# bdaiinstitute/vlfm

Measured on AMD Instinct MI355X. Metric: env-steps/s (VLM+value-map update), 640x480 RGB-D, higher is better.
Workload: dtype f16 ViT-g (f32 accumulate) + f32 Q-Former (split-f16, 22-bit); f32 confidence + f64 value maps; 1 GPU; configs[1] step x resident envs: BLIP-2 ITC + ValueMap+ObstacleMap+sort_waypoints; envs_per_gpu=256, global_envs=256, map=1000x1000 @ 20 px/m, parallelism=env-sharded x1, tuned_gemms=True, vit_gemm=hip:fc1, attention=hip

## Files before the change

### include/vlfm_amd.h

```cpp
#ifndef VLFM_AMD_H
#define VLFM_AMD_H

#include <stddef.h>
#include <stdint.h>

#ifdef __cplusplus
extern "C" {
#endif

typedef enum {
    VLFM_OK = 0,
    VLFM_ERR_INVALID = -1,
    VLFM_ERR_OUTSIDE_MAP = -2,
    VLFM_ERR_INDEX = -3,
    VLFM_ERR_HIP = -4,
    VLFM_ERR_CAPACITY = -5
} vlfm_status;

enum { VLFM_FUSE_DEFAULT = 0, VLFM_FUSE_REPLACE = 1, VLFM_FUSE_EQUAL_WEIGHTING = 2 };

const char* vlfm_last_error(void);
int vlfm_abi_version(void);

int vlfm_profile_enable(int on);
int vlfm_profile_read(const char* kernel_name, double* mean_ms, int* launches);

int vlfm_host_wait_mode(int blocking);

typedef struct {
    double inv_affine[6];
    int32_t row0, col0;
    int32_t env;
    int32_t reserved;
} vlfm_vm_pose;

int vlfm_value_map_pose_params(const double* h_tf, const double* h_yaw, const int32_t* h_env, int n, int map_size,
                               int pixels_per_meter, int template_size, vlfm_vm_pose* h_out, int* bad_index);

int vlfm_cone_template_host(double fov, double max_depth, int pixels_per_meter, double min_confidence,
                            float* h_conf, int conf_capacity, int64_t* h_poly_xy, int poly_capacity,
                            int* n_poly);

int vlfm_tan_table_host(double fov, int width, double* h_out);

int vlfm_cone_template_build(const float* d_conf, const int64_t* d_poly_xy, int n_poly, int template_size,
                             float* d_template, uint32_t* d_template_bits, void* stream);

typedef struct {
    double tf[12];
    float depth_scale;
    float depth_offset;
    float depth_max;
    float reserved0;
    double fx, fy;
    double min_height, max_height;
    int32_t env;
    int32_t scatter;
} vlfm_ingest_params;

typedef struct {
    uint32_t* d_cells;
    int32_t* d_count;
    int32_t capacity;
    int32_t reserved;
} vlfm_scatter_journal;

int vlfm_depth_ingest_batched(const float* d_depth, int n, int height, int width,
                              const vlfm_ingest_params* d_params,
                              uint32_t* d_colmax_keys ,
                              uint32_t* d_obstacle , int map_size, int pixels_per_meter,
                              int32_t* d_status ,
                              uint32_t* d_hole_bits ,
                              const uint32_t* d_filled_bits ,
                              const vlfm_scatter_journal* journal ,
                              void* stream);

int vlfm_selftest_div_exact(const double* d_numerators, int n, double divisor, int32_t* d_mismatches, void* stream);

size_t vlfm_hole_scratch_bytes(int n, int height, int width, int cap_pts, int cap_contours);
int vlfm_fill_small_holes_batched(const uint32_t* d_hole_bits, const int32_t* d_status, int n, int height, int width,
                                  double area_thresh, void* d_scratch, size_t scratch_bytes, int cap_pts,
                                  int cap_contours, uint32_t* d_filled_bits, int32_t* d_counts,
                                  const vlfm_ingest_params* d_params, uint32_t* d_obstacle, int map_size,
                                  const vlfm_scatter_journal* journal, void* stream);
int vlfm_depth_scatter_holes_batched(const vlfm_ingest_params* d_params, int n, int height, int width,
                                     const uint32_t* d_hole_bits, const uint32_t* d_filled_bits,
                                     const int32_t* d_hole_counts ,
                                     uint32_t* d_obstacle, int map_size, int pixels_per_meter, int32_t* d_status,
                                     const float* d_depth ,
                                     void* stream);

int vlfm_fill_small_holes_rig_batched(const uint32_t* d_hole_bits, const int32_t* d_status, int n, int height, int width,
                                      double area_thresh, void* d_scratch, size_t scratch_bytes, int cap_pts,
                                      int cap_contours, uint32_t* d_filled_bits, int32_t* d_counts,
                                      const vlfm_ingest_params* d_params, uint32_t* d_obstacle, int map_size,
                                      const vlfm_scatter_journal* journal, int32_t* d_slot_undone, int n_envs, void* stream);
int vlfm_depth_scatter_holes_rig_batched(const vlfm_ingest_params* d_params, int n, int height, int width,
                                         const uint32_t* d_hole_bits, const uint32_t* d_filled_bits,
                                         const int32_t* d_hole_counts, uint32_t* d_obstacle, int map_size,
                                         int pixels_per_meter, int32_t* d_status, const float* d_depth,
                                         const int32_t* d_slot_undone, void* stream);

int vlfm_value_map_update_fused_batched(uint32_t* d_colmax_keys, int width, const double* d_tan,
                                        const float* d_template, const uint32_t* d_template_bits, int template_size,
                                        const vlfm_vm_pose* d_pose, const double* d_values, int n,
                                        float* d_conf, double* d_value, int map_size, int channels, int pixels_per_meter,
                                        double min_depth, double max_depth, int use_max_confidence, int fusion_type,
                                        const uint32_t* d_explored_bits, uint32_t* d_written_bits, int32_t* d_counters,
                                        const float* d_conf_quadrant, void* stream);

typedef struct {
    const float* d_template;
    const uint32_t* d_template_bits;
    const float* d_conf_quadrant;
    const double* d_tan;
    float depth_scale;
    float depth_offset;
    int32_t template_size;
    int32_t reserved;
} vlfm_vm_optics;

int vlfm_value_map_update_rig_batched(uint32_t* d_colmax_keys, int width, const vlfm_vm_pose* d_pose,
                                      const vlfm_vm_optics* d_optics, const int32_t* d_slots, int n_slots, int n,
                                      int max_template_size, const double* d_values, float* d_conf, double* d_value,
                                      int map_size, int channels, int pixels_per_meter, int use_max_confidence,
                                      int fusion_type, const uint32_t* d_explored_bits, uint32_t* d_written_bits,
                                      int32_t* d_counters, void* stream);

int vlfm_disc_rows_host(int radius, int32_t* h_halfwidth );
int vlfm_value_map_sort_waypoints_batched(const double* d_value, int map_size, int channels,
                                          const int32_t* d_cells, int m, int radius, const int32_t* d_disc,
                                          int value_is_f32, double* d_out, void* stream);



int vlfm_resample_coeffs_host(int in_size, int out_size, int32_t* h_bounds, int32_t* h_kk, int kk_capacity,
                              int* ksize_out);

int vlfm_resample_coeffs_filter_host(int in_size, int out_size, int filter, int32_t* h_bounds, int32_t* h_kk,
                                     int kk_capacity, int* ksize_out);

int vlfm_preprocess_sam_batched(const uint8_t* d_rgb, int n, int height, int width, int out_h, int out_w,
                                const int32_t* d_hbounds, const int32_t* d_hk, int hksize,
                                const int32_t* d_vbounds, const int32_t* d_vk, int vksize,
                                const float* h_mean3, const float* h_std3, int pad_size, uint8_t* d_tmp, float* d_out,
                                void* stream);

int vlfm_preprocess_rgb_batched(const uint8_t* d_rgb, int n, int height, int width, int out_size,
                                const int32_t* d_hbounds, const int32_t* d_hk, int hksize,
                                const int32_t* d_vbounds, const int32_t* d_vk, int vksize,
                                const float* h_mean3, const float* h_std3, uint8_t* d_tmp, void* d_out,
                                int out_dtype, int patch_size, void* stream);

int vlfm_itc_head_batched(const float* d_proj, int batch, int n_query, int proj_dim,
                          const float* d_text, float* d_out, void* stream);

#define VLFM_ITC_MAX_PROMPTS 8
int vlfm_itc_head_multi(const float* d_proj, int batch, int n_query, int proj_dim, const float* d_text_table, int n_text,
                        const int32_t* d_text_index, int n_prompts, float* d_out, void* stream);

int vlfm_layernorm_bias_f16(const void* d_x, const float* d_channel_bias, const void* d_gamma, const void* d_beta,
                            void* d_y, int rows, int dim, float eps, void* stream);

int vlfm_vit_attention_f16(const void* d_qkv, void* d_out, int batch, int tokens, int heads, int head_dim, float scale,
                           void* stream);

int vlfm_gemm_f16_nt(const void* d_x, const void* d_w, const void* d_bias, void* d_c, int m, int n, int k, int epilogue,
                     void* stream);

int vlfm_gemm_f16_pair_f32_nt(const void* d_x, const void* d_w_pair, const void* d_bias_f32, void* d_out, int m, int n_out, int k,
                              void* stream);

int vlfm_qformer_cross_attention_f32(const void* d_q, const void* d_kv_blocks, void* d_out, int batch, int tokens, int queries,
                                     int heads, int k_block0, int v_block0, int m_total, float scale, void* stream);

int vlfm_gemm_f16_tile_order(int m, int n, int group_m, int* out, int capacity_pairs);
int vlfm_gemm_f16_work_items(int m, int n, int grid, int* out, int capacity_pairs);

int vlfm_split_f32_to_f16_pair(const float* d_src, void* d_hi, void* d_lo, long long count, int* d_overflow, void* stream);
int vlfm_gemm_f32_nt(const float* d_x, const float* d_w, const float* d_bias, const float* d_residual, float* d_c, int m, int n,
                     int k, int activation, int precision, const void* d_w_hi, const void* d_w_lo, int* d_overflow, void* stream);


int vlfm_layernorm_rows_f32(const float* d_x, const float* d_gamma, const float* d_beta, float* d_out, int batch, int height,
                            int width, int channels, int window, float eps, void* stream);
int vlfm_window_reverse_add_f32(float* d_x, const float* d_windows, int batch, int height, int width, int channels, int window,
                                void* stream);
int vlfm_dwconv3x3_nhwc_f32(const float* d_x, const float* d_w9c, const float* d_bias, float* d_out, int batch, int height, int width,
                            int channels, void* stream);
int vlfm_window_attention_f32(const float* d_qkv, const float* d_bias_t, float* d_out, long long windows, int tokens, int heads,
                              float scale, void* stream);
int vlfm_layernorm_rows_shifted_f32(const float* d_x, const float* d_gamma, const float* d_beta, float* d_out, int batch, int height,
                                    int width, int channels, int window, float eps, int shift, int pad_zero, void* stream);
int vlfm_window_reverse_add_shifted_f32(float* d_x, const float* d_windows, int batch, int height, int width, int channels, int window,
                                        int shift, void* stream);
int vlfm_window_attention_masked_f32(const float* d_qkv, const float* d_bias_t, const float* d_mask_t, int windows_per_image, float* d_out,
                                     long long windows, int tokens, int heads, float scale, void* stream);

int vlfm_maxpool2x2_nhwc_f16(const void* d_x, void* d_out, int batch, int height, int width, int channels, void* stream);
int vlfm_conv_nhwc_tile(int pixels, int cin, int cout, int ksize, int* tile_pixels, int* tile_channels);
int vlfm_conv_nhwc_f16(const void* d_x, const void* d_w, const void* d_bias, void* d_out, const void* d_zero, int batch,
                       int height, int width, int cin, int cout, int ksize, int stride, int x_pix_stride,
                       int out_pix_stride, int act, void* stream);

int vlfm_resize_area_tab_host(int ssize, int dsize, int32_t* h_first, int32_t* h_count, float* h_w, int ktaps_capacity);

int vlfm_resize_area_batched(const uint8_t* d_rgb, int n, int height, int width, int out_h, int out_w,
                             const int32_t* d_xfirst, const int32_t* d_xcount, const float* d_xw, int xktaps,
                             const int32_t* d_yfirst, const int32_t* d_ycount, const float* d_yw, int yktaps,
                             void* d_out, int out_dtype, void* stream);

int vlfm_to_tensor_normalize_batched(const uint8_t* d_rgb, int n, int height, int width, const float* h_mean3,
                                     const float* h_std3, float* d_out, void* stream);

size_t vlfm_nms_scratch_bytes(int n);
int vlfm_nms(const float* d_boxes_xyxy, const int32_t* d_order, int n, float iou_threshold, void* d_scratch,
             size_t scratch_bytes, int32_t* d_keep, int32_t* d_num_keep, int max_keep, void* stream);

int vlfm_ms_deform_attn(const float* d_value, const int32_t* d_spatial_shapes, const int32_t* d_level_start,
                        const float* d_sampling_loc, const float* d_attn_weight, int batch, int n_query, int n_heads,
                        int head_dim, int n_levels, int n_points, int total_len, float* d_out, void* stream);
int vlfm_ms_deform_attn_fused(const float* d_value, const int32_t* d_spatial_shapes, const int32_t* d_level_start,
                              const float* d_offsets_logits, const float* d_reference, int batch, int n_query, int n_heads,
                              int head_dim, int n_levels, int n_points, int ref_coords, int total_len, float* d_out, void* stream);

int vlfm_dwconv3x3_f32(const float* d_x, const float* d_w, const float* d_bias, float* d_y, int n, int channels, int height,
                       int width, int stride, int gelu, void* stream);

int vlfm_bias_act_nchw(void* d_y, const void* d_bias, int n, int channels, long long hw, int dtype, int act, void* stream);


size_t vlfm_object_cloud_scratch_bytes(int height, int width);
int vlfm_object_cloud_extract(const float* d_depth, const uint8_t* d_mask, int height, int width, int erosion_iterations,
                              double min_depth, double max_depth, double fx, double fy, void* d_scratch, double* d_cloud,
                              int capacity, int32_t* d_count, void* stream);

size_t vlfm_dbscan_scratch_bytes(int n);
int vlfm_dbscan_largest_cluster(const double* d_points, int n, double eps, int min_points, void* d_scratch,
                                size_t scratch_bytes, int32_t* d_labels, int32_t* d_keep, int32_t* d_num_keep, void* stream);

size_t vlfm_object_cloud_batch_scratch_bytes(int jobs, int height, int width);
int vlfm_object_cloud_batch_stats(const uint8_t* d_masks, const int32_t* d_erosion, int jobs, int max_erosion, int height, int width,
                                  void* d_scratch, int32_t* d_stats, void* stream);
int vlfm_object_cloud_batch_expand(const float* d_depth, int frames, int height, int width, double min_depth, double max_depth,
                                   double fx, double fy, const void* d_scratch, int scratch_jobs, const int32_t* d_jobs, int n_jobs,
                                   int max_points, const int32_t* d_ranks, int n_ranks, double* d_points, int capacity, void* stream);
size_t vlfm_dbscan_batch_scratch_bytes(int n);
int vlfm_dbscan_largest_cluster_batch(const double* d_points, int capacity, const int64_t* d_jobs, int n_jobs, int max_n, double eps,
                                      int min_points, void* d_scratch, size_t scratch_bytes, double* d_kept, int32_t* d_num_keep,
                                      void* stream);
long long vlfm_object_cloud_launch_count(void);


typedef struct {
    const double* d_rows;
    const int32_t* d_slots;
    double p[3];
    double heading, half_fov, range;
    int32_t n, k, flag_offset, n_slots;
} vlfm_cloud_query;

int vlfm_cloud_cone_flags(const vlfm_cloud_query* d_queries, int n_queries, int max_points, int32_t* d_flags, void* stream);

size_t vlfm_cloud_closest_scratch_bytes(int n_queries, int max_points);
int vlfm_cloud_closest(const vlfm_cloud_query* d_queries, int n_queries, int max_points, void* d_scratch, size_t scratch_bytes,
                       int32_t* d_result, void* stream);
int vlfm_cloud_query_chunk(void);
long long vlfm_cloud_query_launch_count(void);

int vlfm_bits_pack(const uint8_t* d_src, uint32_t* d_dst, int planes, int rows, int cols, void* stream);
int vlfm_bits_unpack(const uint32_t* d_src, uint8_t* d_dst, int planes, int rows, int cols, void* stream);

int vlfm_bits_dilate(const uint32_t* d_src, uint32_t* d_dst, int planes, int rows, int cols, int kernel_w,
                     int kernel_h, void* stream);

int vlfm_find_contours_external(const uint32_t* d_img, int planes, int rows, int cols, int method,
                                uint32_t* d_scratch , int32_t* d_pts, int cap_pts,
                                int32_t* d_starts, int32_t* d_lens, int cap_contours, int32_t* d_counts, void* stream);

size_t vlfm_find_contours_wg_scratch_bytes(int planes, int rows, int cols, int cap_pts);
int vlfm_walk_path_counters(long long* h_out4, int reset);
int vlfm_find_contours_external_wg(const uint32_t* d_img, int planes, int rows, int cols, int method, void* d_scratch,
                                   size_t scratch_bytes, int32_t* d_pts, int cap_pts, int32_t* d_starts, int32_t* d_lens,
                                   int cap_contours, int32_t* d_counts, void* stream);

#define VLFM_FOG_MAX_POLY 80
typedef struct {
    int32_t env;
    int32_t ax, ay;
    int32_t radius;
    int32_t n_poly;
    int32_t reserved;
    double rot_c, rot_s;
    double line_len;
    long long poly[2 * VLFM_FOG_MAX_POLY];
} vlfm_fog_params;

int vlfm_fog_params_host(const int32_t* h_agent_px, const double* h_angle_cv2_deg, const double* h_rot_cs,
                         double fov_deg, double max_line_len, const int32_t* h_env, const int32_t* h_explore, int n,
                         vlfm_fog_params* h_out);

size_t vlfm_obstacle_scratch_bytes(int n_envs, int map_size, int cap_pts, int cap_contours);

int vlfm_obstacle_map_update_batched(const vlfm_fog_params* d_prm, int n, const uint32_t* d_obstacle,
                                     uint32_t* d_navigable, uint32_t* d_explored, int32_t* d_bbox, int n_envs,
                                     int map_size, int kernel_size, int fog_radius, double area_thresh_px,
                                     void* d_scratch, size_t scratch_bytes, int cap_pts, int cap_contours,
                                     double* d_frontiers, int cap_frontiers, int32_t* d_counts, int update_obstacles,
                                     int explore, const int32_t* d_windows, int window_blocks_navigable,
                                     int window_blocks_prepare, void* stream);

int vlfm_obstacle_status(const void* d_scratch, int n_envs, int map_size, int cap_pts, int cap_contours,
                         int32_t* h_out);

enum { VLFM_REDUCE_MAX = 0,
       VLFM_REDUCE_EXPLORE = 1,
       VLFM_REDUCE_PLANE = 2 };
enum { VLFM_PRIM_CIRCLE_FILL = 0,
       VLFM_PRIM_CIRCLE = 1,
       VLFM_PRIM_LINE = 2,
       VLFM_PRIM_POLYLINE = 3 };
#define VLFM_RENDER_FLIP_ROWS 1
#define VLFM_RENDER_UNDER_PATH 2
typedef struct {
    int32_t frame;
    int32_t kind;
    int32_t flags;
    int32_t thickness;
    int32_t x0, y0, x1, y1;
    int32_t vtx_off, n_vtx;
    uint8_t bgr[4];
    int32_t reserved;
} vlfm_render_prim;

size_t vlfm_value_render_scratch_bytes(int n, int map_size);

int vlfm_value_map_render(const double* d_value, int n_envs, int map_size, int channels, const int32_t* d_frames, int n,
                          int reduce_mode, double explore_thresh, const double* d_plane, const uint32_t* d_explored,
                          const uint32_t* d_path, const int32_t* d_prim_off, const vlfm_render_prim* d_prims,
                          const int64_t* d_vtx, int rgb, void* d_scratch, size_t scratch_bytes, uint8_t* d_out,
                          void* stream);

int vlfm_obstacle_map_render(const uint32_t* d_obstacle, const uint32_t* d_navigable, const uint32_t* d_explored,
                             int n_envs, int map_size, const int32_t* d_frames, int n, uint32_t pad_bgr,
                             const uint32_t* d_path, const int32_t* d_prim_off, const vlfm_render_prim* d_prims,
                             const int64_t* d_vtx, int rgb, uint8_t* d_out, void* stream);

int vlfm_traj_append(uint32_t* d_path, int n_envs, int map_size, const int32_t* d_segs, int m, int thickness,
                     void* stream);

int vlfm_circle_polygon_host(const int32_t* h_circles, int n, int64_t* h_xy, int32_t* h_off, int capacity);

int vlfm_jpeg_quant_tables_host(int quality, uint16_t* h_tables);
size_t vlfm_jpeg_scratch_bytes(int n, int H, int W);
int vlfm_jpeg_roundtrip_batched(const uint8_t* d_in, uint8_t* d_out, int n, int H, int W, const uint16_t* h_tables,
                                void* d_scratch, size_t scratch_bytes, void* stream);

int vlfm_jpeg_header_host(int quality, int H, int W, uint8_t* h_out, size_t cap, size_t* len);
size_t vlfm_jpeg_encode_bound(int H, int W);
size_t vlfm_jpeg_encode_scratch_bytes(int n, int H, int W);
int vlfm_jpeg_encode_batched(const uint8_t* d_in, int n, int H, int W, int rgb_order, const uint16_t* h_tables,
                             uint8_t* d_out, size_t capacity, uint32_t* d_lengths, void* d_scratch, size_t scratch_bytes,
                             void* stream);

typedef struct vlfm_jpeg_huff {
    uint32_t limit[16];
    int32_t delta[16];
    uint8_t vals[256];
} vlfm_jpeg_huff;
typedef struct vlfm_jpeg_table_set {
    uint16_t quant[3][64];
    vlfm_jpeg_huff dc[3];
    vlfm_jpeg_huff ac[3];
} vlfm_jpeg_table_set;
typedef struct vlfm_jpeg_frame {
    int32_t height, width, restart_interval, scan_offset, table_set, reserved[3];
} vlfm_jpeg_frame;
enum {
    VLFM_JPEG_BAD_HEADER = 1,
    VLFM_JPEG_BAD_LENGTH = 2,
    VLFM_JPEG_BAD_EOI = 3,
    VLFM_JPEG_BAD_RESTART = 4,
    VLFM_JPEG_BAD_CODE = 5,
    VLFM_JPEG_BAD_SIZE = 6,
    VLFM_JPEG_BAD_INDEX = 7,
    VLFM_JPEG_BAD_BITS = 8
};
int vlfm_jpeg_parse_host(const uint8_t* h_file, size_t len, vlfm_jpeg_frame* frame, vlfm_jpeg_table_set* set);
const char* vlfm_jpeg_parse_reason(int code);
size_t vlfm_jpeg_decode_chunk_bytes(void);
size_t vlfm_jpeg_decode_scratch_bytes(int n, int H, int W, size_t max_file_bytes);
int vlfm_jpeg_decode_batched(const uint8_t* d_files, size_t files_bytes, const int64_t* d_offsets, size_t stride,
                             const int32_t* d_lengths, int n, int H, int W, const vlfm_jpeg_frame* d_frames,
                             const vlfm_jpeg_table_set* d_sets, int n_sets, const uint8_t* d_header, int header_bytes,
                             int max_segments, size_t max_file_bytes, int rgb_order, uint8_t* d_out, int32_t* d_status,
                             void* d_scratch, size_t scratch_bytes, void* stream);

int vlfm_rooms_raycast(const double* d_cameras, int n, const double* d_boxes, int n_boxes, int H, int W, float* d_out,
                       void* stream);

int vlfm_rooms_raycast_objects(const double* d_cameras, int n, const double* d_boxes, int n_boxes, const double* d_objects,
                               const int32_t* d_env_of, int n_envs, int H, int W, float* d_depth, uint8_t* d_ids,
                               int32_t* d_stats, void* stream);

#ifdef __cplusplus
}
#endif
#endif
```

### vlfm_amd/_lib.py

```python
from __future__ import annotations

import ctypes
import os
import subprocess
from typing import Optional

_HERE = os.path.dirname(os.path.abspath(__file__))
LIB_PATH = os.path.join(_HERE, "libvlfm_amd.so")
SOURCES = ["value_map.hip", "depth_ingest.hip", "depth_holes.hip", "obstacle_map.hip", "vlm_ops.hip", "vit_attention.hip", "qformer_attention.hip", "detect_ops.hip", "object_cloud.hip", "cloud_query.hip", "gemm_f16.hip", "gemm_f32.hip", "conv_nhwc.hip", "sam_ops.hip", "map_render.hip", "jpeg_codec.hip", "jpeg_entropy.hip", "jpeg_decode.hip", "world_render.hip", "host.cpp"]

VLFM_OK = 0
VLFM_ERR_INVALID = -1
VLFM_ERR_OUTSIDE_MAP = -2
VLFM_ERR_INDEX = -3
VLFM_ERR_HIP = -4
VLFM_ERR_CAPACITY = -5

FUSION_TYPES = {"default": 0, "replace": 1, "equal_weighting": 2}


class VmPose(ctypes.Structure):
    _fields_ = [("inv_affine", ctypes.c_double * 6), ("row0", ctypes.c_int32), ("col0", ctypes.c_int32),
                ("env", ctypes.c_int32), ("reserved", ctypes.c_int32)]


class IngestParams(ctypes.Structure):
    _fields_ = [("tf", ctypes.c_double * 12), ("depth_scale", ctypes.c_float), ("depth_offset", ctypes.c_float),
                ("depth_max", ctypes.c_float), ("reserved0", ctypes.c_float), ("fx", ctypes.c_double),
                ("fy", ctypes.c_double), ("min_height", ctypes.c_double), ("max_height", ctypes.c_double),
                ("env", ctypes.c_int32), ("scatter", ctypes.c_int32)]


FOG_MAX_POLY = 80


class FogParams(ctypes.Structure):
    _fields_ = [("env", ctypes.c_int32), ("ax", ctypes.c_int32), ("ay", ctypes.c_int32), ("radius", ctypes.c_int32),
                ("n_poly", ctypes.c_int32), ("reserved", ctypes.c_int32), ("rot_c", ctypes.c_double),
                ("rot_s", ctypes.c_double), ("line_len", ctypes.c_double), ("poly", ctypes.c_longlong * (2 * FOG_MAX_POLY))]


class ScatterJournal(ctypes.Structure):
    _fields_ = [("d_cells", ctypes.c_void_p), ("d_count", ctypes.c_void_p), ("capacity", ctypes.c_int32),
                ("reserved", ctypes.c_int32)]


class VmOptics(ctypes.Structure):
    _fields_ = [("d_template", ctypes.c_void_p), ("d_template_bits", ctypes.c_void_p), ("d_conf_quadrant", ctypes.c_void_p),
                ("d_tan", ctypes.c_void_p), ("depth_scale", ctypes.c_float), ("depth_offset", ctypes.c_float),
                ("template_size", ctypes.c_int32), ("reserved", ctypes.c_int32)]


class CloudQuery(ctypes.Structure):
    _fields_ = [("d_rows", ctypes.c_void_p), ("d_slots", ctypes.c_void_p), ("p", ctypes.c_double * 3),
                ("heading", ctypes.c_double), ("half_fov", ctypes.c_double), ("range", ctypes.c_double),
                ("n", ctypes.c_int32), ("k", ctypes.c_int32), ("flag_offset", ctypes.c_int32), ("n_slots", ctypes.c_int32)]


assert ctypes.sizeof(CloudQuery) == 80
assert ctypes.sizeof(ScatterJournal) == 24 and ctypes.sizeof(VmOptics) == 48
assert ctypes.sizeof(VmPose) == 64 and ctypes.sizeof(IngestParams) == 152 and ctypes.sizeof(FogParams) == 48 + 16 * FOG_MAX_POLY


def build(verbose: bool = False) -> str:
    from concurrent.futures import ThreadPoolExecutor

    csrc = os.path.join(_HERE, "csrc")
    srcs = [os.path.join(csrc, s) for s in SOURCES if os.path.exists(os.path.join(csrc, s))]
    hdrs = [os.path.join(csrc, h) for h in os.listdir(csrc) if h.endswith(".h")] + [
        os.path.join(_HERE, "..", "include", "vlfm_amd.h")]
    hdr_time = max(os.path.getmtime(h) for h in hdrs)
    objdir = os.path.join(csrc, "build")
    os.makedirs(objdir, exist_ok=True)
    flags = ["--offload-arch=gfx950", "-O3", "-std=c++17", "-fPIC", "-ffp-contract=off"]

    def compile_one(src: str) -> str:
        obj = os.path.join(objdir, os.path.basename(src) + ".o")
        if not os.path.exists(obj) or os.path.getmtime(obj) < max(os.path.getmtime(src), hdr_time):
            cmd = ["hipcc"] + flags + ["-c", src, "-o", obj]
            if verbose:
                print(" ".join(cmd), flush=True)
            subprocess.check_call(cmd)
        return obj

    with ThreadPoolExecutor(max_workers=min(8, len(srcs))) as pool:
        objs = list(pool.map(compile_one, srcs))
    if os.path.exists(LIB_PATH) and all(os.path.getmtime(LIB_PATH) >= os.path.getmtime(o) for o in objs):
        return LIB_PATH
    cmd = ["hipcc", "--offload-arch=gfx950", "-shared", "-fPIC", "-o", LIB_PATH] + objs
    if verbose:
        print(" ".join(cmd), flush=True)
    subprocess.check_call(cmd)
    return LIB_PATH


_lib: Optional[ctypes.CDLL] = None


def lib() -> ctypes.CDLL:
    global _lib
    if _lib is None:
        if not os.path.exists(LIB_PATH):
            raise ImportError(
                f"{LIB_PATH} is missing: build it with `python -c 'import __graft_entry__ as g; g.build()'` "
                "(hipcc --offload-arch=gfx950).  vlfm_amd has no CPU fallback.")
        L = ctypes.CDLL(LIB_PATH)
        vp, ci, cd = ctypes.c_void_p, ctypes.c_int, ctypes.c_double
        L.vlfm_last_error.restype = ctypes.c_char_p
        L.vlfm_abi_version.restype = ci
        L.vlfm_profile_enable.argtypes = [ci]
        L.vlfm_host_wait_mode.argtypes = [ci]
        L.vlfm_profile_read.argtypes = [ctypes.c_char_p, ctypes.POINTER(cd), ctypes.POINTER(ci)]
        L.vlfm_value_map_pose_params.argtypes = [vp, vp, vp, ci, ci, ci, ci, vp, ctypes.POINTER(ci)]
        L.vlfm_cone_template_host.argtypes = [cd, cd, ci, cd, vp, ci, vp, ci, ctypes.POINTER(ci)]
        L.vlfm_tan_table_host.argtypes = [cd, ci, vp]
        L.vlfm_disc_rows_host.argtypes = [ci, vp]
        L.vlfm_cone_template_build.argtypes = [vp, vp, ci, ci, vp, vp, vp]
        L.vlfm_depth_ingest_batched.argtypes = [vp, ci, ci, ci, vp, vp, vp, ci, ci, vp, vp, vp, vp, vp]
        L.vlfm_selftest_div_exact.argtypes = [vp, ci, cd, vp, vp]
        L.vlfm_hole_scratch_bytes.argtypes = [ci, ci, ci, ci, ci]
        L.vlfm_hole_scratch_bytes.restype = ctypes.c_size_t
        L.vlfm_fill_small_holes_batched.argtypes = [vp, vp, ci, ci, ci, cd, vp, ctypes.c_size_t, ci, ci, vp, vp, vp, vp,
                                                    ci, vp, vp]
        L.vlfm_depth_scatter_holes_batched.argtypes = [vp, ci, ci, ci, vp, vp, vp, vp, ci, ci, vp, vp, vp]
        L.vlfm_fill_small_holes_rig_batched.argtypes = [vp, vp, ci, ci, ci, cd, vp, ctypes.c_size_t, ci, ci, vp, vp, vp, vp,
                                                        ci, vp, vp, ci, vp]
        L.vlfm_depth_scatter_holes_rig_batched.argtypes = [vp, ci, ci, ci, vp, vp, vp, vp, ci, ci, vp, vp, vp, vp]
        L.vlfm_layernorm_bias_f16.argtypes = [vp, vp, vp, vp, vp, ci, ci, ctypes.c_float, vp]
        L.vlfm_vit_attention_f16.argtypes = [vp, vp, ci, ci, ci, ci, ctypes.c_float, vp]
        L.vlfm_gemm_f16_nt.argtypes = [vp, vp, vp, vp, ci, ci, ci, ci, vp]
        L.vlfm_gemm_f16_pair_f32_nt.argtypes = [vp, vp, vp, vp, ci, ci, ci, vp]
        L.vlfm_qformer_cross_attention_f32.argtypes = [vp, vp, vp, ci, ci, ci, ci, ci, ci, ci, ctypes.c_float, vp]
        L.vlfm_gemm_f32_nt.argtypes = [vp, vp, vp, vp, vp, ci, ci, ci, ci, ci, vp, vp, vp, vp]
        L.vlfm_split_f32_to_f16_pair.argtypes = [vp, vp, vp, ctypes.c_longlong, vp, vp]
        L.vlfm_layernorm_rows_f32.argtypes = [vp, vp, vp, vp, ci, ci, ci, ci, ci, ctypes.c_float, vp]
        L.vlfm_window_reverse_add_f32.argtypes = [vp, vp, ci, ci, ci, ci, ci, vp]
        L.vlfm_dwconv3x3_nhwc_f32.argtypes = [vp, vp, vp, vp, ci, ci, ci, ci, vp]
        L.vlfm_window_attention_f32.argtypes = [vp, vp, vp, ctypes.c_longlong, ci, ci, ctypes.c_float, vp]
        L.vlfm_layernorm_rows_shifted_f32.argtypes = [vp, vp, vp, vp, ci, ci, ci, ci, ci, ctypes.c_float, ci, ci, vp]
        L.vlfm_window_reverse_add_shifted_f32.argtypes = [vp, vp, ci, ci, ci, ci, ci, ci, vp]
        L.vlfm_window_attention_masked_f32.argtypes = [vp, vp, vp, ci, vp, ctypes.c_longlong, ci, ci, ctypes.c_float, vp]
        L.vlfm_maxpool2x2_nhwc_f16.argtypes = [vp, vp, ci, ci, ci, ci, vp]
        L.vlfm_conv_nhwc_tile.argtypes = [ci, ci, ci, ci, ctypes.POINTER(ci), ctypes.POINTER(ci)]
        L.vlfm_conv_nhwc_f16.argtypes = [vp, vp, vp, vp, vp, ci, ci, ci, ci, ci, ci, ci, ci, ci, ci, vp]
        L.vlfm_value_map_update_fused_batched.argtypes = [vp, ci, vp, vp, vp, ci, vp, vp, ci, vp, vp, ci, ci, ci, cd, cd,
                                                          ci, ci, vp, vp, vp, vp, vp]
        L.vlfm_value_map_update_rig_batched.argtypes = [vp, ci, vp, vp, vp, ci, ci, ci, vp, vp, vp, ci, ci, ci, ci, ci, vp, vp,
                                                        vp, vp]
        L.vlfm_value_map_sort_waypoints_batched.argtypes = [vp, ci, ci, vp, ci, ci, vp, ci, vp, vp]
        L.vlfm_resample_coeffs_host.argtypes = [ci, ci, vp, vp, ci, ctypes.POINTER(ci)]
        L.vlfm_resample_coeffs_filter_host.argtypes = [ci, ci, ci, vp, vp, ci, ctypes.POINTER(ci)]
        L.vlfm_preprocess_sam_batched.argtypes = [vp, ci, ci, ci, ci, ci, vp, vp, ci, vp, vp, ci, vp, vp, ci, vp, vp, vp]
        L.vlfm_preprocess_rgb_batched.argtypes = [vp, ci, ci, ci, ci, vp, vp, ci, vp, vp, ci, vp, vp, vp, vp, ci, ci, vp]
        L.vlfm_itc_head_batched.argtypes = [vp, ci, ci, ci, vp, vp, vp]
        L.vlfm_itc_head_multi.argtypes = [vp, ci, ci, ci, vp, ci, vp, ci, vp, vp]
        cf = ctypes.c_float
        L.vlfm_resize_area_tab_host.argtypes = [ci, ci, vp, vp, vp, ci]
        L.vlfm_resize_area_batched.argtypes = [vp, ci, ci, ci, ci, ci, vp, vp, vp, ci, vp, vp, vp, ci, vp, ci, vp]
        L.vlfm_to_tensor_normalize_batched.argtypes = [vp, ci, ci, ci, vp, vp, vp, vp]
        L.vlfm_nms_scratch_bytes.argtypes = [ci]
        L.vlfm_nms_scratch_bytes.restype = ctypes.c_size_t
        L.vlfm_nms.argtypes = [vp, vp, ci, cf, vp, ctypes.c_size_t, vp, vp, ci, vp]
        L.vlfm_ms_deform_attn.argtypes = [vp, vp, vp, vp, vp, ci, ci, ci, ci, ci, ci, ci, vp, vp]
        L.vlfm_ms_deform_attn_fused.argtypes = [vp, vp, vp, vp, vp, ci, ci, ci, ci, ci, ci, ci, ci, vp, vp]
        L.vlfm_object_cloud_scratch_bytes.argtypes = [ci, ci]
        L.vlfm_object_cloud_scratch_bytes.restype = ctypes.c_size_t
        L.vlfm_object_cloud_extract.argtypes = [vp, vp, ci, ci, ci, cd, cd, cd, cd, vp, vp, ci, vp, vp]
        L.vlfm_dbscan_scratch_bytes.argtypes = [ci]
        L.vlfm_dbscan_scratch_bytes.restype = ctypes.c_size_t
        L.vlfm_dbscan_largest_cluster.argtypes = [vp, ci, cd, ci, vp, ctypes.c_size_t, vp, vp, vp, vp]
        L.vlfm_object_cloud_batch_scratch_bytes.argtypes = [ci, ci, ci]
        L.vlfm_object_cloud_batch_scratch_bytes.restype = ctypes.c_size_t
        L.vlfm_object_cloud_batch_stats.argtypes = [vp, vp, ci, ci, ci, ci, vp, vp, vp]
        L.vlfm_object_cloud_batch_expand.argtypes = [vp, ci, ci, ci, cd, cd, cd, cd, vp, ci, vp, ci, ci, vp, ci, vp, ci, vp]
        L.vlfm_dbscan_batch_scratch_bytes.argtypes = [ci]
        L.vlfm_dbscan_batch_scratch_bytes.restype = ctypes.c_size_t
        L.vlfm_dbscan_largest_cluster_batch.argtypes = [vp, ci, vp, ci, ci, cd, ci, vp, ctypes.c_size_t, vp, vp, vp]
        L.vlfm_object_cloud_launch_count.argtypes = []
        L.vlfm_object_cloud_launch_count.restype = ctypes.c_longlong
        L.vlfm_cloud_cone_flags.argtypes = [vp, ci, ci, vp, vp]
        L.vlfm_cloud_closest_scratch_bytes.argtypes = [ci, ci]
        L.vlfm_cloud_closest_scratch_bytes.restype = ctypes.c_size_t
        L.vlfm_cloud_closest.argtypes = [vp, ci, ci, vp, ctypes.c_size_t, vp, vp]
        L.vlfm_cloud_query_chunk.argtypes = []
        L.vlfm_cloud_query_launch_count.argtypes = []
        L.vlfm_cloud_query_launch_count.restype = ctypes.c_longlong
        L.vlfm_bits_pack.argtypes = [vp, vp, ci, ci, ci, vp]
        L.vlfm_bits_unpack.argtypes = [vp, vp, ci, ci, ci, vp]
        L.vlfm_bits_dilate.argtypes = [vp, vp, ci, ci, ci, ci, ci, vp]
        L.vlfm_find_contours_external.argtypes = [vp, ci, ci, ci, ci, vp, vp, ci, vp, vp, ci, vp, vp]
        L.vlfm_dwconv3x3_f32.argtypes = [vp, vp, vp, vp, ci, ci, ci, ci, ci, ci, vp]
        L.vlfm_bias_act_nchw.argtypes = [vp, vp, ci, ci, ctypes.c_longlong, ci, ci, vp]
        L.vlfm_find_contours_wg_scratch_bytes.argtypes = [ci, ci, ci, ci]
        L.vlfm_find_contours_wg_scratch_bytes.restype = ctypes.c_size_t
        L.vlfm_find_contours_external_wg.argtypes = [vp, ci, ci, ci, ci, vp, ctypes.c_size_t, vp, ci, vp, vp, ci, vp, vp]
        L.vlfm_walk_path_counters.argtypes = [vp, ci]
        L.vlfm_fog_params_host.argtypes = [vp, vp, vp, cd, cd, vp, vp, ci, vp]
        L.vlfm_obstacle_scratch_bytes.argtypes = [ci, ci, ci, ci]
        L.vlfm_obstacle_scratch_bytes.restype = ctypes.c_size_t
        L.vlfm_obstacle_map_update_batched.argtypes = [vp, ci, vp, vp, vp, vp, ci, ci, ci, ci, cd, vp, ctypes.c_size_t,
                                                       ci, ci, vp, ci, vp, ci, ci, vp, ci, ci, vp]
        L.vlfm_obstacle_status.argtypes = [vp, ci, ci, ci, ci, vp]
        L.vlfm_value_render_scratch_bytes.argtypes = [ci, ci]
        L.vlfm_value_render_scratch_bytes.restype = ctypes.c_size_t
        L.vlfm_value_map_render.argtypes = [vp, ci, ci, ci, vp, ci, ci, cd, vp, vp, vp, vp, vp, vp, ci, vp,
                                            ctypes.c_size_t, vp, vp]
        L.vlfm_obstacle_map_render.argtypes = [vp, vp, vp, ci, ci, vp, ci, ctypes.c_uint32, vp, vp, vp, vp, ci, vp, vp]
        L.vlfm_traj_append.argtypes = [vp, ci, ci, vp, ci, ci, vp]
        L.vlfm_circle_polygon_host.argtypes = [vp, ci, vp, vp, ci]
        L.vlfm_jpeg_quant_tables_host.argtypes = [ci, vp]
        L.vlfm_jpeg_scratch_bytes.argtypes = [ci, ci, ci]
        L.vlfm_jpeg_scratch_bytes.restype = ctypes.c_size_t
        L.vlfm_jpeg_roundtrip_batched.argtypes = [vp, vp, ci, ci, ci, vp, vp, ctypes.c_size_t, vp]
        L.vlfm_jpeg_header_host.argtypes = [ci, ci, ci, vp, ctypes.c_size_t, ctypes.POINTER(ctypes.c_size_t)]
        L.vlfm_jpeg_encode_bound.argtypes = [ci, ci]
        L.vlfm_jpeg_encode_bound.restype = ctypes.c_size_t
        L.vlfm_jpeg_encode_scratch_bytes.argtypes = [ci, ci, ci]
        L.vlfm_jpeg_encode_scratch_bytes.restype = ctypes.c_size_t
        L.vlfm_jpeg_encode_batched.argtypes = [vp, ci, ci, ci, ci, vp, vp, ctypes.c_size_t, vp, vp, ctypes.c_size_t, vp]
        L.vlfm_jpeg_parse_host.argtypes = [vp, ctypes.c_size_t, vp, vp]
        L.vlfm_jpeg_parse_reason.argtypes = [ci]
        L.vlfm_jpeg_parse_reason.restype = ctypes.c_char_p
        L.vlfm_jpeg_decode_chunk_bytes.restype = ctypes.c_size_t
        L.vlfm_jpeg_decode_scratch_bytes.argtypes = [ci, ci, ci, ctypes.c_size_t]
        L.vlfm_jpeg_decode_scratch_bytes.restype = ctypes.c_size_t
        L.vlfm_jpeg_decode_batched.argtypes = [vp, ctypes.c_size_t, vp, ctypes.c_size_t, vp, ci, ci, ci, vp, vp, ci, vp, ci, ci,
                                               ctypes.c_size_t, ci, vp, vp, vp, ctypes.c_size_t, vp]
        L.vlfm_rooms_raycast.argtypes = [vp, ci, vp, ci, ci, ci, vp, vp]
        L.vlfm_rooms_raycast_objects.argtypes = [vp, ci, vp, ci, vp, vp, ci, ci, ci, vp, vp, vp, vp]
        _lib = L
    return _lib


def profile_read(kernel: str):
    ms, n = ctypes.c_double(0.0), ctypes.c_int(0)
    lib().vlfm_profile_read(kernel.encode(), ctypes.byref(ms), ctypes.byref(n))
    return ms.value, n.value


def last_error() -> str:
    return lib().vlfm_last_error().decode()


def host_wait_blocking(device=None, blocking: bool = True) -> None:
    import torch

    with torch.cuda.device(device if device is not None else torch.cuda.current_device()):
        check(lib().vlfm_host_wait_mode(int(bool(blocking))), "host_wait_mode")


def try_host_wait_blocking(device=None) -> bool:
    import os
    import warnings

    if os.environ.get("VLFM_HOST_WAIT", "blocking") == "spin":
        return False
    try:
        host_wait_blocking(device)
        return True
    except Exception as exc:
        warnings.warn(f"blocking host waits not enabled on {device}: {exc} (call vlfm_amd._lib.host_wait_blocking before the "
                      f"device's first allocation; waits will spin on a host core)")
        return False


def check(rc: int, what: str = "") -> int:
    if rc >= 0:
        return rc
    msg = last_error()
    if rc == VLFM_ERR_OUTSIDE_MAP:
        raise AssertionError(msg or "Pixel location is outside the image.")
    if rc == VLFM_ERR_INDEX:
        raise IndexError(msg or "index out of bounds for obstacle map")
    raise RuntimeError(f"libvlfm_amd {what} failed ({rc}): {msg}")
```

### vlfm_amd/csrc/gemm_f16.hip

```cpp
#include <hip/hip_runtime.h>
#include <stdint.h>

#include "../../include/vlfm_amd.h"
#include "gelu_f16.h"
#include "profile.h"
#include "status.h"

namespace vlfm {

typedef _Float16 half8 __attribute__((ext_vector_type(8)));
typedef _Float16 half4 __attribute__((ext_vector_type(4)));
typedef float floatx4 __attribute__((ext_vector_type(4)));
typedef float f32x16 __attribute__((ext_vector_type(16)));

constexpr int GB = 256;
constexpr int GK = 64;
constexpr int ROWB = GK * 2;
constexpr int OPER = GB * ROWB;
constexpr int BUF = 2 * OPER;
constexpr int EPI_ROW = 272;
constexpr int EPI_WAVE = 64 * EPI_ROW;
constexpr int GEMM_LDS = 8 * EPI_WAVE > 2 * BUF ? 8 * EPI_WAVE : 2 * BUF;
enum { EPI_BIAS = 0, EPI_BIAS_GELU = 1, EPI_ACCUM = 2,
       EPI_PAIR_F32 = 3 };

struct GemmArgs {
    const _Float16* x;
    const _Float16* w;
    const _Float16* bias;
    _Float16* c;
    int M, N, K;
    int tiles_m, tiles_n;
    int group_m;
    int split_ragged;
};

using lds_ptr = __attribute__((address_space(3))) unsigned char*;
using gbl_ptr = const __attribute__((address_space(1))) unsigned char*;

template <int EPI, int BAL, int SYNC = 2>
struct Gemm8p {
    static constexpr int SLOT = 128 * ROWB;
    static constexpr int KBUF = 4 * SLOT;

    const GemmArgs& a;
    lds_ptr lds;
    const unsigned char* smem;
    int wave, lane;
    bool half;
    bool active;
    uint32_t voff[4][2];
    uint32_t rdP[2], rdQ[2];
    half8 fp[4][2], fq0[BAL ? 2 : 1][2][2], fq1[2][2];
    floatx4 acc[8][4];

    __device__ Gemm8p(const GemmArgs& a_, unsigned char* smem_, int m0, int n0) : a(a_), lds((lds_ptr)smem_), smem(smem_) {
        const int tid = threadIdx.x;
        lane = tid & 63;
        wave = __builtin_amdgcn_readfirstlane(tid >> 6);
        const int wn = wave >> 2, wm = wave & 3;
        half = false;
        active = n0 + wn * (half ? 64 : 128) < a.N;
        offsets(m0, n0, voff);
        const int r16 = lane & 15, swz = (r16 >> 1) & 7, s0 = lane >> 4;
        const uint32_t bp = (uint32_t)(wn * 64 + r16) * ROWB + (uint32_t)((s0 ^ swz) << 4);
        const uint32_t bq = (uint32_t)(wm * 32 + r16) * ROWB + (uint32_t)((s0 ^ swz) << 4);
        rdP[0] = bp; rdP[1] = bp ^ 64u;
        rdQ[0] = bq; rdQ[1] = bq ^ 64u;
        zero_acc();
    }
    __device__ inline void zero_acc() {
#pragma unroll
        for (int i = 0; i < 8; i++)
#pragma unroll
            for (int j = 0; j < 4; j++) acc[i][j] = floatx4{0.f, 0.f, 0.f, 0.f};
    }
    __device__ inline void kill_fragments() {
        const half8 z = {(_Float16)0.f, (_Float16)0.f, (_Float16)0.f, (_Float16)0.f, (_Float16)0.f, (_Float16)0.f, (_Float16)0.f, (_Float16)0.f};
#pragma unroll
        for (int f = 0; f < 4; f++) { fp[f][0] = z; fp[f][1] = z; }
#pragma unroll
        for (int g = 0; g < 2; g++)
#pragma unroll
            for (int k = 0; k < 2; k++) {
                fq1[g][k] = z;
#pragma unroll
                for (int q = 0; q < (BAL ? 2 : 1); q++) fq0[q][g][k] = z;
            }
    }
    __device__ inline void offsets(int m0, int n0, uint32_t (&vo)[4][2]) const {
        const int sub = lane >> 3, p = lane & 7;
#pragma unroll
        for (int j = 0; j < 2; j++) {
            const int rho = (wave * 2 + j) * 8 + sub;
            const int s = p ^ ((rho >> 1) & 7);
#pragma unroll
            for (int h = 0; h < 2; h++) {
                const int rq = min(m0 + (rho >> 5) * 64 + h * 32 + (rho & 31), a.M - 1);
                const int rp = min(n0 + (half ? rho + h * 128 : (rho >> 6) * 128 + h * 64 + (rho & 63)), a.N - 1);
                vo[2 * h][j] = (uint32_t)rq * (uint32_t)a.K * 2u + (uint32_t)s * 16u;
                vo[2 * h + 1][j] = (uint32_t)rp * (uint32_t)a.K * 2u + (uint32_t)s * 16u;
            }
        }
    }

    template <int SLOT_ID>
    __device__ inline void stage_at(int b, int t, const uint32_t (&vo)[4][2]) {
        const unsigned char* base = reinterpret_cast<const unsigned char*>((SLOT_ID & 1) ? a.w : a.x) + (size_t)t * (GK * 2);
#pragma unroll
        for (int j = 0; j < 2; j++) {
            const int dst = __builtin_amdgcn_readfirstlane(b * KBUF + SLOT_ID * SLOT + (wave * 2 + j) * 1024);
            __builtin_amdgcn_global_load_lds((gbl_ptr)(base + vo[SLOT_ID][j]), lds + dst, 16, 0, 0);
        }
    }
    template <int SLOT_ID>
    __device__ inline void stage(int b, int t) { stage_at<SLOT_ID>(b, t, voff); }
    template <int B, int SLOT_ID>
    __device__ inline void read_p() {
#pragma unroll
        for (int kk = 0; kk < 2; kk++)
#pragma unroll
            for (int f = 0; f < 4; f++)
                fp[f][kk] = *reinterpret_cast<const half8*>(smem + B * KBUF + SLOT_ID * SLOT + f * 16 * ROWB + rdP[kk]);
    }
    template <int B, int SLOT_ID>
    __device__ inline void read_q(half8 (&fq)[2][2]) {
#pragma unroll
        for (int kk = 0; kk < 2; kk++)
#pragma unroll
            for (int g = 0; g < 2; g++)
                fq[g][kk] = *reinterpret_cast<const half8*>(smem + B * KBUF + SLOT_ID * SLOT + g * 16 * ROWB + rdQ[kk]);
    }
    template <int PI, int QJ>
    __device__ inline void mma(const half8 (&fq)[2][2]) {
#pragma unroll
        for (int kk = 0; kk < 2; kk++)
#pragma unroll
            for (int f = 0; f < 4; f++)
#pragma unroll
                for (int g = 0; g < 2; g++)
                    acc[PI * 4 + f][QJ * 2 + g] =
                        __builtin_amdgcn_mfma_f32_16x16x32_f16(fp[f][kk], fq[g][kk], acc[PI * 4 + f][QJ * 2 + g], 0, 0, 0);
    }
    static __device__ inline void bar() {
        __builtin_amdgcn_s_barrier();
        asm volatile("" ::: "memory");
    }
    template <int PI, int QJ>
    __device__ inline void compute(const half8 (&fq)[2][2], bool work = true) {
        bar();
        __builtin_amdgcn_s_waitcnt(0xC07F);
        __builtin_amdgcn_sched_barrier(0);
        if (active && work) {
            __builtin_amdgcn_s_setprio(1);
            mma<PI, QJ>(fq);
            __builtin_amdgcn_s_setprio(0);
        }
        __builtin_amdgcn_sched_barrier(0);
        if (SYNC == 2) bar();
    }

    template <int B>
    __device__ inline void tile(int t, int NT) {
        constexpr int QS = BAL ? B : 0;
        if (active) {
            if (!BAL) read_q<B, 0>(fq0[QS]);
            read_p<B, 1>();
        }
        __builtin_amdgcn_sched_barrier(0);
        if (t + 1 < NT) stage<2>(B ^ 1, t + 1);
        compute<0, 0>(fq0[QS]);
        if (active) read_q<B, 2>(fq1);
        __builtin_amdgcn_sched_barrier(0);
        if (t + 1 < NT) stage<3>(B ^ 1, t + 1);
        compute<0, 1>(fq1);
        if (active) read_p<B, 3>();
        __builtin_amdgcn_sched_barrier(0);
        if (t + 2 < NT) {
            stage<0>(B, t + 2);
            if (BAL) __builtin_amdgcn_s_waitcnt(0x0F78);
        } else if (BAL) {
            __builtin_amdgcn_s_waitcnt(0x0F76);
        }
        compute<1, 1>(fq1);
        if (BAL && active && t + 1 < NT) read_q<B ^ 1, 0>(fq0[BAL ? (B ^ 1) : 0]);
        __builtin_amdgcn_sched_barrier(0);
        if (t + 2 < NT) {
            stage<1>(B, t + 2);
            __builtin_amdgcn_s_waitcnt(0x0F74);
        } else {
            __builtin_amdgcn_s_waitcnt(0x0F70);
        }
        compute<1, 0>(fq0[QS]);
    }
};

__host__ __device__ inline void tile_of(const GemmArgs& a, int bid, int& tm, int& tn) {
    const int nwg = a.tiles_m * a.tiles_n;
    const int xcd = bid & 7, idx = bid >> 3;
    const int tail_cols = a.N - (a.tiles_n - 1) * GB;
    const bool ragged = a.tiles_n > 1 && tail_cols <= GB / 2;
    const int ncols = ragged ? a.tiles_n - 1 : a.tiles_n;
    const int nfull = a.tiles_m * ncols, nhalf = nwg - nfull;
    const int qf = nfull >> 3, rf = nfull & 7, qh = nhalf >> 3, rh = nhalf & 7;
    const int myfull = qf + (xcd < rf ? 1 : 0);
    if (idx < myfull) {
        const int f = xcd * qf + min(xcd, rf) + idx;
        const int GM = a.group_m;
        const int per_group = GM * ncols, grp = f / per_group, in = f - grp * per_group;
        const int rows = min(GM, a.tiles_m - grp * GM);
        tn = in / rows;
        tm = grp * GM + (in - tn * rows);
    } else {
        int before = 0;
        for (int x = 0; x < xcd; x++) before += (((x - rf) & 7) < rh) ? 1 : 0;
        tm = xcd * qh + before + (idx - myfull);
        tn = a.tiles_n - 1;
    }
}

constexpr int EPI2_ROW = 144;
constexpr int EPI2_WAVE = 64 * EPI2_ROW;
constexpr int PBIAS_OFF = GEMM_LDS;
constexpr int GEMM_LDS_P = GEMM_LDS + 512;

__device__ __forceinline__ half8 add_half8(half8 a, const half8 b) {
#pragma unroll
    for (int e = 0; e < 8; e++) a[e] = (_Float16)((float)a[e] + (float)b[e]);
    return a;
}
template <int EPI, int H>
__device__ __forceinline__ void epi2_pass(const floatx4 (&acc)[8][4], const half4 (&bias4)[8], unsigned char* stg, int g4, int c16, int rsub,
                                 int chunk, half8 (&v)[8]) {
#pragma unroll
    for (int ii = 0; ii < 4; ii++) {
        constexpr int I0 = H * 4;
        const float b0 = (float)bias4[I0 + ii][0], b1 = (float)bias4[I0 + ii][1], b2 = (float)bias4[I0 + ii][2], b3 = (float)bias4[I0 + ii][3];
#pragma unroll
        for (int j = 0; j < 4; j++) {
            float v0 = acc[I0 + ii][j][0] + b0, v1 = acc[I0 + ii][j][1] + b1, v2 = acc[I0 + ii][j][2] + b2, v3 = acc[I0 + ii][j][3] + b3;
            if (EPI == EPI_BIAS_GELU) gelu_erf4(v0, v1, v2, v3);
            const half4 hv = {(_Float16)v0, (_Float16)v1, (_Float16)v2, (_Float16)v3};
            *reinterpret_cast<half4*>(stg + (j * 16 + c16) * EPI2_ROW + (ii * 16 + g4) * 2) = hv;
        }
    }
    __builtin_amdgcn_s_waitcnt(0xC07F);
#pragma unroll
    for (int it = 0; it < 8; it++) v[it] = *reinterpret_cast<const half8*>(stg + (it * 8 + rsub) * EPI2_ROW + chunk * 16);
}
template <int P>
__device__ __forceinline__ void epi_pair_pass(const floatx4 (&acc)[8][4], const floatx4 (&bias4)[4], unsigned char* stg, int g4, int c16,
                                              int rsub, int chunk, floatx4 (&v)[8]) {
#pragma clang fp contract(off)
#pragma unroll
    for (int i2 = 0; i2 < 2; i2++) {
        constexpr int I0 = 2 * P;
#pragma unroll
        for (int j = 0; j < 4; j++) {
            floatx4 r;
#pragma unroll
            for (int e = 0; e < 4; e++) {
                const float low = acc[4 + I0 + i2][j][e] * 0x1p-11f;
                const float mid = bias4[I0 + i2][e] + low;
                r[e] = acc[I0 + i2][j][e] + mid;
            }
            *reinterpret_cast<floatx4*>(stg + (j * 16 + c16) * EPI2_ROW + (i2 * 16 + g4) * 4) = r;
        }
    }
    __builtin_amdgcn_s_waitcnt(0xC07F);
#pragma unroll
    for (int it = 0; it < 8; it++) v[it] = *reinterpret_cast<const floatx4*>(stg + (it * 8 + rsub) * EPI2_ROW + chunk * 16);
}
__device__ __forceinline__ void stage_bias(const GemmArgs& a, lds_ptr lds, int wave, int lane, int n_first) {
    if (a.bias != nullptr && wave == 0 && lane < 32) {
        const _Float16* src = a.bias + min(n_first + lane * 8, a.N - 8);
        __builtin_amdgcn_global_load_lds((gbl_ptr)src, lds + PBIAS_OFF, 16, 0, 0);
    }
}

struct WorkList {
    int nwg, first_split, nitems;
    __host__ __device__ WorkList(int nwg_, int grid, bool allow = true) : nwg(nwg_) {
        const int left = nwg > grid ? nwg % grid : 0;
        const bool split = allow && left > 0 && 2 * left <= grid;
        first_split = split ? nwg - left : nwg;
        nitems = nwg + (split ? left : 0);
    }
    __host__ __device__ void item(int w, int& pos, int& half) const {
        if (w < first_split) { pos = w; half = -1; }
        else { const int j = w - first_split; pos = first_split + (j >> 1); half = j & 1; }
    }
};

template <int EPI>
__global__ __launch_bounds__(512) void gemm_f16_8pp_kernel(GemmArgs a) {
    extern __shared__ __attribute__((aligned(16))) unsigned char smem[];
    using G = Gemm8p<EPI, 1, 2>;
    const int stride = gridDim.x;
    const WorkList work(a.tiles_m * a.tiles_n, stride, a.split_ragged != 0);
    int bid = blockIdx.x;
    int tm, tn, pos, half;
    work.item(bid, pos, half);
    tile_of(a, pos, tm, tn);
    int m0 = tm * GB, n0 = tn * GB;
    G g(a, smem, m0, n0);
    g.active = g.active && (half < 0 || half == (g.wave >> 2));
    const int NT = a.K / GK;
    const int wave = g.wave, lane = g.lane, wn = wave >> 2, wm = wave & 3, late = wn;
    const int g4 = (lane >> 4) * 4, c16 = lane & 15;
    const int rsub = lane >> 3, chunk = lane & 7;
    unsigned char* stg = smem + G::KBUF + wave * EPI2_WAVE;
    const bool has_bias = a.bias != nullptr;
    stage_bias(a, g.lds, wave, lane, n0);
    g.template stage<0>(0, 0); g.template stage<1>(0, 0); g.template stage<2>(0, 0); g.template stage<3>(0, 0);
    if (NT > 1) {
        g.template stage<0>(1, 1); g.template stage<1>(1, 1);
        __builtin_amdgcn_s_waitcnt(0x0F74);
    } else {
        __builtin_amdgcn_s_waitcnt(0x0F70);
    }
    g.bar();
    for (;;) {
        g.kill_fragments();
        if (late) g.bar();
        if (g.active) g.template read_q<0, 0>(g.fq0[0]);
        for (int t = 0; t < NT; t += 2) {
            g.template tile<0>(t, NT);
            if (t + 1 < NT) g.template tile<1>(t + 1, NT);
        }
        if (!late) g.bar();

        half4 bias4[EPI == EPI_PAIR_F32 ? 1 : 8];
        floatx4 biasf[EPI == EPI_PAIR_F32 ? 4 : 1];
        if constexpr (EPI == EPI_PAIR_F32) {
#pragma unroll
            for (int i = 0; i < 4; i++) {
                const floatx4 ld = *reinterpret_cast<const floatx4*>(smem + PBIAS_OFF + (wn * 64 + i * 16 + g4) * 4);
                biasf[i] = has_bias ? ld : floatx4{0.f, 0.f, 0.f, 0.f};
            }
        } else {
#pragma unroll
            for (int i = 0; i < 8; i++) {
                const half4 ld = *reinterpret_cast<const half4*>(smem + PBIAS_OFF + (wn * 128 + i * 16 + g4) * 2);
                bias4[i] = has_bias ? ld : half4{(_Float16)0.f, (_Float16)0.f, (_Float16)0.f, (_Float16)0.f};
            }
        }
        __builtin_amdgcn_sched_barrier(0);
        const int nbid = bid + stride;
        const bool more = nbid < work.nitems;
        const bool store = g.active;
        work.item(more ? nbid : bid, pos, half);
        tile_of(a, pos, tm, tn);
        const int m1 = tm * GB, n1 = tn * GB;
        uint32_t von[4][2];
        g.offsets(m1, n1, von);
        g.template stage_at<0>(0, 0, von); g.template stage_at<1>(0, 0, von);
        g.template stage_at<2>(0, 0, von); g.template stage_at<3>(0, 0, von);
        __builtin_amdgcn_sched_barrier(0);
        half8 old[EPI == EPI_ACCUM ? 16 : 1];
        if (EPI == EPI_ACCUM) {
#pragma unroll
            for (int h = 0; h < 2; h++)
#pragma unroll
                for (int it = 0; it < 8; it++) {
                    const int m = min(m0 + wm * 64 + it * 8 + rsub, a.M - 1);
                    const int n = max(min(n0 + wn * 128 + h * 64 + chunk * 8, a.N - 8), 0);
                    old[h * 8 + it] = *reinterpret_cast<const half8*>(a.c + (size_t)m * a.N + n);
                }
        }
        __builtin_amdgcn_sched_barrier(0);
        if constexpr (EPI == EPI_PAIR_F32) {
            (void)bias4; (void)old;
            floatx4 p0[8], p1[8];
            epi_pair_pass<0>(g.acc, biasf, stg, g4, c16, rsub, chunk, p0);
            epi_pair_pass<1>(g.acc, biasf, stg, g4, c16, rsub, chunk, p1);
            __builtin_amdgcn_sched_barrier(0);
            __builtin_amdgcn_s_waitcnt(0x0F70);
            __builtin_amdgcn_sched_barrier(0);
            const int nblk = n0 + wn * 128;
            if (store && nblk + 128 <= a.N) {
                float* ob = reinterpret_cast<float*>(a.c) + (size_t)(nblk >> 7) * (size_t)a.M * 64 + chunk * 4;
#pragma unroll
                for (int it = 0; it < 8; it++) {
                    const int m = m0 + wm * 64 + it * 8 + rsub;
                    if (m < a.M) *reinterpret_cast<floatx4*>(ob + (size_t)m * 64) = p0[it];
                }
#pragma unroll
                for (int it = 0; it < 8; it++) {
                    const int m = m0 + wm * 64 + it * 8 + rsub;
                    if (m < a.M) *reinterpret_cast<floatx4*>(ob + (size_t)m * 64 + 32) = p1[it];
                }
            }
        } else {
        (void)biasf;
        half8 v0[8], v1[8];
        epi2_pass<EPI, 0>(g.acc, bias4, stg, g4, c16, rsub, chunk, v0);
        epi2_pass<EPI, 1>(g.acc, bias4, stg, g4, c16, rsub, chunk, v1);
        if (EPI == EPI_ACCUM) {
#pragma unroll
            for (int it = 0; it < 8; it++) {
                v0[it] = add_half8(v0[it], old[it]);
                v1[it] = add_half8(v1[it], old[8 + it]);
            }
        }
        __builtin_amdgcn_sched_barrier(0);
        __builtin_amdgcn_s_waitcnt(0x0F70);
        __builtin_amdgcn_sched_barrier(0);
        {
            const int n = n0 + wn * 128 + chunk * 8;
            if (store && n + 8 <= a.N) {
#pragma unroll
                for (int it = 0; it < 8; it++) {
                    const int m = m0 + wm * 64 + it * 8 + rsub;
                    if (m < a.M) *reinterpret_cast<half8*>(a.c + (size_t)m * a.N + n) = v0[it];
                }
            }
            if (store && n + 64 + 8 <= a.N) {
#pragma unroll
                for (int it = 0; it < 8; it++) {
                    const int m = m0 + wm * 64 + it * 8 + rsub;
                    if (m < a.M) *reinterpret_cast<half8*>(a.c + (size_t)m * a.N + n + 64) = v1[it];
                }
            }
        }
        }
        if (!more) break;
        bid = nbid; m0 = m1; n0 = n1;
#pragma unroll
        for (int s = 0; s < 4; s++) { g.voff[s][0] = von[s][0]; g.voff[s][1] = von[s][1]; }
        g.active = n0 + wn * 128 < a.N && (half < 0 || half == wn);
        g.zero_acc();
        g.bar();
        stage_bias(a, g.lds, wave, lane, n0);
        if (NT > 1) { g.template stage<0>(1, 1); g.template stage<1>(1, 1); }
    }
}


}

using namespace vlfm;

template <int EPI>
static int launch_gemm(const GemmArgs& a, hipStream_t stream) {
    const void* fn = reinterpret_cast<const void*>(gemm_f16_8pp_kernel<EPI>);
    static LdsOptIn optp;
    if (!optp.ensure(fn, GEMM_LDS_P)) return fail(VLFM_ERR_HIP, "gemm_f16_nt: cannot opt in to the LDS size");
    const int n_cu = device_cu_count() & ~7;
    const int nwg = a.tiles_m * a.tiles_n;
    const dim3 grid(nwg < n_cu ? nwg : n_cu), block(512);
    VLFM_TIMED(EPI == EPI_BIAS ? "gemm_f16_8pp_kernel<0>" : EPI == EPI_BIAS_GELU ? "gemm_f16_8pp_kernel<1>" :
               EPI == EPI_ACCUM ? "gemm_f16_8pp_kernel<2>" : "gemm_f16_8pp_kernel<3>", stream);
    VLFM_KLAUNCH((gemm_f16_8pp_kernel<EPI>), grid, block, GEMM_LDS_P, stream, a);
    return check_launch("gemm_f16_8pp_kernel");
}

extern "C" int vlfm_gemm_f16_nt(const void* d_x, const void* d_w, const void* d_bias, void* d_c, int m, int n, int k,
                                int epilogue, void* stream) {
    if (m == 0 || n == 0) return VLFM_OK;
    if (!d_x || !d_w || !d_c || m < 0 || n < 0 || k <= 0 || (k % GK) != 0 || (n % 8) != 0 || epilogue < 0 || epilogue > 2)
        return fail(VLFM_ERR_INVALID, "gemm_f16_nt: K must be a multiple of 64, N of 8, epilogue 0, 1 or 2");
    if (((uintptr_t)d_x | (uintptr_t)d_w | (uintptr_t)d_c | (uintptr_t)d_bias) & 15)
        return fail(VLFM_ERR_INVALID, "gemm_f16_nt: X, W, C and the bias must be 16-byte aligned");
    if ((size_t)m * (size_t)k * 2 >= (1ull << 32) || (size_t)n * (size_t)k * 2 >= (1ull << 32))
        return fail(VLFM_ERR_INVALID, "gemm_f16_nt: an operand of 4 GB or more (32-bit byte offsets inside an operand)");
    GemmArgs a;
    a.x = (const _Float16*)d_x; a.w = (const _Float16*)d_w; a.bias = (const _Float16*)d_bias; a.c = (_Float16*)d_c;
    a.M = m; a.N = n; a.K = k;
    a.tiles_m = (m + GB - 1) / GB; a.tiles_n = (n + GB - 1) / GB;
    a.group_m = 4;
    a.split_ragged = 1;
    if (epilogue == 0) return launch_gemm<EPI_BIAS>(a, (hipStream_t)stream);
    if (epilogue == 1) return launch_gemm<EPI_BIAS_GELU>(a, (hipStream_t)stream);
    return launch_gemm<EPI_ACCUM>(a, (hipStream_t)stream);
}

extern "C" int vlfm_gemm_f16_pair_f32_nt(const void* d_x, const void* d_w_pair, const void* d_bias_f32, void* d_out, int m, int n_out,
                                         int k, void* stream) {
    if (m == 0 || n_out == 0) return VLFM_OK;
    if (!d_x || !d_w_pair || !d_out || m < 0 || n_out < 0 || k <= 0 || (k % GK) != 0 || (n_out % 64) != 0)
        return fail(VLFM_ERR_INVALID, "gemm_f16_pair_f32_nt: K and N_out must be multiples of 64");
    if (((uintptr_t)d_x | (uintptr_t)d_w_pair | (uintptr_t)d_out | (uintptr_t)d_bias_f32) & 15)
        return fail(VLFM_ERR_INVALID, "gemm_f16_pair_f32_nt: X, the weight pair, the result and the bias must be 16-byte aligned");
    if ((size_t)m * (size_t)k * 2 >= (1ull << 32) || (size_t)n_out * (size_t)k * 4 >= (1ull << 32))
        return fail(VLFM_ERR_INVALID, "gemm_f16_pair_f32_nt: an operand of 4 GB or more (32-bit byte offsets inside an operand)");
    GemmArgs a;
    a.x = (const _Float16*)d_x; a.w = (const _Float16*)d_w_pair;
    a.bias = (const _Float16*)d_bias_f32;
    a.c = (_Float16*)d_out;
    a.M = m; a.N = 2 * n_out; a.K = k;
    a.tiles_m = (m + GB - 1) / GB; a.tiles_n = (a.N + GB - 1) / GB;
    a.group_m = 4;
    a.split_ragged = 1;
    return launch_gemm<EPI_PAIR_F32>(a, (hipStream_t)stream);
}

extern "C" int vlfm_gemm_f16_tile_order(int m, int n, int group_m, int* out, int capacity_pairs) {
    if (m <= 0 || n <= 0 || !out) return fail(VLFM_ERR_INVALID, "gemm_f16_tile_order: m, n > 0 and an output array");
    GemmArgs a{};
    a.M = m; a.N = n; a.K = GK;
    a.tiles_m = (m + GB - 1) / GB; a.tiles_n = (n + GB - 1) / GB;
    a.group_m = group_m > 0 ? group_m : 4;
    const int nwg = a.tiles_m * a.tiles_n;
    if (capacity_pairs < nwg) return fail(VLFM_ERR_INVALID, "gemm_f16_tile_order: output array too small");
    for (int b = 0; b < nwg; b++) tile_of(a, b, out[2 * b], out[2 * b + 1]);
    return nwg;
}

extern "C" int vlfm_gemm_f16_work_items(int m, int n, int grid, int* out, int capacity_pairs) {
    if (m <= 0 || n <= 0 || grid <= 0 || !out) return fail(VLFM_ERR_INVALID, "gemm_f16_work_items: m, n, grid > 0 and an output array");
    const int nwg = ((m + GB - 1) / GB) * ((n + GB - 1) / GB);
    const WorkList work(nwg, grid < nwg ? grid : nwg);
    if (capacity_pairs < work.nitems) return fail(VLFM_ERR_INVALID, "gemm_f16_work_items: output array too small");
    for (int w = 0; w < work.nitems; w++) work.item(w, out[2 * w], out[2 * w + 1]);
    return work.nitems;
}
```

### vlfm_amd/csrc/host.cpp

```cpp
#include <cmath>
#include <cstdint>
#include <cstring>
#include <mutex>
#include <string>

#include "../../include/vlfm_amd.h"
#include "status.h"

namespace vlfm {
static thread_local std::string g_last_error;
void set_last_error(const char* msg) { g_last_error = msg ? msg : ""; }
}

extern "C" const char* vlfm_last_error(void) { return vlfm::g_last_error.c_str(); }
extern "C" int vlfm_abi_version(void) { return 18; }

namespace {

const double kPi = 3.141592653589793238462643383279502884;

inline long round_half_even(double v) { return std::lrint(v); }

float sin_deg_table(int deg) {
    static float tab[451];
    static std::once_flag once;
    std::call_once(once, [] {
        for (int i = 0; i <= 450; i++) tab[i] = (float)(std::round(std::sin(i * kPi / 180.0) * 1e7) / 1e7);
    });
    return tab[deg];
}

}

extern "C" int vlfm_value_map_pose_params(const double* h_tf, const double* h_yaw, const int32_t* h_env, int n,
                                          int map_size, int pixels_per_meter, int template_size,
                                          vlfm_vm_pose* h_out, int* bad_index) {
    if (!h_tf || !h_out || n < 0 || map_size <= 0 || template_size <= 0)
        return vlfm::fail(VLFM_ERR_INVALID, "value_map_pose_params: bad argument");
    const double ppm = (double)pixels_per_meter;
    const int half = template_size / 2;
    for (int k = 0; k < n; k++) {
        const double* tf = h_tf + 16 * k;
        const double yaw = h_yaw ? h_yaw[k] : std::atan2(tf[4], tf[0]);
        const double degrees = (-yaw) * (180.0 / kPi);
        const double ang = degrees * (kPi / 180);
        const double alpha = std::cos(ang), beta = std::sin(ang);
        const double cx = (double)(float)half, cy = (double)(float)half;
        double M[6] = {alpha, beta, (1 - alpha) * cx - beta * cy, -beta, alpha, beta * cx + (1 - alpha) * cy};
        double D = M[0] * M[4] - M[1] * M[3];
        D = D != 0 ? 1. / D : 0;
        const double A11 = M[4] * D, A22 = M[0] * D;
        M[0] = A11; M[1] *= -D;
        M[3] *= -D; M[4] = A22;
        const double b1 = -M[0] * M[2] - M[1] * M[5];
        const double b2 = -M[3] * M[2] - M[4] * M[5];
        M[2] = b1; M[5] = b2;
        vlfm_vm_pose& p = h_out[k];
        std::memcpy(p.inv_affine, M, sizeof(M));
        const double cam_x = tf[3] / tf[15], cam_y = tf[7] / tf[15];
        const long px = (long)(cam_x * ppm) + map_size / 2;
        const long py = (long)(-cam_y * ppm) + map_size / 2;
        if (px < 0 || px >= map_size || py < 0 || py >= map_size) {
            if (bad_index) *bad_index = k;
            return vlfm::fail(VLFM_ERR_OUTSIDE_MAP, "Pixel location is outside the image.");
        }
        p.row0 = (int32_t)(px - half);
        p.col0 = (int32_t)(py - half);
        p.env = h_env ? h_env[k] : k;
        p.reserved = 0;
    }
    return VLFM_OK;
}

static int ellipse_sector_polygon(int cx, int cy, int radius, double start_angle, double end_angle, int64_t* out_xy,
                                  int capacity) {
    int a0 = (int)round_half_even(start_angle), a1 = (int)round_half_even(end_angle);
    const bool full = (a1 - a0) >= 360;
    if (a0 > a1) { int t = a0; a0 = a1; a1 = t; }
    while (a0 < 0) { a0 += 360; a1 += 360; }
    while (a1 > 360) { a1 -= 360; a0 -= 360; }
    if (a1 - a0 > 360) { a0 = 0; a1 = 360; }
    const int step = radius < 3 ? 90 : radius < 10 ? 30 : radius < 15 ? 18 : 5;
    const double ccx = (double)((int64_t)cx << 16), ccy = (double)((int64_t)cy << 16);
    const double axis = (double)((int64_t)radius << 16);
    int m = 0;
    int64_t last_x = -1, last_y = -1;
    for (int a = a0; a < a1 + step; a += step) {
        int t = a > a1 ? a1 : a;
        if (t < 0) t += 360;
        const double ex = axis * sin_deg_table(450 - t), ey = axis * sin_deg_table(t);
        const double vx = ccx + ex * sin_deg_table(90) - ey * sin_deg_table(0);
        const double vy = ccy + ex * sin_deg_table(0) + ey * sin_deg_table(90);
        int64_t qx = (int64_t)round_half_even(vx / 65536.0) << 16, qy = (int64_t)round_half_even(vy / 65536.0) << 16;
        qx += round_half_even(vx - (double)qx);
        qy += round_half_even(vy - (double)qy);
        if (qx == last_x && qy == last_y) continue;
        if (m >= capacity) return VLFM_ERR_CAPACITY;
        out_xy[2 * m] = qx; out_xy[2 * m + 1] = qy; m++;
        last_x = qx; last_y = qy;
    }
    if (!full) {
        if (m >= capacity) return VLFM_ERR_CAPACITY;
        out_xy[2 * m] = (int64_t)cx << 16; out_xy[2 * m + 1] = (int64_t)cy << 16; m++;
    }
    return m;
}

extern "C" int vlfm_fog_params_host(const int32_t* h_agent_px, const double* h_angle_cv2_deg, const double* h_rot_cs,
                                    double fov_deg, double max_line_len, const int32_t* h_env,
                                    const int32_t* h_explore, int n, vlfm_fog_params* h_out) {
    if (!h_agent_px || !h_angle_cv2_deg || !h_rot_cs || !h_out || n < 0)
        return vlfm::fail(VLFM_ERR_INVALID, "fog_params_host: bad argument");
    for (int k = 0; k < n; k++) {
        vlfm_fog_params& p = h_out[k];
        std::memset(&p, 0, sizeof(p));
        p.env = h_env ? h_env[k] : k;
        p.ax = h_agent_px[2 * k]; p.ay = h_agent_px[2 * k + 1];
        p.radius = (int)max_line_len;
        p.rot_c = h_rot_cs[2 * k]; p.rot_s = h_rot_cs[2 * k + 1];
        p.line_len = max_line_len * 1.05;
        if (h_explore && !h_explore[k]) { p.n_poly = 0; continue; }
        const int m = ellipse_sector_polygon(p.ax, p.ay, p.radius, h_angle_cv2_deg[k] - fov_deg / 2,
                                             h_angle_cv2_deg[k] + fov_deg / 2, (int64_t*)p.poly, VLFM_FOG_MAX_POLY);
        if (m < 0) return vlfm::fail(m, "fog_params_host: sector polygon does not fit VLFM_FOG_MAX_POLY");
        p.n_poly = m;
    }
    return VLFM_OK;
}

extern "C" int vlfm_circle_polygon_host(const int32_t* h_circles, int n, int64_t* h_xy, int32_t* h_off, int capacity) {
    if (!h_circles || !h_xy || !h_off || n < 0 || capacity < 0)
        return vlfm::fail(VLFM_ERR_INVALID, "circle_polygon_host: bad argument");
    int total = 0;
    h_off[0] = 0;
    for (int k = 0; k < n; k++) {
        const int cx = h_circles[3 * k], cy = h_circles[3 * k + 1], r = h_circles[3 * k + 2];
        if (r < 0) return vlfm::fail(VLFM_ERR_INVALID, "circle_polygon_host: negative radius");
        const int m = ellipse_sector_polygon(cx, cy, r, 0.0, 360.0, h_xy + 2 * (size_t)total, capacity - total);
        if (m < 0) return vlfm::fail(m, "circle_polygon_host: vertex capacity");
        if (m == 1) {
            if (total + 2 > capacity) return vlfm::fail(VLFM_ERR_CAPACITY, "circle_polygon_host: vertex capacity");
            for (int i = 0; i < 2; i++) {
                h_xy[2 * (size_t)(total + i)] = (int64_t)cx << 16;
                h_xy[2 * (size_t)(total + i) + 1] = (int64_t)cy << 16;
            }
            total += 2;
        } else {
            total += m;
        }
        h_off[k + 1] = total;
    }
    return total;
}

extern "C" int vlfm_cone_template_host(double fov, double max_depth, int pixels_per_meter, double min_confidence,
                                       float* h_conf, int conf_capacity, int64_t* h_poly_xy, int poly_capacity,
                                       int* n_poly) {
    if (!h_conf || !h_poly_xy || !n_poly || pixels_per_meter <= 0)
        return vlfm::fail(VLFM_ERR_INVALID, "cone_template_host: bad argument");
    const int size = (int)(max_depth * pixels_per_meter);
    const int T = 2 * size + 1;
    if (size <= 0) return vlfm::fail(VLFM_ERR_INVALID, "cone_template_host: empty template");
    if ((long)T * T > conf_capacity) return vlfm::fail(VLFM_ERR_CAPACITY, "cone_template_host: conf capacity");
    const int mid = T / 2;
    for (int r = 0; r < T; r++) {
        const double fwd = std::abs(r - mid);
        for (int c = 0; c < T; c++) {
            const double lat = std::abs(c - mid);
            double ang = std::atan2(lat, fwd);
            ang = (ang - 0) * (kPi / 2 - 0) / (fov / 2 - 0) + 0;
            double cf = std::pow(std::cos(ang), 2.0);
            cf = (cf - 0) * (1 - min_confidence) / (1 - 0) + min_confidence;
            h_conf[(size_t)r * T + c] = (float)cf;
        }
    }
    const double deg = fov * (180.0 / kPi);
    const int m = ellipse_sector_polygon(size, size, size, -deg / 2 + 90, deg / 2 + 90, h_poly_xy, poly_capacity);
    if (m < 0) return vlfm::fail(m, "cone_template_host: polygon capacity");
    *n_poly = m;
    return T;
}

extern "C" int vlfm_tan_table_host(double fov, int width, double* h_out) {
    if (!h_out || width <= 0) return vlfm::fail(VLFM_ERR_INVALID, "tan_table_host: bad argument");
    const double start = -fov / 2, stop = fov / 2;
    const int div = width - 1;
    const double step = div > 0 ? (stop - start) / div : 0.0;
    for (int i = 0; i < width; i++) {
        double a = (double)i * step + start;
        if (i == width - 1 && width > 1) a = stop;
        h_out[i] = std::tan(a);
    }
    return VLFM_OK;
}

extern "C" int vlfm_disc_rows_host(int radius, int32_t* h_halfwidth) {
    if (!h_halfwidth || radius < 0) return vlfm::fail(VLFM_ERR_INVALID, "disc_rows_host: bad argument");
    for (int i = 0; i <= 2 * radius; i++) h_halfwidth[i] = -1;
    int err = 0, dx = radius, dy = 0, plus = 1, minus = (radius << 1) - 1;
    while (dx >= dy) {
        auto widen = [&](int row_off, int hw) {
            int32_t& slot = h_halfwidth[radius + row_off];
            if (hw > slot) slot = hw;
        };
        widen(-dy, dx); widen(dy, dx); widen(-dx, dy); widen(dx, dy);
        dy++;
        err += plus;
        plus += 2;
        const int mask = (err <= 0) - 1;
        err -= minus & mask;
        dx += mask;
        minus -= 2 & mask;
    }
    return VLFM_OK;
}

#include <hip/hip_runtime.h>

#include <map>
#include <vector>

#include "profile.h"

namespace vlfm {
namespace {
struct KernelLog { std::vector<std::pair<hipEvent_t, hipEvent_t>> spans; long launches = 0; };
std::mutex g_prof_mu;
int g_prof_every = 0;
std::map<std::string, KernelLog> g_prof;
const size_t kMaxSpans = 8192;
}

static thread_local ProfileScope* g_scope = nullptr;
ProfileScope* current_profile_scope() { return g_scope; }

ProfileScope::ProfileScope(const char* name, hipStream_t stream) : name_(name), stream_(stream) {
    prev_ = g_scope;
    g_scope = this;
    if (!g_prof_every) return;
    if (g_prof_every > 1) {
        std::lock_guard<std::mutex> lk(g_prof_mu);
        if (g_prof[name_].launches++ % g_prof_every != 0) return;
    }
    if (hipEventCreate(&start_) != hipSuccess || hipEventCreate(&stop_) != hipSuccess) return;
    active_ = true;
}
ProfileScope::~ProfileScope() {
    g_scope = prev_;
    if (!active_) return;
    if (!used_) { (void)hipEventDestroy(start_); (void)hipEventDestroy(stop_); return; }
    std::lock_guard<std::mutex> lk(g_prof_mu);
    KernelLog& log = g_prof[name_];
    if (log.spans.size() < kMaxSpans) log.spans.emplace_back(start_, stop_);
    else { (void)hipEventDestroy(start_); (void)hipEventDestroy(stop_); }
}
}

extern "C" int vlfm_host_wait_mode(int blocking) {
    hipError_t e = hipSetDeviceFlags(blocking ? hipDeviceScheduleBlockingSync : hipDeviceScheduleAuto);
    if (e != hipSuccess) {
        (void)hipGetLastError();
        vlfm::set_last_error((std::string("hipSetDeviceFlags: ") + hipGetErrorString(e)).c_str());
        return VLFM_ERR_HIP;
    }
    return VLFM_OK;
}

extern "C" int vlfm_profile_enable(int on) {
    std::lock_guard<std::mutex> lk(vlfm::g_prof_mu);
    for (auto& kv : vlfm::g_prof)
        for (auto& sp : kv.second.spans) { (void)hipEventDestroy(sp.first); (void)hipEventDestroy(sp.second); }
    vlfm::g_prof.clear();
    vlfm::g_prof_every = on > 0 ? on : 0;
    return VLFM_OK;
}

extern "C" int vlfm_profile_read(const char* kernel_name, double* mean_ms, int* launches) {
    if (!kernel_name || !mean_ms || !launches) return vlfm::fail(VLFM_ERR_INVALID, "profile_read: bad argument");
    std::lock_guard<std::mutex> lk(vlfm::g_prof_mu);
    auto it = vlfm::g_prof.find(kernel_name);
    *mean_ms = 0.0; *launches = 0;
    if (it == vlfm::g_prof.end()) return VLFM_OK;
    double total = 0.0; int n = 0;
    for (auto& sp : it->second.spans) {
        if (hipEventSynchronize(sp.second) != hipSuccess) continue;
        float ms = 0.f;
        if (hipEventElapsedTime(&ms, sp.first, sp.second) == hipSuccess) { total += ms; n++; }
    }
    *launches = n;
    *mean_ms = n ? total / n : 0.0;
    return VLFM_OK;
}
```

### vlfm_amd/csrc/vlm_ops.hip

```cpp
#include <hip/hip_fp16.h>
#include <hip/hip_bf16.h>
#include <hip/hip_runtime.h>
#include <stdint.h>

#include <cmath>
#include <cstdlib>
#include <vector>

#include "../../include/vlfm_amd.h"
#include "profile.h"
#include "status.h"

namespace vlfm {

constexpr int PRECISION_BITS = 32 - 8 - 2;

__device__ inline unsigned char clip8(int v) {
    v >>= PRECISION_BITS;
    return (unsigned char)(v < 0 ? 0 : v > 255 ? 255 : v);
}

__global__ __launch_bounds__(256) void resample_h_kernel(const unsigned char* __restrict__ src, int H, int W, int O,
                                                         const int* __restrict__ bounds, const int* __restrict__ kk,
                                                         int ksize, unsigned char* __restrict__ dst) {
    extern __shared__ __attribute__((aligned(16))) unsigned char smem[];
    const int y = blockIdx.x, n = blockIdx.y;
    const unsigned char* row = src + ((size_t)n * H + y) * W * 3;
    const int row_bytes = W * 3;
    if ((row_bytes & 15) == 0 && ((size_t)row & 15) == 0) {
        for (int i = threadIdx.x; i < row_bytes / 16; i += blockDim.x)
            reinterpret_cast<uint4*>(smem)[i] = reinterpret_cast<const uint4*>(row)[i];
    } else {
        for (int i = threadIdx.x; i < row_bytes; i += blockDim.x) smem[i] = row[i];
    }
    __syncthreads();
    unsigned char* out = dst + ((size_t)n * H + y) * O * 3;
    for (int o = threadIdx.x; o < O * 3; o += blockDim.x) {
        const int xx = o / 3, c = o - xx * 3;
        const int xmin = bounds[2 * xx], cnt = bounds[2 * xx + 1];
        const int* k = kk + xx * ksize;
        int ss = 1 << (PRECISION_BITS - 1);
        for (int x = 0; x < cnt; x++) ss += (int)smem[(xmin + x) * 3 + c] * k[x];
        out[o] = clip8(ss);
    }
}

template <typename OutT>
__device__ inline OutT cast_out(float v);
template <> __device__ inline float cast_out<float>(float v) { return v; }
template <> __device__ inline __half cast_out<__half>(float v) { return __float2half_rn(v); }
template <> __device__ inline __hip_bfloat16 cast_out<__hip_bfloat16>(float v) { return __float2bfloat16(v); }

struct Norm3 { float mean[3]; float std[3]; };

template <typename OutT>
__global__ __launch_bounds__(256) void resample_v_norm_kernel(const unsigned char* __restrict__ src, int H, int O,
                                                              const int* __restrict__ bounds,
                                                              const int* __restrict__ kk, int ksize, Norm3 nrm,
                                                              OutT* __restrict__ dst, int patch) {
    const int yy = blockIdx.x, n = blockIdx.y;
    const int ymin = bounds[2 * yy], cnt = bounds[2 * yy + 1];
    const int* k = kk + yy * ksize;
    const unsigned char* img = src + (size_t)n * H * O * 3;
    for (int o = threadIdx.x; o < 3 * O; o += blockDim.x) {
        const int c = o / O, xx = o - c * O;
        int ss = 1 << (PRECISION_BITS - 1);
        for (int y = 0; y < cnt; y++) ss += (int)img[((size_t)(ymin + y) * O + xx) * 3 + c] * k[y];
        const float px = (float)clip8(ss);
        const float v = __fdiv_rn(__fsub_rn(__fdiv_rn(px, 255.0f), nrm.mean[c]), nrm.std[c]);
        if (patch == 0) {
            dst[(((size_t)n * 3 + c) * O + yy) * O + xx] = cast_out<OutT>(v);
        } else {
            const int g = O / patch, py = yy / patch, px_ = xx / patch;
            const size_t cell = ((size_t)n * g * g + (size_t)py * g + px_) * (3 * patch * patch);
            dst[cell + (size_t)c * patch * patch + (yy - py * patch) * patch + (xx - px_ * patch)] = cast_out<OutT>(v);
        }
    }
}

constexpr int PF_THREADS = 768;
constexpr int PF_GROUPS = PF_THREADS / 256;
constexpr int PF_VGROUP = 192;
constexpr int PF_ROW_BYTES = 4096 + 128;

template <typename OutT> struct alignas(2 * sizeof(OutT)) Pair { OutT a, b; };

template <int KS, typename OutT>
__global__ __launch_bounds__(PF_THREADS) void preprocess_fused_kernel(const unsigned char* __restrict__ src, int H, int W, int O, int R,
                                                                      int TR, const int* __restrict__ hbounds,
                                                                      const int* __restrict__ hk, int hksize,
                                                                      const int* __restrict__ vbounds,
                                                                      const int* __restrict__ vk, int vksize, Norm3 nrm,
                                                                      OutT* __restrict__ dst, int patch) {
    extern __shared__ __attribute__((aligned(16))) unsigned char smem[];
    const int OP = (O + 3) & ~3;
    float* lut = reinterpret_cast<float*>(smem);
    unsigned char* rowbuf = smem + 3 * 256 * 4;
    unsigned char* tmp = rowbuf + 2 * PF_GROUPS * PF_ROW_BYTES;
    const int tid = threadIdx.x, n = blockIdx.y;
    const int yy0 = blockIdx.x * R, yy1 = min(O, yy0 + R);
    const int r0 = vbounds[2 * yy0], r1 = vbounds[2 * (yy1 - 1)] + vbounds[2 * (yy1 - 1) + 1];
    if (r1 - r0 > TR) __builtin_trap();
    {
        const int c = tid >> 8, v = tid & 255;
        lut[tid] = __fdiv_rn(__fsub_rn(__fdiv_rn((float)v, 255.0f), nrm.mean[c]), nrm.std[c]);
    }
    const int g = tid >> 8, xx = tid & 255;
    const bool live = xx < O;
    int k[KS];
    int d0 = 0, b0 = 0;
    if (live) {
        const int xmin = hbounds[2 * xx];
        d0 = (xmin * 3) >> 2;
        b0 = (xmin * 3) & 3;
    }
#pragma unroll
    for (int x = 0; x < KS; x++) k[x] = (live && x < hksize) ? hk[xx * hksize + x] : 0;
    const int row_bytes = W * 3;
    const unsigned char* img = src + (size_t)n * H * row_bytes;
    const int steps = (r1 - r0 + PF_GROUPS - 1) / PF_GROUPS;
    const bool loader = xx * 16 < row_bytes;
    uint4 pre = make_uint4(0u, 0u, 0u, 0u);
    if (loader && r0 + g < r1) pre = *reinterpret_cast<const uint4*>(img + (size_t)(r0 + g) * row_bytes + xx * 16);
    if (loader) *reinterpret_cast<uint4*>(rowbuf + (size_t)g * PF_ROW_BYTES + xx * 16) = pre;
    for (int st = 0; st < steps; st++) {
        const int r = r0 + st * PF_GROUPS + g, rn = r + PF_GROUPS;
        if (loader && rn < r1) pre = *reinterpret_cast<const uint4*>(img + (size_t)rn * row_bytes + xx * 16);
        __syncthreads();
        if (live && r < r1) {
            const unsigned* rowdw = reinterpret_cast<const unsigned*>(rowbuf + (size_t)((st & 1) * PF_GROUPS + g) * PF_ROW_BYTES);
            constexpr int NA = (3 * KS + 3) / 4;
            unsigned w[NA + 1], a[NA];
#pragma unroll
            for (int i = 0; i <= NA; i++) w[i] = rowdw[d0 + i];
#pragma unroll
            for (int i = 0; i < NA; i++) a[i] = __builtin_amdgcn_alignbyte(w[i + 1], w[i], (unsigned)b0);
            int s0 = 1 << (PRECISION_BITS - 1), s1 = s0, s2 = s0;
#pragma unroll
            for (int x = 0; x < KS; x++) {
                const int j = 3 * x;
                s0 = __mul24((int)((a[j >> 2] >> (8 * (j & 3))) & 0xFFu), k[x]) + s0;
                s1 = __mul24((int)((a[(j + 1) >> 2] >> (8 * ((j + 1) & 3))) & 0xFFu), k[x]) + s1;
                s2 = __mul24((int)((a[(j + 2) >> 2] >> (8 * ((j + 2) & 3))) & 0xFFu), k[x]) + s2;
            }
            unsigned char* t = tmp + (size_t)(r - r0) * OP + xx;
            t[0] = clip8(s0);
            t[(size_t)TR * OP] = clip8(s1);
            t[(size_t)2 * TR * OP] = clip8(s2);
        }
        if (loader) *reinterpret_cast<uint4*>(rowbuf + (size_t)(((st + 1) & 1) * PF_GROUPS + g) * PF_ROW_BYTES + xx * 16) = pre;
    }
    __syncthreads();
    const int vg = tid / PF_VGROUP, vt = tid - vg * PF_VGROUP;
    const int opd = OP >> 2;
    const bool vlive = vt < 3 * opd;
    const bool pair_ok = (O & 1) == 0 && (patch & 1) == 0;
    const int c = vlive ? vt / opd : 0, dc = vt - c * opd, x4 = 4 * dc;
    const int cell = 3 * patch * patch, gp = patch ? O / patch : 0;
    int coloff[4];
#pragma unroll
    for (int i = 0; i < 4; i++) {
        const int x = x4 + i;
        coloff[i] = patch ? (x / patch) * cell + (x % patch) : x;
    }
    const int chan_off = c * (patch ? patch * patch : O * O);
    const unsigned* col0 = reinterpret_cast<const unsigned*>(tmp) + (size_t)c * TR * opd + dc;
    const float* lut_c = lut + c * 256;
    for (int yy = yy0 + vg; yy < yy1; yy += PF_THREADS / PF_VGROUP) {
        const int yu = __builtin_amdgcn_readfirstlane(yy);
        const int ymin = vbounds[2 * yu], cnt = vbounds[2 * yu + 1];
        const int* kv = vk + (size_t)yu * vksize;
        size_t row_off;
        if (patch == 0) {
            row_off = ((size_t)n * 3 * O + yu) * O;
        } else {
            const int py = yu / patch;
            row_off = ((size_t)n * gp * gp + (size_t)py * gp) * cell + (size_t)(yu - py * patch) * patch;
        }
        if (!vlive) continue;
        const unsigned* col = col0 + (size_t)(ymin - r0) * opd;
        int s[4];
#pragma unroll
        for (int i = 0; i < 4; i++) s[i] = 1 << (PRECISION_BITS - 1);
        for (int y = 0; y < cnt; y++) {
            const unsigned wv = col[(size_t)y * opd];
            const int kq = kv[y];
            s[0] = __mul24((int)(wv & 0xFFu), kq) + s[0];
            s[1] = __mul24((int)((wv >> 8) & 0xFFu), kq) + s[1];
            s[2] = __mul24((int)((wv >> 16) & 0xFFu), kq) + s[2];
            s[3] = __mul24((int)(wv >> 24), kq) + s[3];
        }
        OutT v[4];
#pragma unroll
        for (int i = 0; i < 4; i++) v[i] = cast_out<OutT>(lut_c[clip8(s[i])]);
        OutT* o = dst + row_off + chan_off;
        if (pair_ok && x4 + 3 < O) {
            *reinterpret_cast<Pair<OutT>*>(o + coloff[0]) = Pair<OutT>{v[0], v[1]};
            *reinterpret_cast<Pair<OutT>*>(o + coloff[2]) = Pair<OutT>{v[2], v[3]};
        } else {
#pragma unroll
            for (int i = 0; i < 4; i++)
                if (x4 + i < O) o[coloff[i]] = v[i];
        }
    }
}

__global__ __launch_bounds__(256) void resample_v_sam_kernel(const unsigned char* __restrict__ src, int H, int OH, int OW,
                                                             int P, const int* __restrict__ bounds,
                                                             const int* __restrict__ kk, int ksize, Norm3 nrm,
                                                             float* __restrict__ dst) {
    const int yy = blockIdx.x, n = blockIdx.y;
    const unsigned char* img = src + (size_t)n * H * OW * 3;
    const bool row_in = yy < OH;
    const int ymin = row_in ? bounds[2 * yy] : 0, cnt = row_in ? bounds[2 * yy + 1] : 0;
    const int* k = kk + (size_t)(row_in ? yy : 0) * ksize;
    for (int o = threadIdx.x; o < 3 * P; o += blockDim.x) {
        const int c = o / P, xx = o - c * P;
        float v = 0.0f;
        if (row_in && xx < OW) {
            int ss = 1 << (PRECISION_BITS - 1);
            for (int y = 0; y < cnt; y++) ss += (int)img[((size_t)(ymin + y) * OW + xx) * 3 + c] * k[y];
            v = __fdiv_rn(__fsub_rn((float)clip8(ss), nrm.mean[c]), nrm.std[c]);
        }
        dst[(((size_t)n * 3 + c) * P + yy) * P + xx] = v;
    }
}

constexpr int LN_MAXV = 4;
constexpr int LN_ROWS = 8;

struct alignas(16) Half8 { __half2 h[4]; };

template <int NV>
__global__ __launch_bounds__(256) void layernorm_bias_f16_kernel(const __half* __restrict__ x, const float* __restrict__ cb,
                                                                 const __half* __restrict__ gamma,
                                                                 const __half* __restrict__ beta, __half* __restrict__ y,
                                                                 int rows, int D, float eps, int rows_per_wave) {
    const int lane = threadIdx.x & 63, wave = (blockIdx.x * blockDim.x + threadIdx.x) >> 6;
    const int nvec = D >> 3;
    const int r0 = wave * rows_per_wave;
    if (r0 >= rows) return;
    Half8 gm[NV], bt[NV];
    float4 c0[NV], c1[NV];
#pragma unroll
    for (int i = 0; i < NV; i++) {
        const int v = lane + 64 * i;
        if (v < nvec) {
            gm[i] = reinterpret_cast<const Half8*>(gamma)[v];
            bt[i] = reinterpret_cast<const Half8*>(beta)[v];
            c0[i] = cb ? reinterpret_cast<const float4*>(cb)[2 * v] : make_float4(0.f, 0.f, 0.f, 0.f);
            c1[i] = cb ? reinterpret_cast<const float4*>(cb)[2 * v + 1] : make_float4(0.f, 0.f, 0.f, 0.f);
        }
    }
    Half8 cur[NV], nxt[NV], nx2[NV];
    auto load_row = [&](int r, Half8* dst) {
#pragma unroll
        for (int i = 0; i < NV; i++) {
            const int v = lane + 64 * i;
            if (v < nvec) dst[i] = reinterpret_cast<const Half8*>(x + (size_t)r * D)[v];
        }
    };
    auto val = [&](const Half8* row, int i, int j) -> float {
        const float2 t = __half22float2(row[i].h[j >> 1]);
        const float cc = j < 4 ? (&c0[i].x)[j] : (&c1[i].x)[j - 4];
        return ((j & 1) ? t.y : t.x) + cc;
    };
    const int r_end = min(rows, r0 + rows_per_wave);
    load_row(r0, cur);
    if (r0 + 1 < r_end) load_row(r0 + 1, nxt);
    const float inv_d = 1.0f / (float)D;
    for (int r = r0; r < r_end; r++) {
        if (r + 2 < r_end) load_row(r + 2, nx2);
        float sum = 0.0f;
#pragma unroll
        for (int i = 0; i < NV; i++) {
            if (lane + 64 * i < nvec) {
#pragma unroll
                for (int j = 0; j < 8; j++) sum += val(cur, i, j);
            }
        }
#pragma unroll
        for (int off = 32; off > 0; off >>= 1) sum += __shfl_xor(sum, off, 64);
        const float mean = sum * inv_d;
        float sq = 0.0f;
#pragma unroll
        for (int i = 0; i < NV; i++) {
            if (lane + 64 * i < nvec) {
#pragma unroll
                for (int j = 0; j < 8; j++) {
                    const float dlt = val(cur, i, j) - mean;
                    sq = fmaf(dlt, dlt, sq);
                }
            }
        }
#pragma unroll
        for (int off = 32; off > 0; off >>= 1) sq += __shfl_xor(sq, off, 64);
        const float rstd = rsqrtf(sq * inv_d + eps);
#pragma unroll
        for (int i = 0; i < NV; i++) {
            const int v = lane + 64 * i;
            if (v < nvec) {
                Half8 o;
#pragma unroll
                for (int j = 0; j < 4; j++) {
                    const float2 g2 = __half22float2(gm[i].h[j]), b2 = __half22float2(bt[i].h[j]);
                    o.h[j] = __floats2half2_rn((val(cur, i, 2 * j) - mean) * rstd * g2.x + b2.x,
                                               (val(cur, i, 2 * j + 1) - mean) * rstd * g2.y + b2.y);
                }
                reinterpret_cast<Half8*>(y + (size_t)r * D)[v] = o;
            }
        }
#pragma unroll
        for (int i = 0; i < NV; i++) { cur[i] = nxt[i]; nxt[i] = nx2[i]; }
    }
}

__global__ __launch_bounds__(512) void itc_head_kernel(const float* __restrict__ proj, int NQ, int P,
                                                       const float* __restrict__ text, float* __restrict__ out) {
    __shared__ float cos_q[64];
    const int b = blockIdx.x, lane = threadIdx.x & 63, wave = threadIdx.x >> 6, n_waves = blockDim.x >> 6;
    const float* t = text + (size_t)b * P;
    for (int q = wave; q < NQ; q += n_waves) {
        const float* p = proj + ((size_t)b * NQ + q) * P;
        float n2 = 0.0f, dt = 0.0f;
        for (int j = lane; j < P; j += 64) {
            const float v = p[j];
            n2 = fmaf(v, v, n2);
            dt = fmaf(v, t[j], dt);
        }
        for (int off = 32; off > 0; off >>= 1) {
            n2 += __shfl_down(n2, off, 64);
            dt += __shfl_down(dt, off, 64);
        }
        if (lane == 0) cos_q[q] = dt / fmaxf(sqrtf(n2), 1e-12f);
    }
    __syncthreads();
    if (wave == 0) {
        float c = lane < NQ ? cos_q[lane] : -__builtin_huge_valf();
        for (int off = 32; off > 0; off >>= 1) c = fmaxf(c, __shfl_down(c, off, 64));
        if (lane == 0) out[b] = c;
    }
}

template <int T>
__global__ __launch_bounds__(512) void itc_head_multi_kernel(const float* __restrict__ proj, int NQ, int P,
                                                             const float* __restrict__ text, int U,
                                                             const int* __restrict__ idx, float* __restrict__ out) {
    __shared__ float cos_q[T][64];
    const int b = blockIdx.x, lane = threadIdx.x & 63, wave = threadIdx.x >> 6, n_waves = blockDim.x >> 6;
    const float* tp[T];
    unsigned ok = 0;
#pragma unroll
    for (int t = 0; t < T; t++) {
        const int u = idx[(size_t)b * T + t];
        const bool in = u >= 0 && u < U;
        ok |= (unsigned)in << t;
        tp[t] = text + (size_t)(in ? u : 0) * P;
    }
    for (int q = wave; q < NQ; q += n_waves) {
        const float* p = proj + ((size_t)b * NQ + q) * P;
        float n2 = 0.0f, dt[T];
#pragma unroll
        for (int t = 0; t < T; t++) dt[t] = 0.0f;
        for (int j = lane; j < P; j += 64) {
            const float v = p[j];
            n2 = fmaf(v, v, n2);
#pragma unroll
            for (int t = 0; t < T; t++) dt[t] = fmaf(v, tp[t][j], dt[t]);
        }
        for (int off = 32; off > 0; off >>= 1) {
            n2 += __shfl_down(n2, off, 64);
#pragma unroll
            for (int t = 0; t < T; t++) dt[t] += __shfl_down(dt[t], off, 64);
        }
        if (lane == 0) {
            const float nrm = fmaxf(sqrtf(n2), 1e-12f);
#pragma unroll
            for (int t = 0; t < T; t++) cos_q[t][q] = dt[t] / nrm;
        }
    }
    __syncthreads();
    if (wave < T) {
        float c = lane < NQ ? cos_q[wave][lane] : -__builtin_huge_valf();
        for (int off = 32; off > 0; off >>= 1) c = fmaxf(c, __shfl_down(c, off, 64));
        if (lane == 0) out[(size_t)b * T + wave] = (ok >> wave) & 1u ? c : __builtin_nanf("");
    }
}

}

using namespace vlfm;

extern "C" int vlfm_resample_coeffs_filter_host(int in_size, int out_size, int filter, int32_t* h_bounds, int32_t* h_kk,
                                                int kk_capacity, int* ksize_out) {
    if (in_size <= 0 || out_size <= 0 || !h_bounds || !h_kk || !ksize_out || (filter != 0 && filter != 1))
        return fail(VLFM_ERR_INVALID, "resample_coeffs_host: bad argument (filter 0 = bicubic, 1 = bilinear)");
    auto bicubic = [filter](double x) {
        if (x < 0.0) x = -x;
        if (filter == 1) return x < 1.0 ? 1.0 - x : 0.0;
        const double a = -0.5;
        if (x < 1.0) return ((a + 2.0) * x - (a + 3.0)) * x * x + 1;
        if (x < 2.0) return (((x - 5) * x + 8) * x - 4) * a;
        return 0.0;
    };
    const float in0 = 0.0f, in1 = (float)in_size;
    double scale = (double)(in1 - in0) / out_size, filterscale = scale;
    if (filterscale < 1.0) filterscale = 1.0;
    const double support = (filter == 1 ? 1.0 : 2.0) * filterscale;
    const int ksize = (int)std::ceil(support) * 2 + 1;
    *ksize_out = ksize;
    if ((long)out_size * ksize > kk_capacity) return fail(VLFM_ERR_CAPACITY, "resample_coeffs_host: kk capacity");
    std::vector<double> k(ksize);
    for (int xx = 0; xx < out_size; xx++) {
        const double center = in0 + (xx + 0.5) * scale;
        double ww = 0.0;
        const double ss = 1.0 / filterscale;
        int xmin = (int)(center - support + 0.5);
        if (xmin < 0) xmin = 0;
        int xmax = (int)(center + support + 0.5);
        if (xmax > in_size) xmax = in_size;
        xmax -= xmin;
        for (int x = 0; x < xmax; x++) {
            const double w = bicubic((x + xmin - center + 0.5) * ss);
            k[x] = w;
            ww += w;
        }
        for (int x = 0; x < xmax; x++)
            if (ww != 0.0) k[x] /= ww;
        for (int x = xmax; x < ksize; x++) k[x] = 0;
        h_bounds[2 * xx] = xmin;
        h_bounds[2 * xx + 1] = xmax;
        for (int x = 0; x < ksize; x++) {
            const double v = k[x];
            h_kk[(size_t)xx * ksize + x] = v < 0 ? (int)(-0.5 + v * (1 << PRECISION_BITS)) : (int)(0.5 + v * (1 << PRECISION_BITS));
        }
    }
    return VLFM_OK;
}

extern "C" int vlfm_resample_coeffs_host(int in_size, int out_size, int32_t* h_bounds, int32_t* h_kk, int kk_capacity,
                                         int* ksize_out) {
    return vlfm_resample_coeffs_filter_host(in_size, out_size, 0, h_bounds, h_kk, kk_capacity, ksize_out);
}

extern "C" int vlfm_preprocess_sam_batched(const uint8_t* d_rgb, int n, int height, int width, int out_h, int out_w,
                                           const int32_t* d_hbounds, const int32_t* d_hk, int hksize,
                                           const int32_t* d_vbounds, const int32_t* d_vk, int vksize,
                                           const float* h_mean3, const float* h_std3, int pad_size, uint8_t* d_tmp,
                                           float* d_out, void* stream) {
    if (n == 0) return VLFM_OK;
    if (!d_rgb || !d_hbounds || !d_hk || !d_vbounds || !d_vk || !h_mean3 || !h_std3 || !d_tmp || !d_out || n < 0 ||
        height <= 0 || width <= 0 || out_h <= 0 || out_w <= 0 || pad_size < out_h || pad_size < out_w)
        return fail(VLFM_ERR_INVALID, "preprocess_sam_batched: bad argument");
    hipStream_t s = (hipStream_t)stream;
    const size_t lds = ((size_t)width * 3 + 15) / 16 * 16;
    {
        VLFM_TIMED("resample_h_kernel", s);
        VLFM_KLAUNCH(resample_h_kernel, dim3(height, n), dim3(256), lds, s, d_rgb, height, width, out_w, d_hbounds, d_hk,
                     hksize, d_tmp);
    }
    int rc = check_launch("resample_h_kernel");
    if (rc != VLFM_OK) return rc;
    Norm3 nrm;
    for (int c = 0; c < 3; c++) { nrm.mean[c] = h_mean3[c]; nrm.std[c] = h_std3[c]; }
    VLFM_TIMED("resample_v_sam_kernel", s);
    VLFM_KLAUNCH(resample_v_sam_kernel, dim3(pad_size, n), dim3(256), 0, s, d_tmp, height, out_h, out_w, pad_size,
                 d_vbounds, d_vk, vksize, nrm, d_out);
    return check_launch("resample_v_sam_kernel");
}

extern "C" int vlfm_preprocess_rgb_batched(const uint8_t* d_rgb, int n, int height, int width, int out_size,
                                           const int32_t* d_hbounds, const int32_t* d_hk, int hksize,
                                           const int32_t* d_vbounds, const int32_t* d_vk, int vksize,
                                           const float* h_mean3, const float* h_std3, uint8_t* d_tmp, void* d_out,
                                           int out_dtype, int patch_size, void* stream) {
    if (n == 0) return VLFM_OK;
    if (!d_rgb || !d_hbounds || !d_hk || !d_vbounds || !d_vk || !h_mean3 || !h_std3 || !d_tmp || !d_out || n < 0 ||
        height <= 0 || width <= 0 || out_size <= 0 || patch_size < 0 || (patch_size > 0 && out_size % patch_size != 0))
        return fail(VLFM_ERR_INVALID, "preprocess_rgb_batched: bad argument");
    hipStream_t s = (hipStream_t)stream;
    Norm3 nrm;
    for (int c = 0; c < 3; c++) { nrm.mean[c] = h_mean3[c]; nrm.std[c] = h_std3[c]; }
    if (out_dtype < 0 || out_dtype > 2)
        return fail(VLFM_ERR_INVALID, "preprocess_rgb_batched: out_dtype must be 0 (f32), 1 (f16) or 2 (bf16)");
    const int row_bytes = width * 3;
    if (row_bytes % 16 == 0 && row_bytes <= 4096 && ((uintptr_t)d_rgb & 15) == 0 && hksize <= 32 && out_size <= 256 &&
        !getenv("VLFM_PREPROCESS_TWO_PASS")) {
        const int OP = (out_size + 3) & ~3;
        auto span = [&](int R) { return (int)(((long)(R - 1) * height + out_size - 1) / out_size) + vksize + 2; };
        auto lds_of = [&](int R) { return (size_t)3 * 256 * 4 + (size_t)2 * PF_GROUPS * PF_ROW_BYTES + (size_t)3 * span(R) * OP; };
        int R = out_size < 32 ? out_size : 32;
        while (R > 1 && lds_of(R) > 80 * 1024) R--;
        while (R > 8 && (long)((out_size + R - 1) / R) * n < 512) R = (R + 1) / 2;
        const int bands = (out_size + R - 1) / R;
        R = (out_size + bands - 1) / bands;
        const size_t lds = lds_of(R);
        const int TR = span(R);
        const dim3 grid(bands, n), block(PF_THREADS);
        VLFM_TIMED("preprocess_fused_kernel", s);
#define VLFM_PF_LAUNCH(KS, T)                                                                                          \
    do {                                                                                                               \
        static LdsOptIn opt;                                                                                           \
        if (!opt.ensure(reinterpret_cast<const void*>(preprocess_fused_kernel<KS, T>), 80 * 1024))                     \
            return fail(VLFM_ERR_HIP, "preprocess_rgb_batched: cannot opt in to 80 KB of LDS");                        \
        VLFM_KLAUNCH((preprocess_fused_kernel<KS, T>), grid, block, lds, s, d_rgb, height, width, out_size, R, TR,     \
                     d_hbounds, d_hk, hksize, d_vbounds, d_vk, vksize, nrm, (T*)d_out, patch_size);                    \
    } while (0)
#define VLFM_PF_DTYPE(KS)                                                                                              \
    do {                                                                                                               \
        if (out_dtype == 0) VLFM_PF_LAUNCH(KS, float);                                                                 \
        else if (out_dtype == 1) VLFM_PF_LAUNCH(KS, __half);                                                           \
        else VLFM_PF_LAUNCH(KS, __hip_bfloat16);                                                                       \
    } while (0)
        if (hksize <= 8) VLFM_PF_DTYPE(8);
        else if (hksize <= 13) VLFM_PF_DTYPE(13);
        else if (hksize <= 16) VLFM_PF_DTYPE(16);
        else if (hksize <= 25) VLFM_PF_DTYPE(25);
        else VLFM_PF_DTYPE(32);
#undef VLFM_PF_DTYPE
#undef VLFM_PF_LAUNCH
        return check_launch("preprocess_fused_kernel");
    }
    const size_t lds = ((size_t)width * 3 + 15) / 16 * 16;
    {
        VLFM_TIMED("resample_h_kernel", s);
    VLFM_KLAUNCH(resample_h_kernel, dim3(height, n), dim3(256), lds, s, d_rgb, height, width, out_size,
                       d_hbounds, d_hk, hksize, d_tmp);
    }
    int rc = check_launch("resample_h_kernel");
    if (rc != VLFM_OK) return rc;
    VLFM_TIMED("resample_v_norm_kernel", s);
    if (out_dtype == 0)
        VLFM_KLAUNCH(resample_v_norm_kernel<float>, dim3(out_size, n), dim3(256), 0, s, d_tmp, height, out_size,
                           d_vbounds, d_vk, vksize, nrm, (float*)d_out, patch_size);
    else if (out_dtype == 1)
        VLFM_KLAUNCH(resample_v_norm_kernel<__half>, dim3(out_size, n), dim3(256), 0, s, d_tmp, height,
                           out_size, d_vbounds, d_vk, vksize, nrm, (__half*)d_out, patch_size);
    else
        VLFM_KLAUNCH(resample_v_norm_kernel<__hip_bfloat16>, dim3(out_size, n), dim3(256), 0, s, d_tmp, height,
                           out_size, d_vbounds, d_vk, vksize, nrm, (__hip_bfloat16*)d_out, patch_size);
    return check_launch("resample_v_norm_kernel");
}

extern "C" int vlfm_itc_head_batched(const float* d_proj, int batch, int n_query, int proj_dim, const float* d_text,
                                     float* d_out, void* stream) {
    if (batch == 0) return VLFM_OK;
    if (!d_proj || !d_text || !d_out || batch < 0 || n_query <= 0 || n_query > 64 || proj_dim <= 0)
        return fail(VLFM_ERR_INVALID, "itc_head_batched: bad argument (n_query <= 64)");
    VLFM_TIMED("itc_head_kernel", stream);
    VLFM_KLAUNCH(itc_head_kernel, dim3(batch), dim3(512), 0, (hipStream_t)stream, d_proj, n_query, proj_dim,
                       d_text, d_out);
    return check_launch("itc_head_kernel");
}

extern "C" int vlfm_itc_head_multi(const float* d_proj, int batch, int n_query, int proj_dim, const float* d_text_table,
                                   int n_text, const int32_t* d_text_index, int n_prompts, float* d_out, void* stream) {
    if (!d_proj || !d_text_table || !d_text_index || !d_out || batch < 0 || n_query <= 0 || n_query > 64 || proj_dim <= 0 ||
        n_text < 1 || n_prompts < 1 || n_prompts > VLFM_ITC_MAX_PROMPTS)
        return fail(VLFM_ERR_INVALID, "itc_head_multi: bad argument (n_query <= 64, 1 <= n_prompts <= 8, n_text >= 1)");
    if (batch == 0) return VLFM_OK;
    VLFM_TIMED("itc_head_multi_kernel", stream);
#define VLFM_ITC_MULTI(T)                                                                                              \
    case T:                                                                                                            \
        VLFM_KLAUNCH(itc_head_multi_kernel<T>, dim3(batch), dim3(512), 0, (hipStream_t)stream, d_proj, n_query,        \
                     proj_dim, d_text_table, n_text, d_text_index, d_out);                                             \
        break
    switch (n_prompts) {
        VLFM_ITC_MULTI(1); VLFM_ITC_MULTI(2); VLFM_ITC_MULTI(3); VLFM_ITC_MULTI(4);
        VLFM_ITC_MULTI(5); VLFM_ITC_MULTI(6); VLFM_ITC_MULTI(7); VLFM_ITC_MULTI(8);
    }
#undef VLFM_ITC_MULTI
    return check_launch("itc_head_multi_kernel");
}

extern "C" int vlfm_layernorm_bias_f16(const void* d_x, const float* d_channel_bias, const void* d_gamma, const void* d_beta,
                                       void* d_y, int rows, int dim, float eps, void* stream) {
    if (rows == 0) return VLFM_OK;
    if (!d_x || !d_gamma || !d_beta || !d_y || rows < 0 || dim <= 0 || dim % 8 != 0 || dim > 64 * 8 * LN_MAXV)
        return fail(VLFM_ERR_INVALID, "layernorm_bias_f16: dim must be a multiple of 8 and <= 2048");
    const int nvec = dim / 8, nv = (nvec + 63) / 64;
    int rpw = rows / 8192;
    rpw = rpw < 1 ? 1 : rpw > LN_ROWS ? LN_ROWS : rpw;
    const int waves = (rows + rpw - 1) / rpw;
    const dim3 grid((waves + 3) / 4), block(256);
    const __half* x = (const __half*)d_x; const __half* g = (const __half*)d_gamma; const __half* b = (const __half*)d_beta;
    __half* y = (__half*)d_y;
    VLFM_TIMED("layernorm_bias_f16_kernel", stream);
    switch (nv) {
        case 1: VLFM_KLAUNCH(layernorm_bias_f16_kernel<1>, grid, block, 0, (hipStream_t)stream, x, d_channel_bias, g, b, y, rows, dim, eps, rpw); break;
        case 2: VLFM_KLAUNCH(layernorm_bias_f16_kernel<2>, grid, block, 0, (hipStream_t)stream, x, d_channel_bias, g, b, y, rows, dim, eps, rpw); break;
        case 3: VLFM_KLAUNCH(layernorm_bias_f16_kernel<3>, grid, block, 0, (hipStream_t)stream, x, d_channel_bias, g, b, y, rows, dim, eps, rpw); break;
        default: VLFM_KLAUNCH(layernorm_bias_f16_kernel<4>, grid, block, 0, (hipStream_t)stream, x, d_channel_bias, g, b, y, rows, dim, eps, rpw); break;
    }
    return check_launch("layernorm_bias_f16_kernel");
}
```

### vlfm_amd/vlm/blip2itm.py

```python
from __future__ import annotations

import hashlib
import math
import os
import re
from dataclasses import dataclass
from typing import Dict, List, Optional, Sequence, Tuple

import numpy as np
import torch
import torch.nn as nn
import torch.nn.functional as F


@dataclass
class Blip2ITCConfig:
    image_size: int = 224
    patch_size: int = 14
    v_hidden: int = 1408
    v_layers: int = 39
    v_heads: int = 16
    v_mlp: int = 6144
    v_ln_eps: float = 1e-6
    q_hidden: int = 768
    q_layers: int = 12
    q_heads: int = 12
    q_mlp: int = 3072
    q_ln_eps: float = 1e-12
    cross_attention_frequency: int = 2
    vocab_size: int = 30523
    max_position_embeddings: int = 512
    num_query_tokens: int = 32
    proj_dim: int = 256
    max_txt_len: int = 32

    @staticmethod
    def tiny() -> "Blip2ITCConfig":
        return Blip2ITCConfig(image_size=28, patch_size=14, v_hidden=32, v_layers=2, v_heads=4, v_mlp=64,
                              q_hidden=24, q_layers=4, q_heads=4, q_mlp=48, vocab_size=97,
                              max_position_embeddings=40, num_query_tokens=5, proj_dim=8)


DEFAULT_HIP_GEMMS = ("fc1",)


def x_is_contiguous_f16(t: torch.Tensor) -> bool:
    return t.dtype == torch.float16 and t.is_contiguous()


class _VitBlock(nn.Module):
    def __init__(self, c: Blip2ITCConfig):
        super().__init__()
        self.heads = c.v_heads
        self.layer_norm1 = nn.LayerNorm(c.v_hidden, eps=c.v_ln_eps)
        self.qkv = nn.Linear(c.v_hidden, 3 * c.v_hidden, bias=True)
        self.projection = nn.Linear(c.v_hidden, c.v_hidden)
        self.layer_norm2 = nn.LayerNorm(c.v_hidden, eps=c.v_ln_eps)
        self.fc1 = nn.Linear(c.v_hidden, c.v_mlp)
        self.fc2 = nn.Linear(c.v_mlp, c.v_hidden)

        self._packed = None
        self.hip_attention = True
        self.strict_hip_attention = True
        self.hip_mlp_min_rows = 32 * 257
        self.hip_gemms = frozenset(DEFAULT_HIP_GEMMS)

    def pack_heads(self, multiple: int = 32) -> None:
        h, d = self.heads, self.qkv.in_features
        hd = d // h
        hp = (hd + multiple - 1) // multiple * multiple
        if hp == hd:
            self._packed = None
            return
        w = self.qkv.weight.detach().view(3, h, hd, d)
        bq = self.qkv.bias.detach().view(3, h, hd)
        wq = torch.zeros((3, h, hp, d), dtype=w.dtype, device=w.device)
        bb = torch.zeros((3, h, hp), dtype=w.dtype, device=w.device)
        wq[:, :, :hd] = w
        bb[:, :, :hd] = bq
        pw = self.projection.weight.detach().view(d, h, hd)
        wp = torch.zeros((d, h, hp), dtype=pw.dtype, device=pw.device)
        wp[:, :, :hd] = pw
        self._packed = (wq.view(3 * h * hp, d).contiguous(), bb.view(-1).contiguous(), wp.view(d, h * hp).contiguous(),
                        hp, float(hd) ** -0.5)

    def hip_gemms_at(self, rows: int) -> frozenset:
        from . import ops

        if not (self.hip_mlp_min_rows and rows >= self.hip_mlp_min_rows):
            return frozenset()
        layers = {"qkv": self.qkv, "proj": self.projection, "fc1": self.fc1, "fc2": self.fc2}

        def ok(lin: nn.Linear) -> bool:
            w, b = lin.weight, lin.bias
            return (x_is_contiguous_f16(w) and w.shape[1] % 64 == 0 and w.shape[0] % 8 == 0 and w.numel() * 2 < (1 << 32)
                    and rows * max(w.shape) * 2 < (1 << 32) and (b is None or x_is_contiguous_f16(b)))

        return frozenset(n for n in self.hip_gemms if ok(layers[n]))

    def forward_deferred(self, x: torch.Tensor, c_in: torch.Tensor, c_mid: torch.Tensor) -> torch.Tensor:
        from . import ops

        b, n, d = x.shape
        hd = d // self.heads
        hip = self.hip_gemms_at(b * n)
        h = ops.layernorm_bias(x, c_in, self.layer_norm1.weight, self.layer_norm1.bias, self.layer_norm1.eps)
        x2 = x.view(b * n, d)
        a = None
        if self.hip_attention and n == ops.VIT_ATTENTION_TOKENS and hd in ops.VIT_ATTENTION_HEADS:
            if "qkv" in hip:
                qkv = ops.linear_f16(h.view(b * n, d), self.qkv.weight, self.qkv.bias, "bias")
            else:
                qkv = F.linear(h.view(b * n, d), self.qkv.weight, self.qkv.bias)
            try:
                a = ops.vit_attention(qkv, b, n, self.heads, hd, float(hd) ** -0.5)
            except (RuntimeError, AssertionError, IndexError) as exc:
                if self.strict_hip_attention:
                    raise
                import warnings

                warnings.warn(f"vlfm_vit_attention_f16 unavailable ({exc}); using the library attention kernel instead")
                self.hip_attention = False
        if a is not None:
            if "proj" in hip and x2.is_contiguous():
                ops.linear_f16(a, self.projection.weight, None, "accumulate", out=x2)
            else:
                x2.addmm_(a, self.projection.weight.t())
        elif self._packed is not None:
            wq, bq, wp, hp, scale = self._packed
            q = F.linear(h.view(b * n, d), wq, bq).view(b, n, 3, self.heads, hp).permute(2, 0, 3, 1, 4)
            a = F.scaled_dot_product_attention(q[0], q[1], q[2], scale=scale).transpose(1, 2).reshape(b * n, self.heads * hp)
            x2.addmm_(a, wp.t())
        else:
            q = self.qkv(h).view(b, n, 3, self.heads, hd).permute(2, 0, 3, 1, 4)
            a = F.scaled_dot_product_attention(q[0], q[1], q[2]).transpose(1, 2).reshape(b * n, d)
            x2.addmm_(a, self.projection.weight.t())
        h = ops.layernorm_bias(x, c_mid, self.layer_norm2.weight, self.layer_norm2.bias, self.layer_norm2.eps)
        if "fc1" in hip:
            act = ops.linear_gelu(h.view(b * n, d), self.fc1.weight, self.fc1.bias)
        else:
            act = F.gelu(F.linear(h, self.fc1.weight, self.fc1.bias)).view(b * n, -1)
        if "fc2" in hip and x2.is_contiguous():
            ops.linear_f16(act, self.fc2.weight, None, "accumulate", out=x2)
        else:
            x2.addmm_(act, self.fc2.weight.t())
        return x

    def forward(self, x: torch.Tensor) -> torch.Tensor:
        b, n, d = x.shape
        if self._packed is not None and self._packed[0].dtype == x.dtype:
            wq, bq, wp, hp, scale = self._packed
            qkv = F.linear(self.layer_norm1(x), wq, bq).view(b, n, 3, self.heads, hp).permute(2, 0, 3, 1, 4)
            a = F.scaled_dot_product_attention(qkv[0], qkv[1], qkv[2], scale=scale)
            x = x + F.linear(a.transpose(1, 2).reshape(b, n, self.heads * hp), wp, self.projection.bias)
        else:
            qkv = self.qkv(self.layer_norm1(x)).view(b, n, 3, self.heads, d // self.heads).permute(2, 0, 3, 1, 4)
            a = F.scaled_dot_product_attention(qkv[0], qkv[1], qkv[2])
            x = x + self.projection(a.transpose(1, 2).reshape(b, n, d))
        return x + self.fc2(F.gelu(self.fc1(self.layer_norm2(x))))


def _exact_split3(w: torch.Tensor) -> Tuple[torch.Tensor, torch.Tensor, torch.Tensor]:
    w = w.detach().float()
    w1 = w.half()
    r = (w - w1.float()) * 2048.0
    w2 = r.half()
    return w1, w2, ((r - w2.float()) * 2048.0).half()


KV_SPLIT_PIECES = 2


def _split_gemm(x16: torch.Tensor, pieces, bias: torch.Tensor, n_pieces: Optional[int] = None) -> torch.Tensor:
    w1t, w2t, w3t = pieces
    if (KV_SPLIT_PIECES if n_pieces is None else n_pieces) >= 3:
        o = torch.addmm(bias, x16, w3t, alpha=2.0 ** -22, out_dtype=torch.float32)
        torch.addmm(o, x16, w2t, alpha=2.0 ** -11, out_dtype=torch.float32, out=o)
    else:
        o = torch.addmm(bias, x16, w2t, alpha=2.0 ** -11, out_dtype=torch.float32)
    torch.addmm(o, x16, w1t, out_dtype=torch.float32, out=o)
    return o


QFORMER_SPLIT_MIN_ROWS = 2048


def _qlinear(x: torch.Tensor, lin_w: torch.Tensor, lin_b, act=None, residual=None) -> torch.Tensor:
    from . import ops

    if (x.is_cuda and x.dtype == torch.float32 and lin_w.dtype == torch.float32 and not torch.is_grad_enabled()
            and x.numel() // x.shape[-1] >= QFORMER_SPLIT_MIN_ROWS and ops.linear_f32_supported(x, lin_w)):
        return ops.linear_f32(x, lin_w, lin_b, act=act, residual=residual, precision="split", owner="blip2")
    y = F.linear(x, lin_w, lin_b)
    if act == "gelu":
        y = F.gelu(y)
    return y if residual is None else y + residual


class _BertAttention(nn.Module):
    def __init__(self, hidden: int, kv_hidden: int, heads: int, eps: float):
        super().__init__()
        self.heads = heads
        self.query = nn.Linear(hidden, hidden)
        self.key = nn.Linear(kv_hidden, hidden)
        self.value = nn.Linear(kv_hidden, hidden)
        self.dense = nn.Linear(hidden, hidden)
        self.LayerNorm = nn.LayerNorm(hidden, eps=eps)
        self._kv_split = None
        self._qkv_fused = None

    def _project_kv_f16(self, kv16: torch.Tensor) -> Tuple[torch.Tensor, torch.Tensor]:
        if self._kv_split is None or self._kv_split[0].device != kv16.device:
            w1, w2, w3 = _exact_split3(torch.cat([self.key.weight, self.value.weight]))
            bias = torch.cat([self.key.bias, self.value.bias]).detach().float()
            self._kv_split = (w1.t(), w2.t(), w3.t(), bias)
        o = _split_gemm(kv16.reshape(-1, kv16.shape[-1]), self._kv_split[:3], self._kv_split[3])
        o = o.view(*kv16.shape[:-1], -1)
        hid = self.key.out_features
        return o[..., :hid], o[..., hid:]

    def forward(self, x: torch.Tensor, kv: Optional[torch.Tensor] = None, mask: Optional[torch.Tensor] = None,
                kv_proj: Optional[Tuple[torch.Tensor, torch.Tensor]] = None, kv_blocks=None) -> torch.Tensor:
        b, n, d = x.shape
        h = self.heads
        if kv_blocks is not None:
            from . import ops

            blocks, tokens, k_block0, v_block0 = kv_blocks
            q = _qlinear(x, self.query.weight, self.query.bias).contiguous()
            a = ops.qformer_cross_attention(q, blocks, tokens, h, k_block0, v_block0, (d // h) ** -0.5)
            return self.LayerNorm(_qlinear(a, self.dense.weight, self.dense.bias, residual=x))
        if kv_proj is not None:
            q = _qlinear(x, self.query.weight, self.query.bias).view(b, n, h, d // h).transpose(1, 2)
            k = kv_proj[0].reshape(b, -1, h, d // h).transpose(1, 2)
            v = kv_proj[1].reshape(b, -1, h, d // h).transpose(1, 2)
        elif kv is None and x.is_cuda and not self.training:
            if self._qkv_fused is None or self._qkv_fused[0].device != x.device or self._qkv_fused[0].dtype != x.dtype:
                self._qkv_fused = (torch.cat([self.query.weight, self.key.weight, self.value.weight]).detach(),
                                   torch.cat([self.query.bias, self.key.bias, self.value.bias]).detach())
            qkv = _qlinear(x, *self._qkv_fused).view(b, n, 3, h, d // h).permute(2, 0, 3, 1, 4)
            q, k, v = qkv[0], qkv[1], qkv[2]
        else:
            q = self.query(x).view(b, n, h, d // h).transpose(1, 2)
            if kv is not None and kv.dtype == torch.float16 and kv.is_cuda and self.key.weight.dtype == torch.float32:
                k, v = self._project_kv_f16(kv)
                src_len = kv.shape[1]
            else:
                src = x if kv is None else kv.to(x.dtype)
                k, v, src_len = self.key(src), self.value(src), src.shape[1]
            k = k.reshape(b, src_len, h, d // h).transpose(1, 2)
            v = v.reshape(b, src_len, h, d // h).transpose(1, 2)
        a = F.scaled_dot_product_attention(q, k, v, attn_mask=mask)
        return self.LayerNorm(_qlinear(a.transpose(1, 2).reshape(b, n, d), self.dense.weight, self.dense.bias,
                                       residual=x))


class _BertFFN(nn.Module):
    def __init__(self, hidden: int, inter: int, eps: float):
        super().__init__()
        self.up = nn.Linear(hidden, inter)
        self.down = nn.Linear(inter, hidden)
        self.LayerNorm = nn.LayerNorm(hidden, eps=eps)

    def forward(self, x: torch.Tensor) -> torch.Tensor:
        hid = _qlinear(x, self.up.weight, self.up.bias, act="gelu")
        return self.LayerNorm(_qlinear(hid, self.down.weight, self.down.bias, residual=x))


class _QFormerLayer(nn.Module):
    def __init__(self, c: Blip2ITCConfig, idx: int):
        super().__init__()
        self.attention = _BertAttention(c.q_hidden, c.q_hidden, c.q_heads, c.q_ln_eps)
        self.crossattention = (_BertAttention(c.q_hidden, c.v_hidden, c.q_heads, c.q_ln_eps)
                               if idx % c.cross_attention_frequency == 0 else None)
        self.ffn_text = _BertFFN(c.q_hidden, c.q_mlp, c.q_ln_eps)
        self.ffn_query = _BertFFN(c.q_hidden, c.q_mlp, c.q_ln_eps)


class Blip2ITCModel(nn.Module):

    def __init__(self, cfg: Blip2ITCConfig):
        super().__init__()
        c = self.cfg = cfg
        n_patches = (c.image_size // c.patch_size) ** 2
        self.class_embedding = nn.Parameter(torch.zeros(1, 1, c.v_hidden))
        self.position_embedding = nn.Parameter(torch.zeros(1, n_patches + 1, c.v_hidden))
        self.patch_embedding = nn.Conv2d(3, c.v_hidden, c.patch_size, c.patch_size)
        self.blocks = nn.ModuleList([_VitBlock(c) for _ in range(c.v_layers)])
        self.post_layernorm = nn.LayerNorm(c.v_hidden, eps=c.v_ln_eps)
        self.query_tokens = nn.Parameter(torch.zeros(1, c.num_query_tokens, c.q_hidden))
        self.word_embeddings = nn.Embedding(c.vocab_size, c.q_hidden)
        self.position_embeddings = nn.Embedding(c.max_position_embeddings, c.q_hidden)
        self.q_layernorm = nn.LayerNorm(c.q_hidden, eps=c.q_ln_eps)
        self.q_layers = nn.ModuleList([_QFormerLayer(c, i) for i in range(c.q_layers)])
        self.vision_projection = nn.Linear(c.q_hidden, c.proj_dim)
        self.text_projection = nn.Linear(c.q_hidden, c.proj_dim)
        self.deferred_bias = True
        self._deferred_c: Optional[torch.Tensor] = None
        self.split_kv = True
        self.split_kv_min_rows = 32 * 257
        self._kv_all = None
        self.fused_cross_kv = True
        self._kv_pair = None

    def init_random(self, seed: int = 0) -> "Blip2ITCModel":
        dev = self.query_tokens.device
        g = torch.Generator(device=dev).manual_seed(seed)
        with torch.no_grad():
            for p in self.parameters():
                if p.dim() > 1:
                    p.copy_(torch.randn(p.shape, generator=g, device=dev) * 0.02)
                else:
                    p.zero_()
            for m in self.modules():
                if isinstance(m, nn.LayerNorm):
                    m.weight.fill_(1.0)
        self.weights_changed()
        return self

    def weights_changed(self) -> None:
        self._deferred_c = None
        self._kv_all = None
        self._kv_pair = None
        for layer in self.q_layers:
            layer.attention._qkv_fused = None
            if layer.crossattention is not None:
                layer.crossattention._kv_split = None

    def vision_dtype(self) -> torch.dtype:
        return self.patch_embedding.weight.dtype

    def set_precision(self, vision_dtype: torch.dtype = torch.float16) -> "Blip2ITCModel":
        for m in (self.patch_embedding, self.blocks, self.post_layernorm):
            m.to(vision_dtype)
        self.class_embedding.data = self.class_embedding.data.to(vision_dtype)
        self.position_embedding.data = self.position_embedding.data.to(vision_dtype)
        self.weights_changed()
        return self

    def load_hf_state_dict(self, sd: Dict[str, torch.Tensor]) -> None:
        own = dict(self.named_parameters())

        def put(name: str, src: str) -> None:
            with torch.no_grad():
                own[name].copy_(sd[src].to(own[name].dtype).reshape(own[name].shape))

        put("class_embedding", "vision_model.embeddings.class_embedding")
        put("position_embedding", "vision_model.embeddings.position_embedding")
        put("patch_embedding.weight", "vision_model.embeddings.patch_embedding.weight")
        put("patch_embedding.bias", "vision_model.embeddings.patch_embedding.bias")
        for i in range(self.cfg.v_layers):
            s, d = f"vision_model.encoder.layers.{i}.", f"blocks.{i}."
            for a, b in [("layer_norm1", "layer_norm1"), ("layer_norm2", "layer_norm2"),
                         ("self_attn.qkv", "qkv"), ("self_attn.projection", "projection"),
                         ("mlp.fc1", "fc1"), ("mlp.fc2", "fc2")]:
                put(d + b + ".weight", s + a + ".weight")
                put(d + b + ".bias", s + a + ".bias")
        put("post_layernorm.weight", "vision_model.post_layernorm.weight")
        put("post_layernorm.bias", "vision_model.post_layernorm.bias")
        put("query_tokens", "query_tokens")
        put("word_embeddings.weight", "embeddings.word_embeddings.weight")
        put("position_embeddings.weight", "embeddings.position_embeddings.weight")
        put("q_layernorm.weight", "qformer.layernorm.weight")
        put("q_layernorm.bias", "qformer.layernorm.bias")
        for i, layer in enumerate(self.q_layers):
            s, d = f"qformer.encoder.layer.{i}.", f"q_layers.{i}."
            atts = [("attention", "attention")] + ([("crossattention", "crossattention")]
                                                   if layer.crossattention is not None else [])
            for a, b in atts:
                for hf, mine in [("attention.query", "query"), ("attention.key", "key"), ("attention.value", "value"),
                                 ("output.dense", "dense"), ("output.LayerNorm", "LayerNorm")]:
                    put(f"{d}{b}.{mine}.weight", f"{s}{a}.{hf}.weight")
                    put(f"{d}{b}.{mine}.bias", f"{s}{a}.{hf}.bias")
            for hf_i, hf_o, mine in [("intermediate", "output", "ffn_text"),
                                     ("intermediate_query", "output_query", "ffn_query")]:
                put(f"{d}{mine}.up.weight", f"{s}{hf_i}.dense.weight")
                put(f"{d}{mine}.up.bias", f"{s}{hf_i}.dense.bias")
                put(f"{d}{mine}.down.weight", f"{s}{hf_o}.dense.weight")
                put(f"{d}{mine}.down.bias", f"{s}{hf_o}.dense.bias")
                put(f"{d}{mine}.LayerNorm.weight", f"{s}{hf_o}.LayerNorm.weight")
                put(f"{d}{mine}.LayerNorm.bias", f"{s}{hf_o}.LayerNorm.bias")
        for n in ("vision_projection", "text_projection"):
            put(n + ".weight", n + ".weight")
            put(n + ".bias", n + ".bias")

    def load_lavis_state_dict(self, sd: Dict[str, torch.Tensor], vit_sd: Optional[Dict[str, torch.Tensor]] = None) -> None:
        c = self.cfg
        sd = {(k[len("module."):] if k.startswith("module.") else k): v for k, v in sd.items()}
        vit = {("visual_encoder." + k): v for k, v in (vit_sd or {}).items()}
        overlap = set(vit) & set(sd)
        if overlap:
            raise KeyError(f"the vision tower is given twice (e.g. {sorted(overlap)[:2]})")
        src = {**sd, **vit}
        own = dict(self.named_parameters())
        used, fed = set(), set()

        def take(key: str) -> torch.Tensor:
            if key not in src:
                raise KeyError(f"LAVIS state dict lacks {key}" + ("" if vit_sd is not None or not key.startswith("visual_encoder.")
                                                                 else " (blip2_pretrained.pth does not carry the frozen ViT: "
                                                                      "pass eva_vit_g.pth as the vision checkpoint)"))
            used.add(key)
            return src[key]

        def put(name: str, value: torch.Tensor) -> None:
            if tuple(value.shape) != tuple(own[name].shape) and value.numel() != own[name].numel():
                raise ValueError(f"{name}: {tuple(own[name].shape)} in the graph, {tuple(value.shape)} in the file")
            with torch.no_grad():
                own[name].copy_(value.to(own[name].dtype).reshape(own[name].shape))
            fed.add(name)

        put("class_embedding", take("visual_encoder.cls_token"))
        put("position_embedding", take("visual_encoder.pos_embed"))
        put("patch_embedding.weight", take("visual_encoder.patch_embed.proj.weight"))
        put("patch_embedding.bias", take("visual_encoder.patch_embed.proj.bias"))
        for i in range(c.v_layers):
            o, d = f"visual_encoder.blocks.{i}.", f"blocks.{i}."
            for a, b in (("norm1", "layer_norm1"), ("norm2", "layer_norm2"), ("attn.proj", "projection"),
                         ("mlp.fc1", "fc1"), ("mlp.fc2", "fc2")):
                put(d + b + ".weight", take(o + a + ".weight"))
                put(d + b + ".bias", take(o + a + ".bias"))
            put(d + "qkv.weight", take(o + "attn.qkv.weight"))
            qb, vb = take(o + "attn.q_bias"), take(o + "attn.v_bias")
            put(d + "qkv.bias", torch.cat([qb, torch.zeros_like(vb), vb]))
        put("post_layernorm.weight", take("ln_vision.weight"))
        put("post_layernorm.bias", take("ln_vision.bias"))
        put("query_tokens", take("query_tokens"))
        put("word_embeddings.weight", take("Qformer.bert.embeddings.word_embeddings.weight"))
        put("position_embeddings.weight", take("Qformer.bert.embeddings.position_embeddings.weight"))
        put("q_layernorm.weight", take("Qformer.bert.embeddings.LayerNorm.weight"))
        put("q_layernorm.bias", take("Qformer.bert.embeddings.LayerNorm.bias"))
        for i, layer in enumerate(self.q_layers):
            o, d = f"Qformer.bert.encoder.layer.{i}.", f"q_layers.{i}."
            for att in ["attention"] + (["crossattention"] if layer.crossattention is not None else []):
                for theirs, mine in (("self.query", "query"), ("self.key", "key"), ("self.value", "value"),
                                     ("output.dense", "dense"), ("output.LayerNorm", "LayerNorm")):
                    put(f"{d}{att}.{mine}.weight", take(f"{o}{att}.{theirs}.weight"))
                    put(f"{d}{att}.{mine}.bias", take(f"{o}{att}.{theirs}.bias"))
            for t_i, t_o, mine in (("intermediate", "output", "ffn_text"), ("intermediate_query", "output_query", "ffn_query")):
                put(f"{d}{mine}.up.weight", take(f"{o}{t_i}.dense.weight"))
                put(f"{d}{mine}.up.bias", take(f"{o}{t_i}.dense.bias"))
                put(f"{d}{mine}.down.weight", take(f"{o}{t_o}.dense.weight"))
                put(f"{d}{mine}.down.bias", take(f"{o}{t_o}.dense.bias"))
                put(f"{d}{mine}.LayerNorm.weight", take(f"{o}{t_o}.LayerNorm.weight"))
                put(f"{d}{mine}.LayerNorm.bias", take(f"{o}{t_o}.LayerNorm.bias"))
        put("vision_projection.weight", take("vision_proj.weight"))
        put("vision_projection.bias", take("vision_proj.bias"))
        put("text_projection.weight", take("text_proj.weight"))
        put("text_projection.bias", take("text_proj.bias"))
        unfed = sorted(set(own) - fed)
        if unfed:
            raise KeyError(f"{len(unfed)} parameters of the graph were not fed, e.g. {unfed[:4]}")

        def unused_ok(k: str) -> bool:
            return (k.startswith(("Qformer.cls.", "itm_head.")) or k in ("temp", "Qformer.bert.embeddings.position_ids")
                    or k.startswith(f"visual_encoder.blocks.{c.v_layers}.")
                    or k.startswith(("visual_encoder.norm.", "visual_encoder.fc_norm.", "visual_encoder.head.")))

        left = sorted(k for k in src if k not in used and not unused_ok(k))
        if left:
            raise KeyError(f"{len(left)} tensors of the file have no place in the ITC graph, e.g. {left[:4]}")
        self.weights_changed()

    def vision_tokens(self, pixel_values: torch.Tensor) -> torch.Tensor:
        c = self.cfg
        if pixel_values.dim() == 4:
            b, g = pixel_values.shape[0], c.image_size // c.patch_size
            pixel_values = pixel_values.reshape(b, 3, g, c.patch_size, g, c.patch_size).permute(0, 2, 4, 1, 3, 5) \
                .reshape(b, g * g, 3 * c.patch_size * c.patch_size)
        w = self.patch_embedding.weight
        x = F.linear(pixel_values.to(w.dtype), w.view(w.shape[0], -1), self.patch_embedding.bias)
        x = torch.cat([self.class_embedding.expand(x.shape[0], -1, -1), x], dim=1) + self.position_embedding
        if self.deferred_bias and x.is_cuda and x.dtype == torch.float16 and c.v_hidden % 8 == 0 and c.v_hidden <= 2048:
            from . import ops

            c = self._deferred_constants()
            x = x.contiguous()
            for i, blk in enumerate(self.blocks):
                x = blk.forward_deferred(x, c[2 * i], c[2 * i + 1])
            return ops.layernorm_bias(x, c[2 * len(self.blocks)], self.post_layernorm.weight, self.post_layernorm.bias,
                                      self.post_layernorm.eps)
        for blk in self.blocks:
            x = blk(x)
        return self.post_layernorm(x)

    def _deferred_constants(self) -> torch.Tensor:
        if self._deferred_c is None or self._deferred_c.device != self.post_layernorm.weight.device:
            rows, run = [], torch.zeros(self.cfg.v_hidden, dtype=torch.float32, device=self.post_layernorm.weight.device)
            for blk in self.blocks:
                rows.append(run.clone())
                run = run + blk.projection.bias.detach().float()
                rows.append(run.clone())
                run = run + blk.fc2.bias.detach().float()
            rows.append(run.clone())
            self._deferred_c = torch.stack(rows).contiguous()
        return self._deferred_c

    def query_features(self, image_tokens: torch.Tensor) -> torch.Tensor:
        split_ok = (self.split_kv and image_tokens.dtype == torch.float16 and image_tokens.is_cuda
                    and image_tokens.shape[0] * image_tokens.shape[1] >= self.split_kv_min_rows)
        enc = image_tokens if split_ok else image_tokens.to(self.q_layernorm.weight.dtype)
        h = self.q_layernorm(self.query_tokens).expand(enc.shape[0], -1, -1)
        fused = split_ok and self._fused_cross_ok(enc)
        blocks = self._project_all_kv_blocks(enc) if fused else None
        proj = self._project_all_kv(enc) if split_ok and not fused else None
        hid, at = self.cfg.q_hidden, 0
        for layer in self.q_layers:
            h = layer.attention(h)
            if layer.crossattention is not None:
                if blocks is not None:
                    h = layer.crossattention(h, kv_blocks=(blocks, enc.shape[1], at // 64, (at + hid) // 64))
                    at += 2 * hid
                elif proj is not None:
                    h = layer.crossattention(h, kv_proj=(proj[..., at:at + hid], proj[..., at + hid:at + 2 * hid]))
                    at += 2 * hid
                else:
                    h = layer.crossattention(h, kv=enc)
            h = layer.ffn_query(h)
        return h

    def _fused_cross_ok(self, tokens16: torch.Tensor) -> bool:
        from . import ops

        c = self.cfg
        return (self.fused_cross_kv and KV_SPLIT_PIECES == 2 and not torch.is_grad_enabled()
                and self.q_layernorm.weight.dtype == torch.float32
                and c.q_hidden % c.q_heads == 0 and c.q_hidden // c.q_heads == ops.QFORMER_ATTENTION_HEAD
                and c.num_query_tokens <= ops.QFORMER_ATTENTION_MAX_QUERIES
                and 1 <= tokens16.shape[1] <= ops.QFORMER_ATTENTION_MAX_TOKENS and c.v_hidden % 64 == 0
                and tokens16.shape[0] * tokens16.shape[1] * c.v_hidden * 2 < (1 << 32))

    def _kv_all_pieces(self, device):
        if self._kv_all is None or self._kv_all[0].device != device:
            cross = [l.crossattention for l in self.q_layers if l.crossattention is not None]
            w = torch.cat([torch.cat([c.key.weight, c.value.weight]) for c in cross])
            bias = torch.cat([torch.cat([c.key.bias, c.value.bias]) for c in cross]).detach().float()
            w1, w2, w3 = _exact_split3(w)
            self._kv_all = (w1.t(), w2.t(), w3.t(), bias)
            self._kv_pair = None
        return self._kv_all

    def _project_all_kv_blocks(self, tokens16: torch.Tensor) -> torch.Tensor:
        from . import ops

        w1t, w2t, _, bias = self._kv_all_pieces(tokens16.device)
        if self._kv_pair is None:
            self._kv_pair = (ops.interleave_pair_weights(w1t.t(), w2t.t()), bias.contiguous())
        return ops.linear_pair_f32(tokens16.reshape(-1, tokens16.shape[-1]), *self._kv_pair)

    def _project_all_kv(self, tokens16: torch.Tensor) -> torch.Tensor:
        pieces = self._kv_all_pieces(tokens16.device)
        o = _split_gemm(tokens16.reshape(-1, tokens16.shape[-1]), pieces[:3], pieces[3])
        return o.view(*tokens16.shape[:-1], -1)

    def text_feature(self, input_ids: torch.Tensor, attention_mask: Optional[torch.Tensor] = None) -> torch.Tensor:
        pos = torch.arange(input_ids.shape[1], device=input_ids.device)[None]
        h = self.q_layernorm(self.word_embeddings(input_ids) + self.position_embeddings(pos))
        mask = None
        if attention_mask is not None:
            mask = (attention_mask[:, None, None, :] > 0)
        for layer in self.q_layers:
            h = layer.ffn_text(layer.attention(h, mask=mask))
        return F.normalize(self.text_projection(h[:, 0, :]), dim=-1)

    def itc_reference_head(self, query_feats: torch.Tensor, text_feat: torch.Tensor) -> torch.Tensor:
        img = F.normalize(self.vision_projection(query_feats.float()), dim=-1)
        return torch.einsum("bqd,bd->bq", img, text_feat.float().expand(img.shape[0], -1)).max(dim=1).values


_CAPTION_STRIP = re.compile(r"([.!\"()*#:;~])")


def blip_caption(text: str, max_words: int = 50) -> str:
    t = _CAPTION_STRIP.sub(" ", text.lower())
    t = re.sub(r"\s{2,}", " ", t).rstrip("\n").strip(" ")
    words = t.split(" ")
    return " ".join(words[:max_words]) if len(words) > max_words else t


class HashTokenizer:

    def __init__(self, vocab_size: int, max_len: int):
        self.vocab_size, self.max_len = vocab_size, max_len

    def __call__(self, text: str) -> List[int]:
        ids = [101 % self.vocab_size]
        for w in text.split():
            hv = int.from_bytes(hashlib.sha1(w.encode()).digest()[:4], "little")
            ids.append(1000 % self.vocab_size + hv % max(1, self.vocab_size - 1000))
        ids = ids[: self.max_len - 1] + [102 % self.vocab_size]
        return ids


class BLIP2ITM:

    def __init__(self, name: str = "blip2_image_text_matching", model_type: str = "pretrain", device=None,
                 model_dir: Optional[str] = None, config: Optional[Blip2ITCConfig] = None,
                 vision_dtype: torch.dtype = torch.float16, seed: int = 0, allow_random_init: bool = False,
                 strict_hip_attention: bool = True, checkpoint: Optional[str] = None, vit_checkpoint: Optional[str] = None,
                 tokenizer_dir: Optional[str] = None) -> None:
        from ..mapping.base_map import require_gpu
        from .. import _lib

        self.device = require_gpu(device)
        _lib.lib()
        from . import ops as _ops

        _ops.use_tuned_gemms()
        self.cfg = config or Blip2ITCConfig()
        self.tokenizer = None
        model_dir = model_dir or os.environ.get("BLIP2ITM_MODEL_DIR")
        checkpoint = checkpoint or os.environ.get("BLIP2_LAVIS_CHECKPOINT")
        vit_checkpoint = vit_checkpoint or os.environ.get("EVA_VIT_G_CHECKPOINT")
        if checkpoint and not model_dir:
            for f in (checkpoint, vit_checkpoint):
                if f and not os.path.isfile(f):
                    raise FileNotFoundError(f"BLIP-2 checkpoint {f!r} not found")
            self.model = Blip2ITCModel(self.cfg)
            ck = torch.load(checkpoint, map_location="cpu", weights_only=True)
            vit = torch.load(vit_checkpoint, map_location="cpu", weights_only=True) if vit_checkpoint else None
            self.model.load_lavis_state_dict(ck["model"] if isinstance(ck, dict) and "model" in ck else ck,
                                             vit["model"] if isinstance(vit, dict) and "model" in vit else vit)
            self.tokenizer = self._lavis_tokenizer(tokenizer_dir)
            self.weights = f"lavis:{checkpoint}" + (f" + {vit_checkpoint}" if vit_checkpoint else "")
        elif model_dir:
            self.model = Blip2ITCModel(self.cfg)
            self._load_pretrained(model_dir)
            self.weights = f"pretrained:{model_dir}"
        elif not (allow_random_init or config is not None):
            raise ValueError("BLIP2ITM needs `checkpoint` (+ `vit_checkpoint`): LAVIS' blip2_pretrained.pth and eva_vit_g.pth, what "
                             "the reference loads -- or model_dir / BLIP2ITM_MODEL_DIR (a Salesforce/blip2-itm-vit-g directory); "
                             "pass allow_random_init=True for a randomly initialised network (benchmarks / geometry tests only)")
        else:
            with torch.device(self.device):
                self.model = Blip2ITCModel(self.cfg)
            self.model.init_random(seed)
            self.weights = "random-init"
        if self.tokenizer is None:
            self.tokenizer = HashTokenizer(self.cfg.vocab_size, self.cfg.max_txt_len)
        self.model.eval().to(self.device).set_precision(vision_dtype)
        for blk in self.model.blocks:
            blk.pack_heads()
            blk.strict_hip_attention = bool(strict_hip_attention)
        self._text_cache: Dict[str, torch.Tensor] = {}
        self._prompt_cache: Dict[tuple, tuple] = {}
        self._proj_t = None
        self._graphs, self._prompt_graphs = {}, {}
        self.two_stream_min = None
        self._side_stream = None

    def _lavis_tokenizer(self, tokenizer_dir: Optional[str]):
        from transformers import BertTokenizer

        path = tokenizer_dir or os.environ.get("BLIP2_TOKENIZER")
        try:
            if path:
                vocab = path if os.path.isfile(path) else os.path.join(path, "vocab.txt")
                tok = BertTokenizer(vocab_file=vocab, do_lower_case=True)
            else:
                tok = BertTokenizer.from_pretrained("bert-base-uncased", local_files_only=True)
                if len(tok) < 30522:
                    raise FileNotFoundError("no cached bert-base-uncased vocabulary")
        except Exception as exc:
            raise ValueError("BLIP-2 weights need the bert-base-uncased vocabulary: pass tokenizer_dir (or set BLIP2_TOKENIZER) "
                             "to a directory with its vocab.txt") from exc
        tok.add_special_tokens({"bos_token": "[DEC]"})
        return lambda t: tok(t, truncation=True, max_length=self.cfg.max_txt_len)["input_ids"]

    @property
    def strict_hip_attention(self) -> bool:
        return all(blk.strict_hip_attention for blk in self.model.blocks)

    @strict_hip_attention.setter
    def strict_hip_attention(self, on: bool) -> None:
        for blk in self.model.blocks:
            blk.strict_hip_attention = bool(on)

    @property
    def attention_path(self) -> str:
        flags = {bool(blk.hip_attention) for blk in self.model.blocks}
        return "hip" if flags == {True} else "library" if flags == {False} else "mixed"

    def mlp_path(self, n_images: int) -> str:
        blk = self.model.blocks[0]
        rows = n_images * ((self.cfg.image_size // self.cfg.patch_size) ** 2 + 1)
        return "hip" if "fc1" in blk.hip_gemms_at(rows) else "library"

    def gemm_path(self, n_images: int) -> str:
        blk = self.model.blocks[0]
        rows = n_images * ((self.cfg.image_size // self.cfg.patch_size) ** 2 + 1)
        names = sorted(blk.hip_gemms_at(rows))
        return "hip:" + ",".join(names) if names else "library"

    def _load_pretrained(self, model_dir: str) -> None:
        from safetensors.torch import load_file

        sd: Dict[str, torch.Tensor] = {}
        for f in sorted(os.listdir(model_dir)):
            if f.endswith(".safetensors"):
                sd.update(load_file(os.path.join(model_dir, f)))
        self.model.load_hf_state_dict(sd)
        from transformers import BertTokenizer

        tok = BertTokenizer.from_pretrained(model_dir)
        self.tokenizer = lambda t: tok(t, truncation=True, max_length=self.cfg.max_txt_len)["input_ids"]

    @torch.inference_mode()
    def text_feature(self, txt: str) -> torch.Tensor:
        if txt not in self._text_cache:
            ids = torch.tensor([self.tokenizer(blip_caption(txt))], device=self.device)
            self._text_cache[txt] = self.model.text_feature(ids)[0].float().contiguous()
        return self._text_cache[txt]

    def cosine_batch_graphed(self, images_u8: torch.Tensor, txts: Sequence[str]) -> torch.Tensor:
        return self._replay(self._graphs, (tuple(images_u8.shape), tuple(txts)), lambda x: self.cosine_batch(x, txts), images_u8)

    def _replay(self, graphs: dict, key, forward, images_u8: torch.Tensor, keep_alive=()) -> torch.Tensor:
        if key not in graphs:
            static_in = images_u8.clone()
            for _ in range(2):
                forward(static_in)
            torch.cuda.synchronize(self.device)
            g = torch.cuda.CUDAGraph()
            with torch.cuda.graph(g):
                static_out = forward(static_in)
            graphs[key] = (g, static_in, static_out, keep_alive)
        g, static_in, static_out, _ = graphs[key]
        static_in.copy_(images_u8)
        g.replay()
        return static_out

    def _projection(self):
        if self._proj_t is None:
            self._proj_t = (self.model.vision_projection.weight.float().t().contiguous(),
                            self.model.vision_projection.bias.float().contiguous())
        return self._proj_t

    def _query_feats(self, images_u8: torch.Tensor) -> torch.Tensor:
        from . import ops

        B = images_u8.shape[0]
        pix = ops.preprocess_rgb(images_u8, self.cfg.image_size, self.model.vision_dtype(),
                                 patch_size=self.cfg.patch_size)
        if self.two_stream_min is not None and B >= self.two_stream_min and not torch.cuda.is_current_stream_capturing():
            main = torch.cuda.current_stream(self.device)
            if self._side_stream is None:
                self._side_stream = torch.cuda.Stream(self.device)
            side = self._side_stream
            half = B // 2
            side.wait_stream(main)
            with torch.cuda.stream(side):
                q_hi = self.model.query_features(self.model.vision_tokens(pix[half:])).float()
            q_lo = self.model.query_features(self.model.vision_tokens(pix[:half])).float()
            main.wait_stream(side)
            q = torch.cat([q_lo, q_hi]).contiguous()
        else:
            q = self.model.query_features(self.model.vision_tokens(pix)).float().contiguous()
        return q

    @torch.inference_mode()
    def cosine_batch(self, images_u8: torch.Tensor, txts: Sequence[str]) -> torch.Tensor:
        from . import ops

        B = images_u8.shape[0]
        q = self._query_feats(images_u8)
        if len(txts) == 1:
            text = self.text_feature(txts[0])[None].expand(B, -1).contiguous()
        else:
            assert len(txts) == B
            text = torch.stack([self.text_feature(t) for t in txts]).contiguous()
        return ops.itc_head(q, *self._projection(), text)

    def _prompt_tensors(self, prompts, B: int):
        from . import ops

        key = (B, tuple(prompts) if isinstance(prompts[0], str) else tuple(tuple(p) for p in prompts))
        hit = self._prompt_cache.get(key)
        if hit is None:
            unique, rows = prompt_table(prompts, B)
            table = torch.stack([self.text_feature(t) for t in unique]).contiguous()
            hit = self._prompt_cache[key] = (table, ops.itc_text_index(rows, len(unique), self.device), key)
        return hit

    @torch.inference_mode()
    def cosine_prompts_batch(self, images_u8: torch.Tensor, prompts) -> torch.Tensor:
        from . import ops

        B = images_u8.shape[0]
        q = self._query_feats(images_u8)
        table, index, _ = self._prompt_tensors(prompts, B)
        return ops.itc_head_multi(q, *self._projection(), table, index)

    def cosine_prompts_batch_graphed(self, images_u8: torch.Tensor, prompts) -> torch.Tensor:
        table, index, structure = self._prompt_tensors(prompts, images_u8.shape[0])
        return self._replay(self._prompt_graphs, (tuple(images_u8.shape), structure),
                            lambda x: self.cosine_prompts_batch(x, prompts), images_u8, keep_alive=(table, index))

    def check_numerics(self) -> None:
        from . import ops

        flag = ops.gemm_f32_overflow_flag(self.device, "blip2")
        if int(flag.item()):
            flag.zero_()
            ops.split_weights_bad(self.device, "blip2")
            raise FloatingPointError("BLIP-2 Q-Former: an activation left f16's range inside a split-precision f32 GEMM; set "
                                     "vlfm_amd.vlm.blip2itm.QFORMER_SPLIT_MIN_ROWS = 1 << 60 to run these layers on the library's f32 GEMMs")

    def cosine(self, image: np.ndarray, txt: str) -> float:
        img = torch.from_numpy(np.ascontiguousarray(image)).to(self.device)[None]
        return float(self.cosine_batch(img, [txt])[0].item())

    def cosines(self, image: np.ndarray, prompts: Sequence[str]) -> List[float]:
        img = torch.from_numpy(np.ascontiguousarray(image)).to(self.device)[None]
        return [float(v) for v in self.cosine_prompts_batch(img, list(prompts))[0].tolist()]


def prompt_table(prompts, n_images: int):
    if len(prompts) == 0:
        raise ValueError("at least one prompt is needed")
    per = [list(prompts)] * n_images if isinstance(prompts[0], str) else [list(p) for p in prompts]
    if len(per) != n_images:
        raise ValueError(f"{len(per)} prompt lists for {n_images} images")
    T = len(per[0]) if per else 0
    if any(len(p) != T for p in per) or (per and T == 0):
        raise ValueError("every image needs the same number (>= 1) of prompts")
    unique: Dict[str, int] = {}
    rows = [[unique.setdefault(t, len(unique)) for t in p] for p in per]
    return list(unique), rows


class BLIP2ITMClient:

    _shared: Dict[str, BLIP2ITM] = {}

    def __init__(self, port: int = 12182, device=None, emulate_jpeg: bool = False, **model_kwargs) -> None:
        key = str(device)
        if key not in BLIP2ITMClient._shared:
            BLIP2ITMClient._shared[key] = BLIP2ITM(device=device, **model_kwargs)
        self._model = BLIP2ITMClient._shared[key]
        self._emulate_jpeg = emulate_jpeg
        self.url = f"inprocess://blip2itm (port {port} ignored)"

    def cosine(self, image: np.ndarray, txt: str) -> float:
        if self._emulate_jpeg:
            from .transport import jpeg_roundtrip

            image = jpeg_roundtrip(image)
        return self._model.cosine(image, txt)

    def cosines(self, image: np.ndarray, prompts: Sequence[str]) -> List[float]:
        if self._emulate_jpeg:
            from .transport import jpeg_roundtrip

            image = jpeg_roundtrip(image)
        return self._model.cosines(image, prompts)
```

### vlfm_amd/vlm/ops.py

```python
from __future__ import annotations

import ctypes
from typing import Dict, Optional, Tuple

import numpy as np
import torch

from .. import _lib

CLIP_MEAN = (0.48145466, 0.4578275, 0.40821073)
CLIP_STD = (0.26862954, 0.26130258, 0.27577711)
_DTYPE_CODE = {torch.float32: 0, torch.float16: 1, torch.bfloat16: 2}
_coeff_cache: Dict[Tuple[str, int, int], Tuple[torch.Tensor, torch.Tensor, int]] = {}


def _stream() -> int:
    return torch._C._cuda_getCurrentRawStream(torch._C._cuda_getDevice())


def resample_coeffs(in_size: int, out_size: int, bilinear: bool = False) -> Tuple[np.ndarray, np.ndarray, int]:
    bounds = np.zeros((out_size, 2), np.int32)
    cap = out_size * (2 * int(np.ceil(2.0 * max(1.0, in_size / out_size))) + 1)
    kk = np.zeros(cap, np.int32)
    ks = ctypes.c_int(0)
    _lib.check(_lib.lib().vlfm_resample_coeffs_filter_host(in_size, out_size, int(bilinear), bounds.ctypes.data,
                                                           kk.ctypes.data, cap, ctypes.byref(ks)),
               "resample_coeffs_host")
    return bounds, kk[: out_size * ks.value].reshape(out_size, ks.value), ks.value


def _device_coeffs(device, in_size: int, out_size: int, bilinear: bool = False):
    key = (str(device), in_size, out_size, bilinear)
    if key not in _coeff_cache:
        b, k, ks = resample_coeffs(in_size, out_size, bilinear)
        _coeff_cache[key] = (torch.from_numpy(b).to(device), torch.from_numpy(np.ascontiguousarray(k)).to(device), ks)
    return _coeff_cache[key]


def preprocess_rgb(images_u8: torch.Tensor, out_size: int = 224, dtype: torch.dtype = torch.float16,
                   mean=CLIP_MEAN, std=CLIP_STD, patch_size: int = 0) -> torch.Tensor:
    assert images_u8.is_cuda and images_u8.dtype == torch.uint8 and images_u8.dim() == 4 and images_u8.shape[-1] == 3
    images_u8 = images_u8.contiguous()
    n, H, W, _ = images_u8.shape
    dev = images_u8.device
    hb, hk, hks = _device_coeffs(dev, W, out_size)
    vb, vk, vks = _device_coeffs(dev, H, out_size)
    tmp = torch.empty((n, H, out_size, 3), dtype=torch.uint8, device=dev)
    if patch_size:
        g = out_size // patch_size
        out = torch.empty((n, g * g, 3 * patch_size * patch_size), dtype=dtype, device=dev)
    else:
        out = torch.empty((n, 3, out_size, out_size), dtype=dtype, device=dev)
    m = (ctypes.c_float * 3)(*mean)
    s = (ctypes.c_float * 3)(*std)
    with torch.cuda.device(dev):
        _lib.check(_lib.lib().vlfm_preprocess_rgb_batched(images_u8.data_ptr(), n, H, W, out_size, hb.data_ptr(),
                                                         hk.data_ptr(), hks, vb.data_ptr(), vk.data_ptr(), vks,
                                                         ctypes.addressof(m), ctypes.addressof(s), tmp.data_ptr(),
                                                         out.data_ptr(), _DTYPE_CODE[dtype], int(patch_size), _stream()),
                   "preprocess_rgb")
    return out


def itc_head(query_feats: torch.Tensor, proj_t: torch.Tensor, proj_bias: torch.Tensor,
             text_feats: torch.Tensor) -> torch.Tensor:
    B, NQ, Hd = query_feats.shape
    P = proj_t.shape[1]
    for t in (query_feats, proj_t, proj_bias, text_feats):
        assert t.is_cuda and t.dtype == torch.float32 and t.is_contiguous()
    assert proj_t.shape[0] == Hd and text_feats.shape == (B, P)
    proj = torch.addmm(proj_bias, query_feats.view(B * NQ, Hd), proj_t)
    out = torch.empty(B, dtype=torch.float32, device=query_feats.device)
    with torch.cuda.device(query_feats.device):
        _lib.check(_lib.lib().vlfm_itc_head_batched(proj.data_ptr(), B, NQ, P, text_feats.data_ptr(), out.data_ptr(),
                                                   _stream()), "itc_head")
    return out


ITC_MAX_PROMPTS = 8


def itc_text_index(rows, n_text: int, device) -> torch.Tensor:
    idx = np.asarray(rows, np.int64)
    if idx.ndim != 2 or idx.shape[1] < 1 or idx.shape[1] > ITC_MAX_PROMPTS:
        raise ValueError(f"text index must be [B, T] with 1 <= T <= {ITC_MAX_PROMPTS}, got shape {idx.shape}")
    if n_text < 1 or (idx.size and (idx.min() < 0 or idx.max() >= n_text)):
        raise ValueError(f"text index outside the table of {n_text} row(s)")
    return torch.from_numpy(idx.astype(np.int32)).to(device)


def itc_head_multi(query_feats: torch.Tensor, proj_t: torch.Tensor, proj_bias: torch.Tensor, text_table: torch.Tensor,
                   text_index: torch.Tensor) -> torch.Tensor:
    B, NQ, Hd = query_feats.shape
    P = proj_t.shape[1]
    for t in (query_feats, proj_t, proj_bias, text_table):
        assert t.is_cuda and t.dtype == torch.float32 and t.is_contiguous()
    assert text_index.is_cuda and text_index.dtype == torch.int32 and text_index.is_contiguous()
    assert proj_t.shape[0] == Hd and text_table.dim() == 2 and text_table.shape[1] == P
    assert text_index.dim() == 2 and text_index.shape[0] == B
    U, T = text_table.shape[0], text_index.shape[1]
    proj = torch.addmm(proj_bias, query_feats.view(B * NQ, Hd), proj_t)
    out = torch.empty((B, T), dtype=torch.float32, device=query_feats.device)
    with torch.cuda.device(query_feats.device):
        _lib.check(_lib.lib().vlfm_itc_head_multi(proj.data_ptr(), B, NQ, P, text_table.data_ptr(), U,
                                                 text_index.data_ptr(), T, out.data_ptr(), _stream()), "itc_head_multi")
    return out


SAM_MEAN = (123.675, 116.28, 103.53)
SAM_STD = (58.395, 57.12, 57.375)


def sam_target_size(h: int, w: int, long_side: int = 1024) -> Tuple[int, int]:
    scale = long_side * 1.0 / max(h, w)
    return int(h * scale + 0.5), int(w * scale + 0.5)


def preprocess_sam(images_u8: torch.Tensor, long_side: int = 1024) -> Tuple[torch.Tensor, Tuple[int, int]]:
    assert images_u8.is_cuda and images_u8.dtype == torch.uint8 and images_u8.dim() == 4 and images_u8.shape[-1] == 3
    images_u8 = images_u8.contiguous()
    n, H, W, _ = images_u8.shape
    oh, ow = sam_target_size(H, W, long_side)
    dev = images_u8.device
    hb, hk, hks = _device_coeffs(dev, W, ow, True)
    vb, vk, vks = _device_coeffs(dev, H, oh, True)
    tmp = torch.empty((n, H, ow, 3), dtype=torch.uint8, device=dev)
    out = torch.empty((n, 3, long_side, long_side), dtype=torch.float32, device=dev)
    m, s = (ctypes.c_float * 3)(*SAM_MEAN), (ctypes.c_float * 3)(*SAM_STD)
    with torch.cuda.device(dev):
        _lib.check(_lib.lib().vlfm_preprocess_sam_batched(images_u8.data_ptr(), n, H, W, oh, ow, hb.data_ptr(),
                                                         hk.data_ptr(), hks, vb.data_ptr(), vk.data_ptr(), vks,
                                                         ctypes.addressof(m), ctypes.addressof(s), long_side,
                                                         tmp.data_ptr(), out.data_ptr(), _stream()), "preprocess_sam")
    return out, (oh, ow)


def layernorm_bias(x: torch.Tensor, channel_bias, weight: torch.Tensor, bias: torch.Tensor, eps: float) -> torch.Tensor:
    assert x.is_cuda and x.dtype == torch.float16 and x.is_contiguous() and weight.dtype == torch.float16
    dim = x.shape[-1]
    y = torch.empty_like(x)
    _lib.check(_lib.lib().vlfm_layernorm_bias_f16(x.data_ptr(), channel_bias.data_ptr() if channel_bias is not None else None,
                                                  weight.data_ptr(), bias.data_ptr(), y.data_ptr(), x.numel() // dim, dim,
                                                  float(eps), _stream()), "layernorm_bias_f16")
    return y


_ACT_CODE = {None: 0, "none": 0, "gelu": 1, "silu": 2}


def bias_act_(y: torch.Tensor, bias: torch.Tensor, act=None) -> torch.Tensor:
    assert y.is_cuda and y.dim() == 4 and y.is_contiguous() and y.dtype in (torch.float32, torch.float16)
    assert bias.dtype == y.dtype and bias.numel() == y.shape[1] and bias.is_contiguous()
    n, c, h, w = y.shape
    _lib.check(_lib.lib().vlfm_bias_act_nchw(y.data_ptr(), bias.data_ptr(), n, c, h * w, 0 if y.dtype == torch.float32 else 1,
                                             _ACT_CODE[act], _stream()), "bias_act_nchw")
    return y


_BIAS_ACT_MAX_PLANES = 65535 * 16


class BiasAct(torch.nn.Module):

    def __init__(self, bias: torch.Tensor, act=None, inplace: bool = False):
        super().__init__()
        self.bias = torch.nn.Parameter(bias.detach().clone(), requires_grad=False)
        self.act = act
        self.inplace = inplace

    def forward(self, x):
        return bias_act(x, self.bias, self.act, inplace=self.inplace)


def bias_act(x: torch.Tensor, bias: torch.Tensor, act=None, inplace: bool = False) -> torch.Tensor:
    if (inplace and x.is_cuda and x.dim() == 4 and x.dtype in (torch.float32, torch.float16) and x.is_contiguous()
            and not x.requires_grad and x.shape[0] * x.shape[1] <= _BIAS_ACT_MAX_PLANES):
        return bias_act_(x, bias if bias.dtype == x.dtype else bias.to(x.dtype), act)
    y = x + bias.to(x.dtype).view(1, -1, 1, 1)
    if act == "gelu":
        return torch.nn.functional.gelu(y)
    if act == "silu":
        return torch.nn.functional.silu(y)
    return y


def depthwise_conv3x3(x: torch.Tensor, weight: torch.Tensor, bias, stride: int = 1, gelu: bool = False) -> torch.Tensor:
    assert x.is_cuda and x.dtype == torch.float32 and x.dim() == 4 and x.is_contiguous()
    n, c, h, w = x.shape
    assert weight.shape == (c, 1, 3, 3) and weight.dtype == torch.float32 and weight.is_contiguous()
    ho, wo = (h - 1) // stride + 1, (w - 1) // stride + 1
    y = torch.empty((n, c, ho, wo), dtype=torch.float32, device=x.device)
    _lib.check(_lib.lib().vlfm_dwconv3x3_f32(x.data_ptr(), weight.data_ptr(), bias.data_ptr() if bias is not None else None,
                                             y.data_ptr(), n, c, h, w, int(stride), int(gelu), _stream()), "dwconv3x3_f32")
    return y


def layernorm_rows(x: torch.Tensor, weight: torch.Tensor, bias: torch.Tensor, eps: float, window: int = 0, shift: int = 0,
                   pad_zero: bool = False) -> torch.Tensor:
    assert x.is_cuda and x.dtype == torch.float32 and x.dim() == 4 and x.is_contiguous()
    B, H, W, C = x.shape
    assert weight.dtype == torch.float32 and bias.dtype == torch.float32 and weight.numel() == C == bias.numel()
    if window > 0:
        nwy, nwx = (H + window - 1) // window, (W + window - 1) // window
        out = torch.empty((B * nwy * nwx, window * window, C), dtype=torch.float32, device=x.device)
    else:
        out = torch.empty_like(x)
    _lib.check(_lib.lib().vlfm_layernorm_rows_shifted_f32(x.data_ptr(), weight.data_ptr(), bias.data_ptr(), out.data_ptr(), B, H, W, C,
                                                          int(window), float(eps), int(shift), int(pad_zero), _stream()),
               "layernorm_rows_f32")
    return out


def window_reverse_add_(x: torch.Tensor, windows: torch.Tensor, window: int, shift: int = 0) -> torch.Tensor:
    assert x.is_cuda and x.dtype == torch.float32 and x.dim() == 4 and x.is_contiguous()
    B, H, W, C = x.shape
    nwy, nwx = (H + window - 1) // window, (W + window - 1) // window
    assert windows.is_contiguous() and windows.dtype == torch.float32 and windows.numel() == B * nwy * nwx * window * window * C
    _lib.check(_lib.lib().vlfm_window_reverse_add_shifted_f32(x.data_ptr(), windows.data_ptr(), B, H, W, C, int(window), int(shift),
                                                              _stream()), "window_reverse_add_f32")
    return x


def depthwise_conv3x3_nhwc(x: torch.Tensor, w9c: torch.Tensor, bias) -> torch.Tensor:
    assert x.is_cuda and x.dtype == torch.float32 and x.dim() == 4 and x.is_contiguous()
    B, H, W, C = x.shape
    assert w9c.shape == (9, C) and w9c.is_contiguous() and w9c.dtype == torch.float32
    out = torch.empty_like(x)
    _lib.check(_lib.lib().vlfm_dwconv3x3_nhwc_f32(x.data_ptr(), w9c.data_ptr(), bias.data_ptr() if bias is not None else None,
                                                  out.data_ptr(), B, H, W, C, _stream()), "dwconv3x3_nhwc_f32")
    return out


def window_attention(qkv: torch.Tensor, bias_t: torch.Tensor, heads: int, scale: float, mask_t=None) -> torch.Tensor:
    assert qkv.is_cuda and qkv.dtype == torch.float32 and qkv.dim() == 3 and qkv.is_contiguous() and qkv.shape[2] == heads * 96
    nw, n, _ = qkv.shape
    assert bias_t.shape == (heads, n, n) and bias_t.is_contiguous() and bias_t.dtype == torch.float32 and n <= 256
    out = torch.empty((nw, n, heads * 32), dtype=torch.float32, device=qkv.device)
    per_image = 1
    if mask_t is not None:
        assert mask_t.dim() == 3 and mask_t.shape[1:] == (n, n) and mask_t.is_contiguous() and mask_t.dtype == torch.float32
        per_image = mask_t.shape[0]
        assert nw % per_image == 0
    _lib.check(_lib.lib().vlfm_window_attention_masked_f32(qkv.data_ptr(), bias_t.data_ptr(),
                                                           mask_t.data_ptr() if mask_t is not None else None, per_image,
                                                           out.data_ptr(), nw, n, heads, float(scale), _stream()),
               "window_attention_f32")
    return out


GEMM_F16_EPILOGUE = {"bias": 0, "bias_gelu": 1, "accumulate": 2}


def linear_f16_supported(x: torch.Tensor, weight: torch.Tensor) -> bool:
    k = weight.shape[1]
    return (x.is_cuda and x.dtype == torch.float16 and weight.dtype == torch.float16 and x.shape[-1] == k and k % 64 == 0
            and weight.shape[0] % 8 == 0 and x.numel() * 2 < (1 << 32) and weight.numel() * 2 < (1 << 32))


def linear_f16(x: torch.Tensor, weight: torch.Tensor, bias: Optional[torch.Tensor] = None, epilogue: str = "bias",
               out: Optional[torch.Tensor] = None) -> torch.Tensor:
    assert x.is_cuda and x.dtype == torch.float16 and x.is_contiguous() and x.dim() == 2
    assert weight.dtype == torch.float16 and weight.is_contiguous() and weight.shape[1] == x.shape[1]
    assert bias is None or (bias.dtype == torch.float16 and bias.is_contiguous())
    M, K = x.shape
    N = weight.shape[0]
    assert all(t is None or t.data_ptr() % 16 == 0 for t in (x, weight, bias, out)), "linear_f16: 16-byte aligned tensors only"
    if out is None:
        assert epilogue != "accumulate", "accumulate needs the tensor to accumulate into"
        out = torch.empty((M, N), dtype=torch.float16, device=x.device)
    else:
        assert out.dtype == torch.float16 and out.is_contiguous() and out.shape == (M, N) and out.device == x.device
    _lib.check(_lib.lib().vlfm_gemm_f16_nt(x.data_ptr(), weight.data_ptr(), bias.data_ptr() if bias is not None else None,
                                           out.data_ptr(), M, N, K, GEMM_F16_EPILOGUE[epilogue], _stream()), "gemm_f16_nt")
    return out


def linear_gelu(x: torch.Tensor, weight: torch.Tensor, bias: torch.Tensor) -> torch.Tensor:
    return linear_f16(x, weight, bias, "bias_gelu")


def interleave_pair_weights(w1: torch.Tensor, w2: torch.Tensor) -> torch.Tensor:
    assert w1.shape == w2.shape and w1.dtype == w2.dtype == torch.float16 and w1.dim() == 2 and w1.shape[0] % 64 == 0
    n, k = w1.shape
    return torch.stack([w1.reshape(n // 64, 64, k), w2.reshape(n // 64, 64, k)], dim=1).reshape(2 * n, k).contiguous()


def linear_pair_f32(x: torch.Tensor, w_pair: torch.Tensor, bias: Optional[torch.Tensor] = None,
                    out: Optional[torch.Tensor] = None) -> torch.Tensor:
    assert x.is_cuda and x.dtype == torch.float16 and x.is_contiguous() and x.dim() == 2
    assert w_pair.dtype == torch.float16 and w_pair.is_contiguous() and w_pair.shape[1] == x.shape[1] and w_pair.shape[0] % 128 == 0
    M, K = x.shape
    N = w_pair.shape[0] // 2
    assert bias is None or (bias.dtype == torch.float32 and bias.is_contiguous() and bias.numel() == N)
    assert all(t is None or t.data_ptr() % 16 == 0 for t in (x, w_pair, bias, out)), "linear_pair_f32: 16-byte aligned tensors only"
    if out is None:
        out = torch.empty((N // 64, M, 64), dtype=torch.float32, device=x.device)
    else:
        assert out.dtype == torch.float32 and out.is_contiguous() and out.shape == (N // 64, M, 64) and out.device == x.device
    _lib.check(_lib.lib().vlfm_gemm_f16_pair_f32_nt(x.data_ptr(), w_pair.data_ptr(), bias.data_ptr() if bias is not None else None,
                                                    out.data_ptr(), M, N, K, _stream()), "gemm_f16_pair_f32_nt")
    return out


QFORMER_ATTENTION_MAX_TOKENS, QFORMER_ATTENTION_MAX_QUERIES, QFORMER_ATTENTION_HEAD = 257, 32, 64


def qformer_cross_attention(q: torch.Tensor, kv_blocks: torch.Tensor, tokens: int, heads: int, k_block0: int, v_block0: int,
                            scale: float, out: Optional[torch.Tensor] = None) -> torch.Tensor:
    assert q.is_cuda and q.dtype == torch.float32 and q.is_contiguous() and q.dim() == 3 and q.shape[2] == heads * 64
    assert kv_blocks.dtype == torch.float32 and kv_blocks.is_contiguous() and kv_blocks.dim() == 3 and kv_blocks.shape[2] == 64
    assert kv_blocks.device == q.device and max(k_block0, v_block0) + heads <= kv_blocks.shape[0] and min(k_block0, v_block0) >= 0
    B, Q, _ = q.shape
    if out is None:
        out = torch.empty_like(q)
    else:
        assert out.dtype == torch.float32 and out.is_contiguous() and out.shape[1:] == q.shape[1:] and out.shape[0] >= B
    _lib.check(_lib.lib().vlfm_qformer_cross_attention_f32(q.data_ptr(), kv_blocks.data_ptr(), out.data_ptr(), B, tokens, Q, heads,
                                                           k_block0, v_block0, kv_blocks.shape[1], float(scale), _stream()),
               "qformer_cross_attention_f32")
    return out


VIT_ATTENTION_TOKENS, VIT_ATTENTION_HEADS = 257, (88,)


def vit_attention(qkv: torch.Tensor, batch: int, tokens: int, heads: int, head_dim: int, scale: float) -> torch.Tensor:
    assert qkv.is_cuda and qkv.dtype == torch.float16 and qkv.is_contiguous()
    assert qkv.numel() == batch * tokens * 3 * heads * head_dim
    out = torch.empty((batch * tokens, heads * head_dim), dtype=torch.float16, device=qkv.device)
    _lib.check(_lib.lib().vlfm_vit_attention_f16(qkv.data_ptr(), out.data_ptr(), batch, tokens, heads, head_dim,
                                                 float(scale), _stream()), "vit_attention_f16")
    return out


_ACT32 = {None: 0, "none": 0, "relu": 1, "gelu": 2}
GEMM_F32_PRECISION = {"exact": 0, "split": 1}
_overflow_flags: Dict[tuple, torch.Tensor] = {}
_split_cache: Dict[int, tuple] = {}


def gemm_f32_overflow_flag(device, owner: str = "") -> torch.Tensor:
    d = torch.device(device)
    index = d.index if d.index is not None else (torch.cuda.current_device() if d.type == "cuda" else 0)
    key = (d.type, index, owner)
    if key not in _overflow_flags:
        _overflow_flags[key] = torch.zeros(1, dtype=torch.int32, device=torch.device(d.type, index))
    return _overflow_flags[key]


def tensor_version(t: torch.Tensor) -> int:
    try:
        return t._version
    except RuntimeError:
        return 0


def split_weight(weight: torch.Tensor, owner: str = "") -> Tuple[torch.Tensor, torch.Tensor]:
    import weakref

    key = id(weight)
    hit = _split_cache.get(key)
    if hit is not None and hit[0]() is weight and hit[1] == tensor_version(weight) and hit[2] == weight.data_ptr():
        if hit[6]:
            gemm_f32_overflow_flag(weight.device, owner).bitwise_or_(hit[5])
        return hit[3], hit[4]
    if len(_split_cache) > 2048:
        for k in [k for k, v in _split_cache.items() if v[0]() is None]:
            del _split_cache[k]
    w = weight.detach().contiguous()
    hi = torch.empty(w.shape, dtype=torch.float16, device=w.device)
    lo = torch.empty_like(hi)
    bad = torch.zeros(1, dtype=torch.int32, device=w.device)
    _lib.check(_lib.lib().vlfm_split_f32_to_f16_pair(w.data_ptr(), hi.data_ptr(), lo.data_ptr(), w.numel(), bad.data_ptr(),
                                                     _stream()), "split_f32")
    gemm_f32_overflow_flag(w.device, owner).bitwise_or_(bad)
    _split_cache[key] = [weakref.ref(weight), tensor_version(weight), weight.data_ptr(), hi, lo, bad, False, owner]
    return hi, lo


def split_weights_bad(device, owner: str = "") -> bool:
    d = torch.device(device)
    entries = [v for v in _split_cache.values() if v[7] == owner and v[0]() is not None and v[5].device.type == d.type
               and (d.index is None or v[5].device.index == d.index)]
    if not entries:
        return False
    verdict = torch.cat([v[5] for v in entries]).cpu().tolist()
    for v, b in zip(entries, verdict):
        v[6] = bool(b)
    return any(verdict)


def linear_f32_supported(x: torch.Tensor, weight: torch.Tensor) -> bool:
    k = weight.shape[1]
    return (x.is_cuda and x.dtype == torch.float32 and weight.dtype == torch.float32 and k % 32 == 0 and x.shape[-1] == k
            and weight.shape[0] >= 32 and x.numel() // k >= 64 and not torch.is_grad_enabled())


def linear_f32(x: torch.Tensor, weight: torch.Tensor, bias=None, act=None, residual=None, precision: str = "exact",
               out=None, owner: str = "") -> torch.Tensor:
    K = weight.shape[1]
    N = weight.shape[0]
    lead = x.shape[:-1]
    x2 = x.reshape(-1, K)
    if not x2.is_contiguous() or x2.data_ptr() % 16:
        x2 = x2.contiguous()
    w = weight if weight.is_contiguous() else weight.contiguous()
    M = x2.shape[0]
    if out is None:
        out = torch.empty((M, N), dtype=torch.float32, device=x.device)
    res = None
    if residual is not None:
        res = residual.reshape(M, N)
        if not res.is_contiguous() or res.data_ptr() % 16:
            res = res.contiguous()
    b = None
    if bias is not None:
        b = bias if bias.is_contiguous() else bias.contiguous()
    prec = GEMM_F32_PRECISION[precision]
    hi = lo = None
    if prec == 1:
        hi, lo = split_weight(w, owner)
    _lib.check(_lib.lib().vlfm_gemm_f32_nt(x2.data_ptr(), w.data_ptr(), b.data_ptr() if b is not None else None,
                                           res.data_ptr() if res is not None else None, out.data_ptr(), M, N, K, _ACT32[act], prec,
                                           hi.data_ptr() if hi is not None else None, lo.data_ptr() if lo is not None else None,
                                           gemm_f32_overflow_flag(x.device, owner).data_ptr(), _stream()), "gemm_f32_nt")
    return out.view(*lead, N)


_tuned_gemms_state = None


def use_tuned_gemms() -> bool:
    global _tuned_gemms_state
    if _tuned_gemms_state is None:
        import os

        path = os.path.join(os.path.dirname(os.path.dirname(os.path.abspath(__file__))), "tunableop_results.csv")
        ok = False
        if os.environ.get("VLFM_TUNED_GEMMS", "1") != "0" and os.path.exists(path) and torch.cuda.is_available():
            try:
                import torch.cuda.tunable as tunable

                import tempfile

                tunable.enable(True)
                tunable.tuning_enable(False)
                tunable.set_filename(os.path.join(tempfile.gettempdir(), f"vlfm_amd_tunableop_{os.getpid()}.csv"))
                ok = bool(tunable.read_file(path))
            except Exception as exc:
                import warnings

                warnings.warn(f"tuned GEMM solutions not loaded ({type(exc).__name__}: {exc})")
                ok = False
        _tuned_gemms_state = ok
    return _tuned_gemms_state
```

Before: 1760 env-steps/s.

## Fold ViT LayerNorm2 into fc1 GEMM epilogue using per-row statistics

Instead of materialising the normalised activation before fc1, a light kernel computes per-row rstd and -rstd·mean. The LayerNorm gamma is folded into the fc1 weights, and beta, the fc1 bias and the deferred channel bias become column vectors. A new GEMM epilogue stages these row and column values in LDS and applies the affine correction before GELU. This removes the full write and re-read of the LayerNorm output in every block. A second change replaces the torch cat-plus-add for class and position embeddings with a single fused kernel. The price is extra LDS and epilogue register pressure, plus slightly different rounding, since gamma is now baked into f16 weights.

```diff
diff --git a/include/vlfm_amd.h b/include/vlfm_amd.h
--- a/include/vlfm_amd.h
+++ b/include/vlfm_amd.h
@@ -162,6 +162,11 @@
 int vlfm_layernorm_bias_f16(const void* d_x, const float* d_channel_bias, const void* d_gamma, const void* d_beta,
                             void* d_y, int rows, int dim, float eps, void* stream);
 
+int vlfm_row_stats_f16(const void* d_x, const float* d_channel_bias, void* d_out, int rows, int dim, float eps, void* stream);
+
+int vlfm_vit_assemble_tokens_f16(const void* d_patch, const void* d_cls, const void* d_pos, void* d_out, int batch, int tokens,
+                                 int dim, void* stream);
+
 int vlfm_vit_attention_f16(const void* d_qkv, void* d_out, int batch, int tokens, int heads, int head_dim, float scale,
                            void* stream);
 
@@ -170,6 +175,9 @@
 
 int vlfm_gemm_f16_pair_f32_nt(const void* d_x, const void* d_w_pair, const void* d_bias_f32, void* d_out, int m, int n_out, int k,
                               void* stream);
+
+int vlfm_gemm_f16_ln_gelu_nt(const void* d_x, const void* d_w_folded, const void* d_stats, const void* d_colvec, void* d_c, int m,
+                             int n, int k, void* stream);
 
 int vlfm_qformer_cross_attention_f32(const void* d_q, const void* d_kv_blocks, void* d_out, int batch, int tokens, int queries,
                                      int heads, int k_block0, int v_block0, int m_total, float scale, void* stream);
diff --git a/vlfm_amd/_lib.py b/vlfm_amd/_lib.py
--- a/vlfm_amd/_lib.py
+++ b/vlfm_amd/_lib.py
@@ -127,6 +127,9 @@
                                                         ci, vp, vp, ci, vp]
         L.vlfm_depth_scatter_holes_rig_batched.argtypes = [vp, ci, ci, ci, vp, vp, vp, vp, ci, ci, vp, vp, vp, vp]
         L.vlfm_layernorm_bias_f16.argtypes = [vp, vp, vp, vp, vp, ci, ci, ctypes.c_float, vp]
+        L.vlfm_row_stats_f16.argtypes = [vp, vp, vp, ci, ci, ctypes.c_float, vp]
+        L.vlfm_vit_assemble_tokens_f16.argtypes = [vp, vp, vp, vp, ci, ci, ci, vp]
+        L.vlfm_gemm_f16_ln_gelu_nt.argtypes = [vp, vp, vp, vp, vp, ci, ci, ci, vp]
         L.vlfm_vit_attention_f16.argtypes = [vp, vp, ci, ci, ci, ci, ctypes.c_float, vp]
         L.vlfm_gemm_f16_nt.argtypes = [vp, vp, vp, vp, ci, ci, ci, ci, vp]
         L.vlfm_gemm_f16_pair_f32_nt.argtypes = [vp, vp, vp, vp, ci, ci, ci, vp]
diff --git a/vlfm_amd/csrc/gemm_f16.hip b/vlfm_amd/csrc/gemm_f16.hip
--- a/vlfm_amd/csrc/gemm_f16.hip
+++ b/vlfm_amd/csrc/gemm_f16.hip
@@ -22,7 +22,8 @@
 constexpr int EPI_WAVE = 64 * EPI_ROW;
 constexpr int GEMM_LDS = 8 * EPI_WAVE > 2 * BUF ? 8 * EPI_WAVE : 2 * BUF;
 enum { EPI_BIAS = 0, EPI_BIAS_GELU = 1, EPI_ACCUM = 2,
-       EPI_PAIR_F32 = 3 };
+       EPI_PAIR_F32 = 3,
+       EPI_LN_GELU = 4 };
 
 struct GemmArgs {
     const _Float16* x;
@@ -33,6 +34,7 @@
     int tiles_m, tiles_n;
     int group_m;
     int split_ragged;
+    const float* stats;
 };
 
 using lds_ptr = __attribute__((address_space(3))) unsigned char*;
@@ -223,6 +225,9 @@
 constexpr int EPI2_WAVE = 64 * EPI2_ROW;
 constexpr int PBIAS_OFF = GEMM_LDS;
 constexpr int GEMM_LDS_P = GEMM_LDS + 512;
+constexpr int PLN_OFF = GEMM_LDS_P;
+constexpr int PLN_STATS = PLN_OFF + 3 * 1024;
+constexpr int GEMM_LDS_LN = PLN_STATS + 2048;
 
 __device__ __forceinline__ half8 add_half8(half8 a, const half8 b) {
 #pragma unroll
@@ -275,6 +280,65 @@
     if (a.bias != nullptr && wave == 0 && lane < 32) {
         const _Float16* src = a.bias + min(n_first + lane * 8, a.N - 8);
         __builtin_amdgcn_global_load_lds((gbl_ptr)src, lds + PBIAS_OFF, 16, 0, 0);
+    }
+}
+
+__device__ __forceinline__ int lane_now() {
+    int l;
+    asm volatile("v_mbcnt_lo_u32_b32 %0, -1, 0\n\tv_mbcnt_hi_u32_b32 %0, -1, %0" : "=v"(l));
+    return l;
+}
+struct LnRegs { floatx2 ad[4]; floatx4 s4[4], t4[4], b4[4]; };
+template <int H>
+__device__ __forceinline__ void epi_ln_read(const unsigned char* smem, int wn, int wm, LnRegs& r) {
+    const int ln = lane_now();
+    const unsigned char* prow = smem + PLN_STATS + (wm * 64 + (ln & 15)) * 8;
+    const unsigned char* pcol = smem + PLN_OFF + (wn * 128 + (ln >> 4) * 4) * 4;
+    constexpr int I0 = H * 4;
+#pragma unroll
+    for (int j = 0; j < 4; j++) r.ad[j] = *reinterpret_cast<const floatx2*>(prow + j * 128);
+#pragma unroll
+    for (int ii = 0; ii < 4; ii++) {
+        const int col = (I0 + ii) * 64;
+        r.s4[ii] = *reinterpret_cast<const floatx4*>(pcol + col);
+        r.t4[ii] = *reinterpret_cast<const floatx4*>(pcol + 1024 + col);
+        r.b4[ii] = *reinterpret_cast<const floatx4*>(pcol + 2048 + col);
+    }
+}
+template <int H>
+__device__ __forceinline__ void epi_ln_pass(const floatx4 (&acc)[8][4], const LnRegs& r, unsigned char* stg, int g4, int c16, int rsub, int chunk,
+                                            half8 (&v)[8]) {
+#pragma clang fp contract(off)
+    constexpr int I0 = H * 4;
+#pragma unroll
+    for (int ii = 0; ii < 4; ii++) {
+#pragma unroll
+        for (int j = 0; j < 4; j++) {
+            float z[4];
+#pragma unroll
+            for (int e = 0; e < 4; e++) {
+                const float p = acc[I0 + ii][j][e] + r.t4[ii][e];
+                const float q = __builtin_fmaf(r.ad[j][1], r.s4[ii][e], r.b4[ii][e]);
+                z[e] = __builtin_fmaf(r.ad[j][0], p, q);
+            }
+            gelu_erf4(z[0], z[1], z[2], z[3]);
+            const half4 hv = {(_Float16)z[0], (_Float16)z[1], (_Float16)z[2], (_Float16)z[3]};
+            *reinterpret_cast<half4*>(stg + (j * 16 + c16) * EPI2_ROW + (ii * 16 + g4) * 2) = hv;
+        }
+    }
+    __builtin_amdgcn_s_waitcnt(0xC07F);
+#pragma unroll
+    for (int it = 0; it < 8; it++) v[it] = *reinterpret_cast<const half8*>(stg + (it * 8 + rsub) * EPI2_ROW + chunk * 16);
+}
+__device__ __forceinline__ void stage_ln(const GemmArgs& a, lds_ptr lds, int wave, int m_first, int n_first) {
+    const int lane = lane_now();
+    const float* st = a.stats + min(m_first * 2 + wave * 64 + lane, a.M * 2 - 1);
+    const int dst = __builtin_amdgcn_readfirstlane(PLN_STATS + wave * 256);
+    __builtin_amdgcn_global_load_lds((gbl_ptr)st, lds + dst, 4, 0, 0);
+    if (wave < 3) {
+        const float* src = reinterpret_cast<const float*>(a.bias) + (size_t)wave * (size_t)a.N + min(n_first + lane * 4, a.N - 4);
+        const int dc = __builtin_amdgcn_readfirstlane(PLN_OFF + wave * 1024);
+        __builtin_amdgcn_global_load_lds((gbl_ptr)src, lds + dc, 16, 0, 0);
     }
 }
 
@@ -311,7 +375,8 @@
     const int rsub = lane >> 3, chunk = lane & 7;
     unsigned char* stg = smem + G::KBUF + wave * EPI2_WAVE;
     const bool has_bias = a.bias != nullptr;
-    stage_bias(a, g.lds, wave, lane, n0);
+    if constexpr (EPI == EPI_LN_GELU) stage_ln(a, g.lds, wave, m0, n0);
+    else stage_bias(a, g.lds, wave, lane, n0);
     g.template stage<0>(0, 0); g.template stage<1>(0, 0); g.template stage<2>(0, 0); g.template stage<3>(0, 0);
     if (NT > 1) {
         g.template stage<0>(1, 1); g.template stage<1>(1, 1);
@@ -332,7 +397,11 @@
 
         half4 bias4[EPI == EPI_PAIR_F32 ? 1 : 8];
         floatx4 biasf[EPI == EPI_PAIR_F32 ? 4 : 1];
-        if constexpr (EPI == EPI_PAIR_F32) {
+        LnRegs lnr;
+        if constexpr (EPI == EPI_LN_GELU) {
+            (void)has_bias;
+            epi_ln_read<0>(smem, wn, wm, lnr);
+        } else if constexpr (EPI == EPI_PAIR_F32) {
 #pragma unroll
             for (int i = 0; i < 4; i++) {
                 const floatx4 ld = *reinterpret_cast<const floatx4*>(smem + PBIAS_OFF + (wn * 64 + i * 16 + g4) * 4);
@@ -370,7 +439,7 @@
         }
         __builtin_amdgcn_sched_barrier(0);
         if constexpr (EPI == EPI_PAIR_F32) {
-            (void)bias4; (void)old;
+            (void)bias4; (void)old; (void)lnr;
             floatx4 p0[8], p1[8];
             epi_pair_pass<0>(g.acc, biasf, stg, g4, c16, rsub, chunk, p0);
             epi_pair_pass<1>(g.acc, biasf, stg, g4, c16, rsub, chunk, p1);
@@ -394,8 +463,16 @@
         } else {
         (void)biasf;
         half8 v0[8], v1[8];
-        epi2_pass<EPI, 0>(g.acc, bias4, stg, g4, c16, rsub, chunk, v0);
-        epi2_pass<EPI, 1>(g.acc, bias4, stg, g4, c16, rsub, chunk, v1);
+        if constexpr (EPI == EPI_LN_GELU) {
+            (void)bias4;
+            epi_ln_pass<0>(g.acc, lnr, stg, g4, c16, rsub, chunk, v0);
+            epi_ln_read<1>(smem, wn, wm, lnr);
+            epi_ln_pass<1>(g.acc, lnr, stg, g4, c16, rsub, chunk, v1);
+        } else {
+            (void)lnr;
+            epi2_pass<EPI, 0>(g.acc, bias4, stg, g4, c16, rsub, chunk, v0);
+            epi2_pass<EPI, 1>(g.acc, bias4, stg, g4, c16, rsub, chunk, v1);
+        }
         if (EPI == EPI_ACCUM) {
 #pragma unroll
             for (int it = 0; it < 8; it++) {
@@ -431,7 +508,8 @@
         g.active = n0 + wn * 128 < a.N && (half < 0 || half == wn);
         g.zero_acc();
         g.bar();
-        stage_bias(a, g.lds, wave, lane, n0);
+        if constexpr (EPI == EPI_LN_GELU) stage_ln(a, g.lds, wave, m0, n0);
+        else stage_bias(a, g.lds, wave, lane, n0);
         if (NT > 1) { g.template stage<0>(1, 1); g.template stage<1>(1, 1); }
     }
 }
@@ -445,13 +523,14 @@
 static int launch_gemm(const GemmArgs& a, hipStream_t stream) {
     const void* fn = reinterpret_cast<const void*>(gemm_f16_8pp_kernel<EPI>);
     static LdsOptIn optp;
-    if (!optp.ensure(fn, GEMM_LDS_P)) return fail(VLFM_ERR_HIP, "gemm_f16_nt: cannot opt in to the LDS size");
+    constexpr int lds_bytes = EPI == EPI_LN_GELU ? GEMM_LDS_LN : GEMM_LDS_P;
+    if (!optp.ensure(fn, lds_bytes)) return fail(VLFM_ERR_HIP, "gemm_f16_nt: cannot opt in to the LDS size");
     const int n_cu = device_cu_count() & ~7;
     const int nwg = a.tiles_m * a.tiles_n;
     const dim3 grid(nwg < n_cu ? nwg : n_cu), block(512);
     VLFM_TIMED(EPI == EPI_BIAS ? "gemm_f16_8pp_kernel<0>" : EPI == EPI_BIAS_GELU ? "gemm_f16_8pp_kernel<1>" :
-               EPI == EPI_ACCUM ? "gemm_f16_8pp_kernel<2>" : "gemm_f16_8pp_kernel<3>", stream);
-    VLFM_KLAUNCH((gemm_f16_8pp_kernel<EPI>), grid, block, GEMM_LDS_P, stream, a);
+               EPI == EPI_ACCUM ? "gemm_f16_8pp_kernel<2>" : EPI == EPI_PAIR_F32 ? "gemm_f16_8pp_kernel<3>" : "gemm_f16_8pp_kernel<4>", stream);
+    VLFM_KLAUNCH((gemm_f16_8pp_kernel<EPI>), grid, block, lds_bytes, stream, a);
     return check_launch("gemm_f16_8pp_kernel");
 }
 
@@ -470,6 +549,7 @@
     a.tiles_m = (m + GB - 1) / GB; a.tiles_n = (n + GB - 1) / GB;
     a.group_m = 4;
     a.split_ragged = 1;
+    a.stats = nullptr;
     if (epilogue == 0) return launch_gemm<EPI_BIAS>(a, (hipStream_t)stream);
     if (epilogue == 1) return launch_gemm<EPI_BIAS_GELU>(a, (hipStream_t)stream);
     return launch_gemm<EPI_ACCUM>(a, (hipStream_t)stream);
@@ -492,7 +572,29 @@
     a.tiles_m = (m + GB - 1) / GB; a.tiles_n = (a.N + GB - 1) / GB;
     a.group_m = 4;
     a.split_ragged = 1;
+    a.stats = nullptr;
     return launch_gemm<EPI_PAIR_F32>(a, (hipStream_t)stream);
+}
+
+extern "C" int vlfm_gemm_f16_ln_gelu_nt(const void* d_x, const void* d_w_folded, const void* d_stats, const void* d_colvec, void* d_c,
+                                        int m, int n, int k, void* stream) {
+    if (m == 0 || n == 0) return VLFM_OK;
+    if (!d_x || !d_w_folded || !d_stats || !d_colvec || !d_c || m < 0 || n < 0 || k <= 0 || (k % GK) != 0 || (n % 8) != 0)
+        return fail(VLFM_ERR_INVALID, "gemm_f16_ln_gelu_nt: K must be a multiple of 64, N of 8; row statistics and column vectors are required");
+    if (((uintptr_t)d_x | (uintptr_t)d_w_folded | (uintptr_t)d_stats | (uintptr_t)d_colvec | (uintptr_t)d_c) & 15)
+        return fail(VLFM_ERR_INVALID, "gemm_f16_ln_gelu_nt: X, W, the statistics, the column vectors and C must be 16-byte aligned");
+    if ((size_t)m * (size_t)k * 2 >= (1ull << 32) || (size_t)n * (size_t)k * 2 >= (1ull << 32))
+        return fail(VLFM_ERR_INVALID, "gemm_f16_ln_gelu_nt: an operand of 4 GB or more (32-bit byte offsets inside an operand)");
+    GemmArgs a;
+    a.x = (const _Float16*)d_x; a.w = (const _Float16*)d_w_folded;
+    a.bias = (const _Float16*)d_colvec;
+    a.c = (_Float16*)d_c;
+    a.M = m; a.N = n; a.K = k;
+    a.tiles_m = (m + GB - 1) / GB; a.tiles_n = (n + GB - 1) / GB;
+    a.group_m = 4;
+    a.split_ragged = 1;
+    a.stats = (const float*)d_stats;
+    return launch_gemm<EPI_LN_GELU>(a, (hipStream_t)stream);
 }
 
 extern "C" int vlfm_gemm_f16_tile_order(int m, int n, int group_m, int* out, int capacity_pairs) {
diff --git a/vlfm_amd/csrc/host.cpp b/vlfm_amd/csrc/host.cpp
--- a/vlfm_amd/csrc/host.cpp
+++ b/vlfm_amd/csrc/host.cpp
@@ -13,7 +13,7 @@
 }
 
 extern "C" const char* vlfm_last_error(void) { return vlfm::g_last_error.c_str(); }
-extern "C" int vlfm_abi_version(void) { return 18; }
+extern "C" int vlfm_abi_version(void) { return 19; }
 
 namespace {
 
diff --git a/vlfm_amd/csrc/vlm_ops.hip b/vlfm_amd/csrc/vlm_ops.hip
--- a/vlfm_amd/csrc/vlm_ops.hip
+++ b/vlfm_amd/csrc/vlm_ops.hip
@@ -313,6 +313,92 @@
 #pragma unroll
         for (int i = 0; i < NV; i++) { cur[i] = nxt[i]; nxt[i] = nx2[i]; }
     }
+}
+
+template <int NV>
+__global__ __launch_bounds__(256) void row_stats_f16_kernel(const __half* __restrict__ x, const float* __restrict__ cb,
+                                                            float2* __restrict__ out, int rows, int D, float eps, int rows_per_wave) {
+    const int lane = threadIdx.x & 63, wave = (blockIdx.x * blockDim.x + threadIdx.x) >> 6;
+    const int nvec = D >> 3;
+    const int r0 = wave * rows_per_wave;
+    if (r0 >= rows) return;
+    float4 c0[NV], c1[NV];
+#pragma unroll
+    for (int i = 0; i < NV; i++) {
+        const int v = lane + 64 * i;
+        if (v < nvec) {
+            c0[i] = cb ? reinterpret_cast<const float4*>(cb)[2 * v] : make_float4(0.f, 0.f, 0.f, 0.f);
+            c1[i] = cb ? reinterpret_cast<const float4*>(cb)[2 * v + 1] : make_float4(0.f, 0.f, 0.f, 0.f);
+        }
+    }
+    Half8 cur[NV], nxt[NV], nx2[NV];
+    auto load_row = [&](int r, Half8* dst) {
+#pragma unroll
+        for (int i = 0; i < NV; i++) {
+            const int v = lane + 64 * i;
+            if (v < nvec) dst[i] = reinterpret_cast<const Half8*>(x + (size_t)r * D)[v];
+        }
+    };
+    auto val = [&](const Half8* row, int i, int j) -> float {
+        const float2 t = __half22float2(row[i].h[j >> 1]);
+        const float cc = j < 4 ? (&c0[i].x)[j] : (&c1[i].x)[j - 4];
+        return ((j & 1) ? t.y : t.x) + cc;
+    };
+    const int r_end = min(rows, r0 + rows_per_wave);
+    load_row(r0, cur);
+    if (r0 + 1 < r_end) load_row(r0 + 1, nxt);
+    const float inv_d = 1.0f / (float)D;
+    for (int r = r0; r < r_end; r++) {
+        if (r + 2 < r_end) load_row(r + 2, nx2);
+        float sum = 0.0f;
+#pragma unroll
+        for (int i = 0; i < NV; i++) {
+            if (lane + 64 * i < nvec) {
+#pragma unroll
+                for (int j = 0; j < 8; j++) sum += val(cur, i, j);
+            }
+        }
+#pragma unroll
+        for (int off = 32; off > 0; off >>= 1) sum += __shfl_xor(sum, off, 64);
+        const float mean = sum * inv_d;
+        float sq = 0.0f;
+#pragma unroll
+        for (int i = 0; i < NV; i++) {
+            if (lane + 64 * i < nvec) {
+#pragma unroll
+                for (int j = 0; j < 8; j++) {
+                    const float dlt = val(cur, i, j) - mean;
+                    sq = fmaf(dlt, dlt, sq);
+                }
+            }
+        }
+#pragma unroll
+        for (int off = 32; off > 0; off >>= 1) sq += __shfl_xor(sq, off, 64);
+        const float rstd = rsqrtf(sq * inv_d + eps);
+        if (lane == 0) out[r] = make_float2(rstd, -(rstd * mean));
+#pragma unroll
+        for (int i = 0; i < NV; i++) { cur[i] = nxt[i]; nxt[i] = nx2[i]; }
+    }
+}
+
+__global__ __launch_bounds__(256) void vit_assemble_tokens_f16_kernel(const Half8* __restrict__ patch, const Half8* __restrict__ cls,
+                                                                      const Half8* __restrict__ pos, Half8* __restrict__ out,
+                                                                      int tokens, int nvec, size_t total) {
+    const size_t v = (size_t)blockIdx.x * blockDim.x + threadIdx.x;
+    if (v >= total) return;
+    const size_t row = v / (size_t)nvec;
+    const int col = (int)(v - row * (size_t)nvec);
+    const size_t b = row / (size_t)tokens;
+    const int t = (int)(row - b * (size_t)tokens);
+    const Half8 a = t == 0 ? cls[col] : patch[(b * (size_t)(tokens - 1) + (size_t)(t - 1)) * (size_t)nvec + col];
+    const Half8 p = pos[(size_t)t * nvec + col];
+    Half8 o;
+#pragma unroll
+    for (int j = 0; j < 4; j++) {
+        const float2 fa = __half22float2(a.h[j]), fp = __half22float2(p.h[j]);
+        o.h[j] = __floats2half2_rn(fa.x + fp.x, fa.y + fp.y);
+    }
+    out[v] = o;
 }
 
 __global__ __launch_bounds__(512) void itc_head_kernel(const float* __restrict__ proj, int NQ, int P,
@@ -594,3 +680,43 @@
     }
     return check_launch("layernorm_bias_f16_kernel");
 }
+
+extern "C" int vlfm_row_stats_f16(const void* d_x, const float* d_channel_bias, void* d_out, int rows, int dim, float eps,
+                                  void* stream) {
+    if (rows == 0) return VLFM_OK;
+    if (!d_x || !d_out || rows < 0 || dim <= 0 || dim % 8 != 0 || dim > 64 * 8 * LN_MAXV)
+        return fail(VLFM_ERR_INVALID, "row_stats_f16: dim must be a multiple of 8 and <= 2048");
+    if ((((uintptr_t)d_x | (uintptr_t)d_channel_bias) & 15) || ((uintptr_t)d_out & 7))
+        return fail(VLFM_ERR_INVALID, "row_stats_f16: x and the channel constant must be 16-byte aligned, the result 8-byte aligned");
+    const int nvec = dim / 8, nv = (nvec + 63) / 64;
+    int rpw = rows / 8192;
+    rpw = rpw < 1 ? 1 : rpw > LN_ROWS ? LN_ROWS : rpw;
+    const int waves = (rows + rpw - 1) / rpw;
+    const dim3 grid((waves + 3) / 4), block(256);
+    const __half* x = (const __half*)d_x;
+    float2* out = (float2*)d_out;
+    VLFM_TIMED("row_stats_f16_kernel", stream);
+    switch (nv) {
+        case 1: VLFM_KLAUNCH(row_stats_f16_kernel<1>, grid, block, 0, (hipStream_t)stream, x, d_channel_bias, out, rows, dim, eps, rpw); break;
+        case 2: VLFM_KLAUNCH(row_stats_f16_kernel<2>, grid, block, 0, (hipStream_t)stream, x, d_channel_bias, out, rows, dim, eps, rpw); break;
+        case 3: VLFM_KLAUNCH(row_stats_f16_kernel<3>, grid, block, 0, (hipStream_t)stream, x, d_channel_bias, out, rows, dim, eps, rpw); break;
+        default: VLFM_KLAUNCH(row_stats_f16_kernel<4>, grid, block, 0, (hipStream_t)stream, x, d_channel_bias, out, rows, dim, eps, rpw); break;
+    }
+    return check_launch("row_stats_f16_kernel");
+}
+
+extern "C" int vlfm_vit_assemble_tokens_f16(const void* d_patch, const void* d_cls, const void* d_pos, void* d_out, int batch,
+                                            int tokens, int dim, void* stream) {
+    if (batch == 0) return VLFM_OK;
+    if (!d_patch || !d_cls || !d_pos || !d_out || batch < 0 || tokens < 2 || dim <= 0 || dim % 8 != 0)
+        return fail(VLFM_ERR_INVALID, "vit_assemble_tokens_f16: tokens >= 2 and dim a multiple of 8");
+    if (((uintptr_t)d_patch | (uintptr_t)d_cls | (uintptr_t)d_pos | (uintptr_t)d_out) & 15)
+        return fail(VLFM_ERR_INVALID, "vit_assemble_tokens_f16: every pointer must be 16-byte aligned");
+    const int nvec = dim / 8;
+    const size_t total = (size_t)batch * (size_t)tokens * (size_t)nvec;
+    if ((total + 255) / 256 > 0x7fffffffull) return fail(VLFM_ERR_INVALID, "vit_assemble_tokens_f16: too many tokens for one launch");
+    VLFM_TIMED("vit_assemble_tokens_f16_kernel", stream);
+    VLFM_KLAUNCH(vit_assemble_tokens_f16_kernel, dim3((unsigned)((total + 255) / 256)), dim3(256), 0, (hipStream_t)stream,
+                 (const Half8*)d_patch, (const Half8*)d_cls, (const Half8*)d_pos, (Half8*)d_out, tokens, nvec, total);
+    return check_launch("vit_assemble_tokens_f16_kernel");
+}
diff --git a/vlfm_amd/vlm/blip2itm.py b/vlfm_amd/vlm/blip2itm.py
--- a/vlfm_amd/vlm/blip2itm.py
+++ b/vlfm_amd/vlm/blip2itm.py
@@ -64,6 +64,8 @@
         self.strict_hip_attention = True
         self.hip_mlp_min_rows = 32 * 257
         self.hip_gemms = frozenset(DEFAULT_HIP_GEMMS)
+        self.fold_ln2 = True
+        self._ln2_fold = None
 
     def pack_heads(self, multiple: int = 32) -> None:
         h, d = self.heads, self.qkv.in_features
@@ -135,16 +137,44 @@
             q = self.qkv(h).view(b, n, 3, self.heads, hd).permute(2, 0, 3, 1, 4)
             a = F.scaled_dot_product_attention(q[0], q[1], q[2]).transpose(1, 2).reshape(b * n, d)
             x2.addmm_(a, self.projection.weight.t())
+        if self.folds_ln2(hip) and x2.is_contiguous():
+            wf, colvec = self._ln2_constants(c_mid)
+            stats = ops.row_stats(x, c_mid, self.layer_norm2.eps)
+            act = ops.linear_gelu(x2, wf, None, (stats, colvec))
+        else:
+            act = self._fc1_unfolded(x, c_mid, hip)
+        if "fc2" in hip and x2.is_contiguous():
+            ops.linear_f16(act, self.fc2.weight, None, "accumulate", out=x2)
+        else:
+            x2.addmm_(act, self.fc2.weight.t())
+        return x
+
+    def folds_ln2(self, hip: frozenset) -> bool:
+        from . import ops
+
+        return bool(self.fold_ln2) and "fc1" in hip and ops.row_stats_supported(self.fc1.in_features) \
+            and x_is_contiguous_f16(self.layer_norm2.weight) and x_is_contiguous_f16(self.layer_norm2.bias)
+
+    def _ln2_constants(self, c_mid: torch.Tensor):
+        from . import ops
+
+        f = self._ln2_fold
+        if f is None or f[0].device != c_mid.device or f[2] != c_mid.data_ptr():
+            wf, colvec = ops.fold_layernorm_weights(self.fc1.weight, self.fc1.bias, self.layer_norm2.weight, self.layer_norm2.bias,
+                                                    c_mid)
+            f = self._ln2_fold = (wf, colvec, c_mid.data_ptr())
+        return f[0], f[1]
+
+    def _fc1_unfolded(self, x: torch.Tensor, c_mid: torch.Tensor, hip: frozenset) -> torch.Tensor:
+        from . import ops
+
+        b, n, d = x.shape
         h = ops.layernorm_bias(x, c_mid, self.layer_norm2.weight, self.layer_norm2.bias, self.layer_norm2.eps)
         if "fc1" in hip:
             act = ops.linear_gelu(h.view(b * n, d), self.fc1.weight, self.fc1.bias)
         else:
             act = F.gelu(F.linear(h, self.fc1.weight, self.fc1.bias)).view(b * n, -1)
-        if "fc2" in hip and x2.is_contiguous():
-            ops.linear_f16(act, self.fc2.weight, None, "accumulate", out=x2)
-        else:
-            x2.addmm_(act, self.fc2.weight.t())
-        return x
+        return act
 
     def forward(self, x: torch.Tensor) -> torch.Tensor:
         b, n, d = x.shape
@@ -322,6 +352,8 @@
         self._deferred_c = None
         self._kv_all = None
         self._kv_pair = None
+        for blk in self.blocks:
+            blk._ln2_fold = None
         for layer in self.q_layers:
             layer.attention._qkv_fused = None
             if layer.crossattention is not None:
@@ -470,8 +502,15 @@
                 .reshape(b, g * g, 3 * c.patch_size * c.patch_size)
         w = self.patch_embedding.weight
         x = F.linear(pixel_values.to(w.dtype), w.view(w.shape[0], -1), self.patch_embedding.bias)
-        x = torch.cat([self.class_embedding.expand(x.shape[0], -1, -1), x], dim=1) + self.position_embedding
-        if self.deferred_bias and x.is_cuda and x.dtype == torch.float16 and c.v_hidden % 8 == 0 and c.v_hidden <= 2048:
+        fast = self.deferred_bias and x.is_cuda and x.dtype == torch.float16 and c.v_hidden % 8 == 0 and c.v_hidden <= 2048
+        if (fast and x.is_contiguous() and x_is_contiguous_f16(self.class_embedding) and x_is_contiguous_f16(self.position_embedding)
+                and x.data_ptr() % 16 == 0):
+            from . import ops
+
+            x = ops.assemble_tokens(x, self.class_embedding, self.position_embedding)
+        else:
+            x = torch.cat([self.class_embedding.expand(x.shape[0], -1, -1), x], dim=1) + self.position_embedding
+        if fast:
             from . import ops
 
             c = self._deferred_constants()
@@ -689,7 +728,8 @@
     def gemm_path(self, n_images: int) -> str:
         blk = self.model.blocks[0]
         rows = n_images * ((self.cfg.image_size // self.cfg.patch_size) ** 2 + 1)
-        names = sorted(blk.hip_gemms_at(rows))
+        hip = blk.hip_gemms_at(rows)
+        names = [n + "+ln" if n == "fc1" and blk.folds_ln2(hip) else n for n in sorted(hip)]
         return "hip:" + ",".join(names) if names else "library"
 
     def _load_pretrained(self, model_dir: str) -> None:
diff --git a/vlfm_amd/vlm/ops.py b/vlfm_amd/vlm/ops.py
--- a/vlfm_amd/vlm/ops.py
+++ b/vlfm_amd/vlm/ops.py
@@ -145,6 +145,34 @@
     return y
 
 
+ROW_STATS_MAX_DIM = 2048
+
+
+def row_stats_supported(dim: int) -> bool:
+    return dim % 8 == 0 and 0 < dim <= ROW_STATS_MAX_DIM
+
+
+def row_stats(x: torch.Tensor, channel_bias, eps: float) -> torch.Tensor:
+    assert x.is_cuda and x.dtype == torch.float16 and x.is_contiguous()
+    assert channel_bias is None or (channel_bias.dtype == torch.float32 and channel_bias.is_contiguous())
+    dim = x.shape[-1]
+    rows = x.numel() // dim
+    out = torch.empty((rows, 2), dtype=torch.float32, device=x.device)
+    _lib.check(_lib.lib().vlfm_row_stats_f16(x.data_ptr(), channel_bias.data_ptr() if channel_bias is not None else None,
+                                             out.data_ptr(), rows, dim, float(eps), _stream()), "row_stats_f16")
+    return out
+
+
+def assemble_tokens(patch: torch.Tensor, cls: torch.Tensor, pos: torch.Tensor) -> torch.Tensor:
+    assert patch.is_cuda and patch.dim() == 3 and all(t.dtype == torch.float16 and t.is_contiguous() for t in (patch, cls, pos))
+    B, P, D = patch.shape
+    assert cls.numel() == D and pos.numel() == (P + 1) * D
+    out = torch.empty((B, P + 1, D), dtype=torch.float16, device=patch.device)
+    _lib.check(_lib.lib().vlfm_vit_assemble_tokens_f16(patch.data_ptr(), cls.data_ptr(), pos.data_ptr(), out.data_ptr(), B, P + 1, D,
+                                                       _stream()), "vit_assemble_tokens_f16")
+    return out
+
+
 _ACT_CODE = {None: 0, "none": 0, "gelu": 1, "silu": 2}
 
 
@@ -275,8 +303,38 @@
     return out
 
 
-def linear_gelu(x: torch.Tensor, weight: torch.Tensor, bias: torch.Tensor) -> torch.Tensor:
+def linear_gelu(x: torch.Tensor, weight: torch.Tensor, bias: Optional[torch.Tensor], ln=None) -> torch.Tensor:
+    if ln is not None:
+        assert bias is None
+        return linear_ln_gelu(x, weight, ln[0], ln[1])
     return linear_f16(x, weight, bias, "bias_gelu")
+
+
+def fold_layernorm_weights(weight: torch.Tensor, bias: Optional[torch.Tensor], gamma: torch.Tensor, beta: torch.Tensor,
+                           channel_bias: Optional[torch.Tensor]) -> Tuple[torch.Tensor, torch.Tensor]:
+    w64, g64, be64 = weight.detach().double(), gamma.detach().double(), beta.detach().double()
+    wf = (w64 * g64).to(torch.float16).contiguous()
+    wf64 = wf.double()
+    s = wf64.sum(dim=1)
+    t = wf64 @ channel_bias.detach().double() if channel_bias is not None else torch.zeros_like(s)
+    b = w64 @ be64
+    if bias is not None:
+        b = b + bias.detach().double()
+    return wf, torch.stack([s, t, b]).to(torch.float32).contiguous()
+
+
+def linear_ln_gelu(x: torch.Tensor, w_folded: torch.Tensor, stats: torch.Tensor, colvec: torch.Tensor) -> torch.Tensor:
+    assert x.is_cuda and x.dtype == torch.float16 and x.is_contiguous() and x.dim() == 2
+    assert w_folded.dtype == torch.float16 and w_folded.is_contiguous() and w_folded.shape[1] == x.shape[1]
+    M, K = x.shape
+    N = w_folded.shape[0]
+    assert stats.dtype == torch.float32 and stats.is_contiguous() and stats.shape == (M, 2)
+    assert colvec.dtype == torch.float32 and colvec.is_contiguous() and colvec.shape == (3, N)
+    assert all(t.data_ptr() % 16 == 0 for t in (x, w_folded, stats, colvec)), "linear_ln_gelu: 16-byte aligned tensors only"
+    out = torch.empty((M, N), dtype=torch.float16, device=x.device)
+    _lib.check(_lib.lib().vlfm_gemm_f16_ln_gelu_nt(x.data_ptr(), w_folded.data_ptr(), stats.data_ptr(), colvec.data_ptr(),
+                                                   out.data_ptr(), M, N, K, _stream()), "gemm_f16_ln_gelu_nt")
+    return out
 
 
 def interleave_pair_weights(w1: torch.Tensor, w2: torch.Tensor) -> torch.Tensor:
```

Result: no change. 1772 env-steps/s (median of 6 runs) (+0.7%).
